# hitbc/deSAMBA

Measured on AMD Instinct MI355X. Metric: classified reads/s (50 kbp ONT reads, viral index), higher is better.
Workload: dtype u8/u64 integer

## Files before the change

desamba_amd/__init__.py:

```python
import ctypes as C
import os

_HERE = os.path.dirname(os.path.abspath(__file__))
LIB_PATH = os.environ.get("DSB_LIB_PATH", os.path.join(_HERE, "libdesamba_amd.so"))

DSB_OK, DSB_EIO, DSB_ENODEV, DSB_ENOMEM, DSB_EINVAL, DSB_ECAP = 0, -1, -2, -3, -4, -5


class DsbOpts(C.Structure):
    _fields_ = [("L_min_matching", C.c_int), ("min_score", C.c_int), ("max_sec_N", C.c_int), ("n_slots", C.c_int),
                ("max_read_len", C.c_uint32), ("max_batch_reads", C.c_uint32), ("input_slots", C.c_int), ("reserved", C.c_int), ("max_batch_bases", C.c_uint64)]


class DsbRead(C.Structure):
    _fields_ = [("name", C.c_char_p), ("seq", C.c_char_p), ("qual", C.c_char_p), ("len", C.c_uint32)]


class DsbHit(C.Structure):
    _fields_ = [("ref_ID", C.c_uint32), ("t_st", C.c_uint32), ("t_ed", C.c_uint32), ("q_st", C.c_uint32), ("q_ed", C.c_uint32),
                ("sum_score", C.c_uint32), ("indel", C.c_uint32), ("direction", C.c_uint8), ("primary", C.c_uint8),
                ("pri_index", C.c_uint8), ("pad", C.c_uint8)]

    def key(self):
        return (self.ref_ID, self.t_st, self.t_ed, self.q_st, self.q_ed, self.sum_score, self.direction, self.primary, self.pri_index)


class DsbReadResult(C.Structure):
    _fields_ = [("first", C.c_uint32), ("n", C.c_uint32), ("status", C.c_int32), ("fast", C.c_uint32), ("device_us", C.c_uint32), ("n_anc", C.c_uint32)]


class DsbResult(C.Structure):
    _fields_ = [("reads", C.POINTER(DsbReadResult)), ("hits", C.POINTER(DsbHit)), ("n_hits", C.c_size_t)]


class DsbSeed(C.Structure):
    _fields_ = [("offset", C.c_uint32), ("len", C.c_uint32), ("top", C.c_uint8), ("pad", C.c_uint8 * 3)]


class DsbTiming(C.Structure):
    _fields_ = [("encode_ms", C.c_float), ("seed_probe_ms", C.c_float), ("classify_ms", C.c_float), ("total_ms", C.c_float),
                ("windows", C.c_uint64), ("probes_t1", C.c_uint64), ("bases", C.c_uint64),
                ("order_ms", C.c_float), ("tail_ms", C.c_float), ("n_early", C.c_uint32), ("n_retry", C.c_uint32),
                ("n_regrow", C.c_uint32), ("seed_scan", C.c_uint32),
                ("n_occ", C.c_uint64), ("n_mem", C.c_uint64), ("n_sa", C.c_uint64), ("ref_bases", C.c_uint64),
                ("main_occ", C.c_uint64), ("main_mem", C.c_uint64), ("main_sa", C.c_uint64), ("main_ref_bases", C.c_uint64),
                ("n_heavy_mw", C.c_uint32), ("n_requeue", C.c_uint32), ("upload_bytes", C.c_uint64),
                ("anc_pool_asked", C.c_uint64), ("anc_pool_cap", C.c_uint64)]


class DsbBuildStats(C.Structure):
    _fields_ = [(n, C.c_uint64) for n in ("n_bases", "n_refs", "n_kmer", "n_unitig", "n_rows")] + \
               [(n, C.c_double) for n in ("parse_s", "sort_s", "graph_s", "walk_s", "rows_s", "tables_s", "write_s", "total_s")] + \
               [(n, C.c_uint64) for n in ("budget_bytes", "peak_device_bytes")] + \
               [(n, C.c_uint32) for n in ("ranges_kmers", "ranges_unitig_numbers", "ranges_rows", "ranges_exist")] + \
               [("spilled_bytes", C.c_uint64)]


class DsbReadTaxon(C.Structure):
    _fields_ = [("taxid", C.c_uint32), ("score", C.c_uint32), ("len", C.c_uint32), ("mapq", C.c_uint8), ("flags", C.c_uint8), ("pad", C.c_uint16)]


DSB_TAXON_CLASSIFIED, DSB_TAXON_HOST = 1, 2


class DsbRefCoverage(C.Structure):
    _fields_ = [("numreads", C.c_uint64), ("covbases", C.c_uint64), ("aligned_bases", C.c_uint64), ("mapq_sum", C.c_uint64)]


COVERAGE_FIELDS = ("numreads", "covbases", "aligned_bases", "mapq_sum")


class DsbEmOpts(C.Structure):
    _fields_ = [("max_iter", C.c_uint32), ("reserved", C.c_uint32), ("tol", C.c_double)]


class DsbAbundanceSummary(C.Structure):
    _fields_ = [("reads", C.c_uint64), ("classified", C.c_uint64), ("classes", C.c_uint64), ("iterations", C.c_uint32),
                ("converged", C.c_uint32), ("max_change", C.c_double), ("min_permille", C.c_uint32), ("reserved", C.c_uint32)]


ABUNDANCE_DTYPE = [("numreads", "<u8"), ("uniqreads", "<u8"), ("est_reads", "<f8"), ("read_share", "<f8"), ("copy_share", "<f8")]


class DsbReadLca(C.Structure):
    _fields_ = [("taxid", C.c_uint32), ("score", C.c_uint32), ("n_pass", C.c_uint32), ("depth", C.c_uint16), ("flags", C.c_uint8), ("pad", C.c_uint8)]


DSB_LCA_CLASSIFIED, DSB_LCA_NO_TAXON, DSB_LCA_AMBIGUOUS = 1, 2, 4
LCA_DTYPE = [("taxid", "<u4"), ("score", "<u4"), ("n_pass", "<u4"), ("depth", "<u2"), ("flags", "u1"), ("pad", "u1")]
TAXON_COUNT_DTYPE = [("taxid", "<u4"), ("pad", "<u4"), ("clade_reads", "<u8"), ("direct_reads", "<u8")]


class DsbLcaSummary(C.Structure):
    _fields_ = [("reads", C.c_uint64), ("classified", C.c_uint64), ("no_taxon", C.c_uint64), ("ambiguous", C.c_uint64),
                ("min_permille", C.c_uint32), ("reserved", C.c_uint32)]


LCA_SUMMARY_FIELDS = ("reads", "classified", "no_taxon", "ambiguous", "min_permille")


class DsbChunk(C.Structure):
    _fields_ = [("start", C.c_uint64), ("end", C.c_uint64), ("hist_max_before", C.c_uint32), ("rank", C.c_int32)]


EXPORTS = ["dsb_index_open", "dsb_index_close", "dsb_index_n_ref", "dsb_index_ref_name", "dsb_index_ref_len", "dsb_index_ek_len",
           "dsb_index_occ_host", "dsb_ctx_create", "dsb_ctx_destroy", "dsb_ctx_reset_history", "dsb_ctx_reload_env", "dsb_classify_batch",
           "dsb_batch_upload", "dsb_batch_upload_fastq", "dsb_batch_upload_text", "dsb_ctx_set_history", "dsb_host_alloc", "dsb_host_free", "dsb_host_cpus", "dsb_batch_run", "dsb_batch_fetch", "dsb_batch_timing", "dsb_batch_seeds", "dsb_batch_exist_bits",
           "dsb_format_sam", "dsb_format_des", "dsb_strerror", "dsb_version",
           "dsb_device_count", "dsb_ctx_select_slot", "dsb_ctx_create_multi", "dsb_multi_destroy", "dsb_multi_n", "dsb_multi_ctx",
           "dsb_multi_reset_history", "dsb_multi_last_calls", "dsb_multi_classify_batch", "dsb_shard_plan", "dsb_ctx_use_synthetic_filter", "dsb_synthetic_filter_bit", "dsb_index_prefix_interval", "dsb_index_build",
           "dsb_taxonomy_load", "dsb_taxonomy_load_any", "dsb_taxonomy_close", "dsb_taxonomy_max_tid", "dsb_taxonomy_parent",
           "dsb_ctx_set_taxonomy", "dsb_multi_set_taxonomy", "dsb_batch_taxa", "dsb_multi_taxa",
           "dsb_report_create", "dsb_report_add", "dsb_report_add_sam", "dsb_report_format", "dsb_report_destroy",
           "dsb_ctx_enable_coverage", "dsb_ctx_reset_coverage", "dsb_ctx_coverage", "dsb_multi_enable_coverage", "dsb_multi_coverage",
           "dsb_coverage_format", "dsb_ctx_enable_abundance", "dsb_ctx_reset_abundance", "dsb_ctx_abundance", "dsb_multi_enable_abundance",
           "dsb_multi_abundance", "dsb_abundance_format",
           "dsb_ctx_enable_lca", "dsb_ctx_reset_lca", "dsb_batch_lca", "dsb_ctx_lca_counts", "dsb_multi_enable_lca", "dsb_multi_lca",
           "dsb_multi_lca_counts", "dsb_taxnames_load", "dsb_taxnames_close", "dsb_format_kraken", "dsb_lca_report_format"]

_lib = None


def lib():
    global _lib
    if _lib is not None:
        return _lib
    if not os.path.exists(LIB_PATH):
        raise RuntimeError("desamba_amd: %s is missing -- run __graft_entry__.build(); there is no CPU fallback" % LIB_PATH)
    L = C.CDLL(LIB_PATH)
    L.dsb_index_open.argtypes = [C.c_char_p, C.POINTER(C.c_void_p)]
    L.dsb_index_close.argtypes = [C.c_void_p]
    L.dsb_index_n_ref.argtypes = [C.c_void_p]; L.dsb_index_n_ref.restype = C.c_uint64
    L.dsb_index_ref_name.argtypes = [C.c_void_p, C.c_uint32]; L.dsb_index_ref_name.restype = C.c_char_p
    L.dsb_index_ref_len.argtypes = [C.c_void_p, C.c_uint32]; L.dsb_index_ref_len.restype = C.c_uint64
    L.dsb_index_ek_len.argtypes = [C.c_void_p]
    L.dsb_index_occ_host.argtypes = [C.c_void_p, C.c_uint64, C.POINTER(C.c_uint8)]; L.dsb_index_occ_host.restype = C.c_uint64
    L.dsb_ctx_create.argtypes = [C.c_void_p, C.c_int, C.POINTER(DsbOpts), C.POINTER(C.c_void_p)]
    L.dsb_ctx_destroy.argtypes = [C.c_void_p]
    L.dsb_ctx_reset_history.argtypes = [C.c_void_p]
    L.dsb_ctx_reload_env.argtypes = [C.c_void_p]; L.dsb_ctx_reload_env.restype = None
    L.dsb_classify_batch.argtypes = [C.c_void_p, C.POINTER(DsbRead), C.c_size_t, C.POINTER(DsbResult)]
    L.dsb_batch_upload.argtypes = [C.c_void_p, C.POINTER(DsbRead), C.c_size_t]
    L.dsb_batch_upload_fastq.argtypes = [C.c_void_p, C.c_char_p, C.c_size_t, C.c_size_t]; L.dsb_batch_upload_fastq.restype = C.c_long
    L.dsb_batch_run.argtypes = [C.c_void_p]
    L.dsb_batch_fetch.argtypes = [C.c_void_p, C.POINTER(DsbResult)]
    L.dsb_batch_timing.argtypes = [C.c_void_p, C.POINTER(DsbTiming)]
    L.dsb_batch_seeds.argtypes = [C.c_void_p, C.c_size_t, C.c_int, C.POINTER(DsbSeed), C.c_size_t, C.POINTER(C.c_uint32), C.POINTER(C.c_uint32)]
    L.dsb_batch_exist_bits.argtypes = [C.c_void_p, C.c_size_t, C.c_int, C.POINTER(C.c_uint8), C.c_size_t, C.POINTER(C.c_uint32)]
    L.dsb_format_sam.argtypes = [C.c_void_p, C.POINTER(DsbRead), C.POINTER(DsbHit), C.c_uint32, C.c_int, C.c_int, C.c_char_p, C.c_size_t]
    L.dsb_format_sam.restype = C.c_long
    L.dsb_format_des.argtypes = [C.c_void_p, C.POINTER(DsbRead), C.POINTER(DsbReadResult), C.POINTER(DsbHit), C.c_int, C.c_int, C.c_char_p, C.c_size_t]
    L.dsb_format_des.restype = C.c_long
    L.dsb_batch_upload_text.argtypes = [C.c_void_p, C.c_void_p, C.c_size_t, C.POINTER(C.c_uint64), C.POINTER(C.c_uint32), C.c_size_t]
    L.dsb_ctx_set_history.argtypes = [C.c_void_p, C.c_uint32]; L.dsb_ctx_set_history.restype = None
    L.dsb_host_alloc.argtypes = [C.c_size_t]; L.dsb_host_alloc.restype = C.c_void_p
    L.dsb_host_free.argtypes = [C.c_void_p]; L.dsb_host_free.restype = None
    L.dsb_device_count.argtypes = []; L.dsb_device_count.restype = C.c_int
    L.dsb_ctx_select_slot.argtypes = [C.c_void_p, C.c_int]
    L.dsb_ctx_create_multi.argtypes = [C.c_void_p, C.POINTER(C.c_int), C.c_int, C.POINTER(DsbOpts), C.POINTER(C.c_void_p)]
    L.dsb_multi_destroy.argtypes = [C.c_void_p]; L.dsb_multi_destroy.restype = None
    L.dsb_multi_n.argtypes = [C.c_void_p]
    L.dsb_multi_ctx.argtypes = [C.c_void_p, C.c_int]; L.dsb_multi_ctx.restype = C.c_void_p
    L.dsb_multi_reset_history.argtypes = [C.c_void_p]; L.dsb_multi_reset_history.restype = None
    L.dsb_multi_last_calls.argtypes = [C.c_void_p, C.c_int]; L.dsb_multi_last_calls.restype = C.c_uint32
    L.dsb_multi_classify_batch.argtypes = [C.c_void_p, C.POINTER(DsbRead), C.c_size_t, C.POINTER(DsbResult)]
    L.dsb_shard_plan.argtypes = [C.POINTER(C.c_uint32), C.c_size_t, C.c_int, C.c_uint64, C.c_uint32, C.POINTER(DsbChunk), C.c_size_t, C.POINTER(C.c_size_t)]
    L.dsb_ctx_use_synthetic_filter.argtypes = [C.c_void_p, C.c_uint64, C.c_double]
    L.dsb_synthetic_filter_bit.argtypes = [C.c_int, C.c_uint64, C.c_double]
    L.dsb_index_prefix_interval.argtypes = [C.c_void_p, C.c_uint32, C.c_int, C.POINTER(C.c_uint64), C.POINTER(C.c_uint64)]
    L.dsb_index_build.argtypes = [C.c_char_p, C.c_char_p, C.c_char_p, C.c_int, C.POINTER(DsbBuildStats)]
    L.dsb_index_close.restype = None; L.dsb_ctx_destroy.restype = None; L.dsb_ctx_reset_history.restype = None
    L.dsb_taxonomy_load.argtypes = [C.c_char_p, C.POINTER(C.c_void_p)]
    L.dsb_taxonomy_load_any.argtypes = [C.c_char_p, C.POINTER(C.c_void_p)]
    L.dsb_taxonomy_close.argtypes = [C.c_void_p]; L.dsb_taxonomy_close.restype = None
    L.dsb_taxonomy_max_tid.argtypes = [C.c_void_p]; L.dsb_taxonomy_max_tid.restype = C.c_uint32
    L.dsb_taxonomy_parent.argtypes = [C.c_void_p, C.c_uint32]; L.dsb_taxonomy_parent.restype = C.c_uint32
    L.dsb_ctx_set_taxonomy.argtypes = [C.c_void_p, C.c_void_p]
    L.dsb_multi_set_taxonomy.argtypes = [C.c_void_p, C.c_void_p]
    L.dsb_batch_taxa.argtypes = [C.c_void_p, C.POINTER(C.POINTER(DsbReadTaxon))]
    L.dsb_multi_taxa.argtypes = [C.c_void_p, C.POINTER(C.POINTER(DsbReadTaxon))]
    L.dsb_report_create.argtypes = [C.c_void_p, C.POINTER(C.c_void_p)]
    L.dsb_report_add.argtypes = [C.c_void_p, C.c_void_p, C.POINTER(DsbRead), C.POINTER(DsbResult), C.POINTER(DsbReadTaxon), C.c_size_t, C.c_int]
    L.dsb_report_add_sam.argtypes = [C.c_void_p, C.c_char_p, C.c_size_t]
    L.dsb_report_format.argtypes = [C.c_void_p, C.c_int, C.c_char_p, C.c_size_t]; L.dsb_report_format.restype = C.c_long
    L.dsb_report_destroy.argtypes = [C.c_void_p]; L.dsb_report_destroy.restype = None
    L.dsb_ctx_enable_coverage.argtypes = [C.c_void_p, C.c_int]
    L.dsb_ctx_reset_coverage.argtypes = [C.c_void_p]
    L.dsb_ctx_coverage.argtypes = [C.c_void_p, C.c_void_p]
    L.dsb_multi_enable_coverage.argtypes = [C.c_void_p, C.c_int]
    L.dsb_multi_coverage.argtypes = [C.c_void_p, C.c_void_p]
    L.dsb_coverage_format.argtypes = [C.c_void_p, C.c_void_p, C.c_char_p, C.c_size_t]; L.dsb_coverage_format.restype = C.c_long
    L.dsb_ctx_enable_abundance.argtypes = [C.c_void_p, C.c_int, C.c_uint32]
    L.dsb_ctx_reset_abundance.argtypes = [C.c_void_p]
    L.dsb_ctx_abundance.argtypes = [C.c_void_p, C.c_void_p, C.c_void_p, C.c_void_p]
    L.dsb_multi_enable_abundance.argtypes = [C.c_void_p, C.c_int, C.c_uint32]
    L.dsb_multi_abundance.argtypes = [C.c_void_p, C.c_void_p, C.c_void_p, C.c_void_p]
    L.dsb_abundance_format.argtypes = [C.c_void_p, C.c_void_p, C.c_void_p, C.c_char_p, C.c_size_t]; L.dsb_abundance_format.restype = C.c_long
    L.dsb_ctx_enable_lca.argtypes = [C.c_void_p, C.c_int, C.c_uint32]
    L.dsb_ctx_reset_lca.argtypes = [C.c_void_p]
    L.dsb_batch_lca.argtypes = [C.c_void_p, C.POINTER(C.POINTER(DsbReadLca))]
    L.dsb_ctx_lca_counts.argtypes = [C.c_void_p, C.c_void_p, C.c_size_t, C.POINTER(C.c_size_t), C.c_void_p]
    L.dsb_multi_enable_lca.argtypes = [C.c_void_p, C.c_int, C.c_uint32]
    L.dsb_multi_lca.argtypes = [C.c_void_p, C.POINTER(C.POINTER(DsbReadLca))]
    L.dsb_multi_lca_counts.argtypes = [C.c_void_p, C.c_void_p, C.c_size_t, C.POINTER(C.c_size_t), C.c_void_p]
    L.dsb_taxnames_load.argtypes = [C.c_char_p, C.POINTER(C.c_void_p)]
    L.dsb_taxnames_close.argtypes = [C.c_void_p]; L.dsb_taxnames_close.restype = None
    L.dsb_format_kraken.argtypes = [C.c_void_p, C.c_void_p, C.c_char_p, C.c_size_t]; L.dsb_format_kraken.restype = C.c_long
    L.dsb_lca_report_format.argtypes = [C.c_void_p, C.c_void_p, C.c_void_p, C.c_size_t, C.c_void_p, C.c_char_p, C.c_size_t]; L.dsb_lca_report_format.restype = C.c_long
    L.dsb_strerror.argtypes = [C.c_int]; L.dsb_strerror.restype = C.c_char_p
    L.dsb_version.restype = C.c_char_p
    _lib = L
    return L


class DsbError(RuntimeError):
    def __init__(self, code, what):
        RuntimeError.__init__(self, "%s: %s (%d)" % (what, lib().dsb_strerror(code).decode(), code))
        self.code = code


class Index:

    def __init__(self, path):
        self.h = C.c_void_p()
        rc = lib().dsb_index_open(os.fsencode(path), C.byref(self.h))
        if rc != 0:
            raise DsbError(rc, "dsb_index_open(%s)" % path)
        self.path = path

    def close(self):
        if self.h:
            lib().dsb_index_close(self.h); self.h = C.c_void_p()

    @property
    def n_ref(self):
        return lib().dsb_index_n_ref(self.h)

    @property
    def ek_len(self):
        return lib().dsb_index_ek_len(self.h)

    def ref_name(self, i):
        return lib().dsb_index_ref_name(self.h, i).decode()

    def ref_len(self, i):
        return int(lib().dsb_index_ref_len(self.h, i))

    def occ_host(self, r, c):
        cc = C.c_uint8(c)
        v = lib().dsb_index_occ_host(self.h, r, C.byref(cc))
        return v, cc.value


def build_index(fasta, out_dir, kmer_srt=None, device=0):
    st = DsbBuildStats()
    rc = lib().dsb_index_build(kmer_srt.encode() if kmer_srt else None, fasta.encode(), out_dir.encode(), device, C.byref(st))
    if rc != 0:
        raise DsbError(rc, "dsb_index_build(%s)" % fasta)
    return st


def make_reads(records):
    n = len(records)
    arr = (DsbRead * n)()
    keep = []
    for i, (name, seq, qual) in enumerate(records):
        name = name if isinstance(name, bytes) else name.encode()
        seq = seq if isinstance(seq, bytes) else seq.encode()
        qual = (qual if isinstance(qual, bytes) else qual.encode()) if qual is not None else None
        keep.append((name, seq, qual))
        arr[i].name, arr[i].seq, arr[i].qual, arr[i].len = name, seq, qual, len(seq)
    arr._keep = keep
    return arr


class Ctx:

    def __init__(self, index, device=0, L_min_matching=170, min_score=64, max_sec_N=5, n_slots=0, max_read_len=0, max_batch_reads=0, input_slots=1, max_batch_bases=0):
        self.index = index
        self.opts = DsbOpts(L_min_matching, min_score, max_sec_N, n_slots, max_read_len, max_batch_reads, input_slots, 0, max_batch_bases)
        self.h = C.c_void_p()
        rc = lib().dsb_ctx_create(index.h, device, C.byref(self.opts), C.byref(self.h))
        if rc != 0:
            raise DsbError(rc, "dsb_ctx_create(device %d)" % device)
        self.reads = None
        self.slot = 0
        self.staged = {}
        self.ran = (None, 0)

    def close(self):
        if self.h:
            lib().dsb_ctx_destroy(self.h); self.h = C.c_void_p()

    def reset_history(self):
        lib().dsb_ctx_reset_history(self.h)

    def reload_env(self):
        lib().dsb_ctx_reload_env(self.h)

    def set_history(self, max_len_before):
        lib().dsb_ctx_set_history(self.h, max_len_before)

    def use_synthetic_filter(self, table_bytes, fill):
        rc = lib().dsb_ctx_use_synthetic_filter(self.h, table_bytes, fill)
        if rc != 0:
            raise DsbError(rc, "dsb_ctx_use_synthetic_filter")
        self.synthetic = (table_bytes, fill)

    def select_slot(self, slot):
        rc = lib().dsb_ctx_select_slot(self.h, slot)
        if rc != 0:
            raise DsbError(rc, "dsb_ctx_select_slot(%d)" % slot)
        self.slot = slot

    def upload_text(self, text_ptr, text_len, seq_off, seq_len, n):
        self.reads = None
        rc = lib().dsb_batch_upload_text(self.h, text_ptr, text_len, seq_off, seq_len, n)
        if rc != 0:
            raise DsbError(rc, "dsb_batch_upload_text")
        self.staged[self.slot] = (None, int(n))

    def upload(self, reads):
        self.reads = reads
        rc = lib().dsb_batch_upload(self.h, reads, len(reads))
        if rc != 0:
            raise DsbError(rc, "dsb_batch_upload")
        self.staged[self.slot] = (reads, len(reads))

    def upload_fastq(self, path, skip=0, max_reads=1 << 62):
        self.reads = None
        n = lib().dsb_batch_upload_fastq(self.h, os.fsencode(path), skip, max_reads)
        if n < 0:
            raise DsbError(int(n), "dsb_batch_upload_fastq(%s)" % path)
        self.n_uploaded = int(n)
        self.staged[self.slot] = (None, int(n))
        return int(n)

    def run(self):
        rc = lib().dsb_batch_run(self.h)
        if rc != 0:
            raise DsbError(rc, "dsb_batch_run")
        self.ran = self.staged.get(self.slot, (None, 0))

    def fetch(self, strict=True):
        res = DsbResult()
        rc = lib().dsb_batch_fetch(self.h, C.byref(res))
        if rc != 0 and (strict or rc != DSB_ECAP):
            raise DsbError(rc, "dsb_batch_fetch")
        return res

    def classify(self, reads, strict=True):
        self.upload(reads); self.run()
        return self.fetch(strict)

    def timing(self):
        t = DsbTiming()
        lib().dsb_batch_timing(self.h, C.byref(t))
        return t

    def seeds(self, read, strand):
        cap = (self.reads[read].len >> 1) + 64
        buf = (DsbSeed * cap)(); n = C.c_uint32(); ts = C.c_uint32()
        rc = lib().dsb_batch_seeds(self.h, read, strand, buf, cap, C.byref(n), C.byref(ts))
        if rc != 0:
            raise DsbError(rc, "dsb_batch_seeds")
        return [(buf[i].offset, buf[i].len, buf[i].top) for i in range(n.value)], ts.value

    def exist_bits(self, read, strand):
        cap = self.reads[read].len + 1
        buf = (C.c_uint8 * cap)(); n = C.c_uint32()
        rc = lib().dsb_batch_exist_bits(self.h, read, strand, buf, cap, C.byref(n))
        if rc != 0:
            raise DsbError(rc, "dsb_batch_exist_bits")
        return bytes(buf[:n.value])

    def set_taxonomy(self, taxonomy):
        rc = lib().dsb_ctx_set_taxonomy(self.h, taxonomy.h if taxonomy is not None else None)
        if rc != 0:
            raise DsbError(rc, "dsb_ctx_set_taxonomy")
        self.taxonomy = taxonomy

    def taxa(self, records=False):
        p = C.POINTER(DsbReadTaxon)()
        rc = lib().dsb_batch_taxa(self.h, C.byref(p))
        if rc != 0:
            raise DsbError(rc, "dsb_batch_taxa")
        n = self.in_last_batch()
        return _taxa(p, n, records)

    def enable_coverage(self, on=True):
        rc = lib().dsb_ctx_enable_coverage(self.h, 1 if on else 0)
        if rc != 0:
            raise DsbError(rc, "dsb_ctx_enable_coverage")

    def reset_coverage(self):
        rc = lib().dsb_ctx_reset_coverage(self.h)
        if rc != 0:
            raise DsbError(rc, "dsb_ctx_reset_coverage")

    def coverage(self):
        return _coverage(lib().dsb_ctx_coverage, self.h, self.index.n_ref, "dsb_ctx_coverage")

    def enable_abundance(self, on=True, min_frac=0.95):
        rc = lib().dsb_ctx_enable_abundance(self.h, 1 if on else 0, _permille(min_frac) if on else 0)
        if rc != 0:
            raise DsbError(rc, "dsb_ctx_enable_abundance")

    def reset_abundance(self):
        rc = lib().dsb_ctx_reset_abundance(self.h)
        if rc != 0:
            raise DsbError(rc, "dsb_ctx_reset_abundance")

    def abundance(self, max_iter=10000, tol=0.01):
        return _abundance(lib().dsb_ctx_abundance, self.h, self.index.n_ref, max_iter, tol, "dsb_ctx_abundance")

    def enable_lca(self, on=True, min_frac=0.95):
        rc = lib().dsb_ctx_enable_lca(self.h, 1 if on else 0, _permille(min_frac) if on else 0)
        if rc != 0:
            raise DsbError(rc, "dsb_ctx_enable_lca")

    def reset_lca(self):
        rc = lib().dsb_ctx_reset_lca(self.h)
        if rc != 0:
            raise DsbError(rc, "dsb_ctx_reset_lca")

    def lca(self):
        p = C.POINTER(DsbReadLca)()
        rc = lib().dsb_batch_lca(self.h, C.byref(p))
        if rc != 0:
            raise DsbError(rc, "dsb_batch_lca")
        return _lca(p, self.in_last_batch())

    def lca_counts(self):
        return _lca_counts(lib().dsb_ctx_lca_counts, self.h, "dsb_ctx_lca_counts")

    def in_last_batch(self):
        return self.ran[1]

    def sam(self, res, full=False, reads=None):
        if reads is None:
            reads = self.ran[0] if self.ran[0] is not None else self.reads
        return format_sam(self.index, reads, res, self.opts.max_sec_N, full)


def format_sam(index, reads, res, max_sec_N=5, full=False):
    out = []
    buf = C.create_string_buffer(1 << 20)
    for i in range(len(reads)):
        rr = res.reads[i]
        hits = C.cast(C.byref(res.hits.contents, rr.first * C.sizeof(DsbHit)), C.POINTER(DsbHit)) if rr.n else None
        cap = len(buf)
        need = 4096 + 700 * rr.n + (2 * reads[i].len if full else 0)
        if need > cap:
            buf = C.create_string_buffer(need)
        n = lib().dsb_format_sam(index.h, C.byref(reads[i]), hits, rr.n, max_sec_N, 1 if full else 0, buf, len(buf))
        if n < 0:
            raise DsbError(DSB_EINVAL, "dsb_format_sam")
        out.append(buf.raw[:n])
    return b"".join(out)


class Multi:

    def __init__(self, index, devices, L_min_matching=170, min_score=64, max_sec_N=5, n_slots=0):
        self.index = index
        self.opts = DsbOpts(L_min_matching, min_score, max_sec_N, n_slots, 0, 0, 1, 0)
        ids = (C.c_int * len(devices))(*devices)
        self.h = C.c_void_p()
        rc = lib().dsb_ctx_create_multi(index.h, ids, len(devices), C.byref(self.opts), C.byref(self.h))
        if rc != 0:
            raise DsbError(rc, "dsb_ctx_create_multi(%r)" % (devices,))

    def close(self):
        if self.h:
            lib().dsb_multi_destroy(self.h); self.h = C.c_void_p()

    def reset_history(self):
        lib().dsb_multi_reset_history(self.h)

    def last_calls(self):
        return [int(lib().dsb_multi_last_calls(self.h, i)) for i in range(int(lib().dsb_multi_n(self.h)))]

    def classify(self, reads, strict=True):
        res = DsbResult()
        rc = lib().dsb_multi_classify_batch(self.h, reads, len(reads), C.byref(res))
        if rc != 0 and (strict or rc != DSB_ECAP):
            raise DsbError(rc, "dsb_multi_classify_batch")
        self.n_last = len(reads)
        return res

    def set_taxonomy(self, taxonomy):
        rc = lib().dsb_multi_set_taxonomy(self.h, taxonomy.h if taxonomy is not None else None)
        if rc != 0:
            raise DsbError(rc, "dsb_multi_set_taxonomy")
        self.taxonomy = taxonomy

    def enable_coverage(self, on=True):
        rc = lib().dsb_multi_enable_coverage(self.h, 1 if on else 0)
        if rc != 0:
            raise DsbError(rc, "dsb_multi_enable_coverage")

    def coverage(self):
        return _coverage(lib().dsb_multi_coverage, self.h, self.index.n_ref, "dsb_multi_coverage")

    def enable_abundance(self, on=True, min_frac=0.95):
        rc = lib().dsb_multi_enable_abundance(self.h, 1 if on else 0, _permille(min_frac) if on else 0)
        if rc != 0:
            raise DsbError(rc, "dsb_multi_enable_abundance")

    def reset_abundance(self):
        for i in range(int(lib().dsb_multi_n(self.h))):
            rc = lib().dsb_ctx_reset_abundance(lib().dsb_multi_ctx(self.h, i))
# ... 310 lines not shown
```

desamba_amd/csrc/dsb_ctx.h:

```cpp
#pragma once
#include <stdio.h>
#include <string.h>
#include <time.h>
#include <string>
#include "dsb_seed_scan.h"
#include "dsb_reductions.h"

#define HIPCHK(e) do { hipError_t _e = (e); if (_e != hipSuccess) { fprintf(stderr, "[desamba_amd] HIP error %s at %s:%d\n", hipGetErrorString(_e), __FILE__, __LINE__); return DSB_ENODEV; } } while (0)

struct DsbStaged;

struct InSlot {
	DsbReadDesc *d_rd = nullptr; char *d_ascii = nullptr; size_t cap_rd = 0, cap_ascii = 0;
	std::vector<DsbReadDesc> h_rd;
	size_t n_reads = 0; uint64_t n_words_total = 0, total_bases = 0, total_windows = 0, seed_entries = 0; uint32_t max_len = 0, min_len = 0;
	uint32_t *d_scan_order = nullptr; size_t cap_scan_order = 0;
	bool ragged = false;
	uint64_t upload_bytes = 0;
	bool packed = false;
};

struct UpStage { char *buf[2] = {nullptr, nullptr}; hipEvent_t ev[2] = {nullptr, nullptr}; bool used[2] = {false, false}; hipStream_t st = nullptr; };

struct DsbKnobs {
	bool upload_text = false;
	bool debug = false, upload_trace = false, no_turn = false, turn_whole_run = false, no_group = false, heavy_first_set = false;
	long hout_cap = 0, sms_cap = 0, anc_cap_rt = 0, upload_chunk_kb = 0, step_limit_rt = 0, group_head = -1;
	int upload_threads = 0, seed_scan = -1, heavy_mw = -1, heavy_first = 0;
	bool heavy_preds_set = false; uint32_t heavy_preds = 0;
	uint64_t em_hash_mask = ~0ull;
	bool anchor_kernel = true; long anc_pool_rt = 0;
	bool scan_look_set = false; DsbScanLook scan_look;
	std::string order_file;
};
inline bool g_upload_trace = false;

struct dsb_ctx {
	bool ek_dense = false;
	DsbKnobs knobs;
	dsb_index *idx = nullptr; int device = 0; hipStream_t stream = nullptr;
	DsbStaged *staged = nullptr; DsbDevIndex dx;
	std::vector<InSlot> in; int cur = 0;
	DsbWordDesc *d_wd = nullptr; uint8_t *d_bin = nullptr; uint64_t *d_pk = nullptr; uint64_t *d_bits = nullptr;
	size_t cap_wd = 0, cap_bin = 0, cap_pk = 0, cap_bits = 0;
	DsbReadOut *d_rout = nullptr; DsbHitOut *d_hout = nullptr; size_t cap_rout = 0, cap_hout = 0;
	unsigned int *d_counters = nullptr;
	DsbSlotArena arena; int n_slots = 0, n_extra = 0;
	DsbSlotArena arena_big; int n_slots_big = 0;
	DsbSlotArena arena_anc; int n_slots_anc = 0;
	DsbAncRec *d_arec = nullptr; DsbAnchor *d_apool = nullptr; size_t cap_arec = 0, cap_apool = 0;
	uint32_t hint_len = 0;
	unsigned mw_reads = 16; bool mw_grown = false; int mw_calm = 0;
	uint32_t *d_score = nullptr, *d_order = nullptr, *d_heavy = nullptr; size_t cap_score = 0, cap_order = 0, cap_heavy = 0;
	DsbSeed *d_seeds = nullptr; DsbSeedInfo *d_sinfo = nullptr; size_t cap_seeds = 0, cap_sinfo = 0;
	uint8_t *d_summ = nullptr; int summ_shift = 0;
	uint8_t *syn0 = nullptr, *syn1 = nullptr; bool seed_only = false;
	bool bits_valid = false, seeds_valid = false;
	unsigned n_early = 0;
	std::vector<DsbReadOut> h_rout; std::vector<DsbHitOut> h_hout;
	std::vector<dsb_read_result> res_reads;
	int hist_max = 0;
	hipEvent_t ev[4] = {nullptr, nullptr, nullptr, nullptr}; dsb_timing timing; unsigned long long p1 = 0;
	hipStream_t stream3 = nullptr; hipEvent_t ev_heavy3 = nullptr;
	hipStream_t stream2 = nullptr; hipEvent_t ev_order = nullptr, ev_heavy = nullptr, ev_hprobe = nullptr, ev_cls = nullptr, ev_cls_wait = nullptr;
	uint32_t *dbg_host = nullptr, *dbg_dev = nullptr;
	std::vector<UpStage> up; size_t up_chunk = 0;
	dsb_opts opts;
	DsbTaxa taxa; DsbCover cover; DsbEmStore em; DsbLca lca;
	dsb_ctx() { memset(&dx, 0, sizeof dx); memset(&arena, 0, sizeof arena); memset(&arena_big, 0, sizeof arena_big); memset(&arena_anc, 0, sizeof arena_anc); memset(&timing, 0, sizeof timing); memset(&opts, 0, sizeof opts); }
};

struct dsb_multi {
	dsb_index *idx = nullptr; std::vector<dsb_ctx *> ctx; uint32_t hist = 0;
	uint32_t chunk_reads_env = 0;
	std::vector<uint32_t> last_calls;
	std::vector<dsb_read_result> reads; std::vector<dsb_hit> hits;
	const dsb_taxonomy *tx = nullptr; std::vector<dsb_read_taxon> taxa; bool taxa_ok = false;
	std::vector<dsb_read_lca> lca; bool lca_on = false, lca_ok = false;
};

template <class T> static int grow(T **p, size_t *cap, size_t need)
{
	if (need <= *cap) return 0;
	const bool tr = g_upload_trace; struct timespec t0, t1; if (tr) clock_gettime(CLOCK_MONOTONIC, &t0);
	const size_t old = *cap;
	if (*p) hipFree(*p);
	size_t n = need + need / 8 + 1024;
	if (hipMalloc((void **)p, n * sizeof(T)) != hipSuccess) { *p = nullptr; *cap = 0; return DSB_ENOMEM; }
	*cap = n;
	if (tr) { clock_gettime(CLOCK_MONOTONIC, &t1); fprintf(stderr, "[upload] a device buffer grew from %zu to %zu elements of %zu bytes (needed: %zu) in %.3f s\n", old, n, sizeof(T), need, (t1.tv_sec - t0.tv_sec) + 1e-9 * (t1.tv_nsec - t0.tv_nsec)); }
	return 0;
}
```

desamba_amd/csrc/dsb_gpu.hip:

```cpp
#include <hip/hip_runtime.h>
#include <stdint.h>
#include <stdio.h>
#include <string.h>
#include <stdlib.h>
#include <vector>
#include <string>
#include <unistd.h>
#include <fcntl.h>
#include <sys/mman.h>
#include <sys/stat.h>
#include "dsb_device.h"
#include "dsb_probe.h"
#include "dsb_seed_scan.h"
#define DSB_GROUP 64
#define DSB_NS dsb_g64
#include "dsb_classify_dev.h"
#undef DSB_GROUP
#undef DSB_NS
#include "dsb_host.h"
#include "dsb_sam_fields.h"

#if !defined(DSB_KUNIT)
#define DSB_UNIT_HAS(n) 1
#define DSB_UNIT_HOST 1
// ... 170 lines not shown
}
#define DSB_HPROBE_SPLIT 16
__global__ void __launch_bounds__(256) k_seed_probe_reads(DsbDevIndex x, const DsbReadDesc *__restrict__ rd, const uint32_t *__restrict__ list,
                                                          const uint64_t *__restrict__ pk, uint64_t *__restrict__ bits, const uint8_t *__restrict__ summ, int summ_shift)
{
	const int lane = threadIdx.x & 63;
	const uint32_t wave = __builtin_amdgcn_readfirstlane((uint32_t)((blockIdx.x % DSB_HPROBE_SPLIT) * 4 + (threadIdx.x >> 6)));
	const uint32_t r = list[blockIdx.x / DSB_HPROBE_SPLIT];
	const uint32_t n_words = rd[r].n_words, n_items = 2 * n_words;
	const int k = x.ek_len; const int sbm = x.single_base_max;
	const uint64_t kmask = k >= 32 ? ~0ULL : ((1ULL << (2 * k)) - 1ULL);
	unsigned long long p1_local = 0;
	for (uint32_t w0 = wave * DSB_PROBE_UN; w0 < n_items; w0 += 4 * DSB_HPROBE_SPLIT * DSB_PROBE_UN) {
		DsbWordDesc wds[DSB_PROBE_UN]; bool have[DSB_PROBE_UN];
#pragma unroll
		for (int u = 0; u < DSB_PROBE_UN; u++) {
			uint32_t it = w0 + u; have[u] = it < n_items;
			wds[u].read = r; wds[u].word = it >= n_words ? ((it - n_words) | 0x80000000u) : it;
		}
		probe_un(x, rd, pk, bits, wds, have, lane, k, sbm, kmask, summ, summ_shift, p1_local);
	}
}


__global__ void __launch_bounds__(256) k_seed_scan(DsbDevIndex x, const DsbReadDesc *__restrict__ rd, const uint32_t *__restrict__ order, uint32_t n_reads,
                                                   const uint64_t *__restrict__ pk, DsbSeed *__restrict__ seeds, DsbSeedInfo *__restrict__ sinfo,
                                                   const uint8_t *__restrict__ summ, int summ_shift, unsigned long long *counters, DsbScanLook look)
{
	const uint64_t g = (uint64_t)blockIdx.x * 256 + threadIdx.x;
	const bool active = g < 2ull * n_reads;
	const uint32_t r = active ? (order ? order[g >> 1] : (uint32_t)(g >> 1)) : 0u;
	const bool rc = (g & 1) != 0;
	DsbReadDesc d = rd[r];
	const uint64_t *__restrict__ P = pk + d.pk_off;
	const uint32_t L = d.len, nF = L >> 2, cap = rc ? ((L >> 1) + 64 - nF) : nF;
	DsbSeed *__restrict__ sv = seeds + d.seed_off + (rc ? nF : 0);
	auto store = [&](uint32_t idx, uint32_t off, uint32_t len) { if (idx < cap) { DsbSeed v; v.offset = off; v.len = (uint16_t)len; v.top = 0; sv[idx] = v; } };
	auto mark = [&](uint32_t idx) { if (idx < cap) sv[idx].top = 1; };
	const int k = x.ek_len, sbm = x.single_base_max;
	const uint64_t kmask = k >= 32 ? ~0ULL : ((1ULL << (2 * k)) - 1ULL);
	DsbScan s; dsb_scan_init(s, active ? d.n_win : 0u, look);
	uint32_t p0 = 0, p1 = 0;
	uint64_t K0 = 0, K1 = 0, K2 = 0; uint32_t wbase = 0xfffffff0u;
	for (;;) {
		if (!__any(s.mode != DSB_SCAN_DONE)) break;
		uint32_t want[DSB_SCAN_W]; dsb_scan_want(s, want);
		uint32_t lo = DSB_SCAN_NONE;
#pragma unroll
		for (int t = 0; t < DSB_SCAN_W; t++) lo = want[t] < lo ? want[t] : lo;
		const uint32_t base = lo & ~31u;
		if (lo != DSB_SCAN_NONE) {
			const uint32_t wi = lo >> 5;
			uint64_t n0, n1, n2;
#define DSB_SCAN_WORD(dst, idx) \
			if ((idx) == wbase) dst = K0; else if ((idx) == wbase + 1) dst = K1; else if ((idx) == wbase + 2) dst = K2; \
			else { dst = P[idx]; if (rc) dst = dsb_revcomp_kmer(dst, 32); }
			DSB_SCAN_WORD(n0, wi) DSB_SCAN_WORD(n1, wi + 1) DSB_SCAN_WORD(n2, wi + 2)
#undef DSB_SCAN_WORD
			K0 = n0; K1 = n1; K2 = n2; wbase = wi;
		}
		const uint64_t B0 = rc ? K2 : K0, B1 = K1, B2 = rc ? K0 : K2;
		uint64_t km[DSB_SCAN_W], h1[DSB_SCAN_W]; bool ok[DSB_SCAN_W];
#pragma unroll
		for (int t = 0; t < DSB_SCAN_W; t++) {
			ok[t] = want[t] != DSB_SCAN_NONE; km[t] = 0; h1[t] = 0;
			if (ok[t]) {
				uint32_t rel = want[t] - base;
				if (rc) rel = 96u - rel - (uint32_t)k;
				const uint64_t a = rel < 32 ? B0 : rel < 64 ? B1 : B2, b = rel < 32 ? B1 : B2; const uint32_t sh = (rel & 31u) * 2;
				const uint64_t hi = sh ? ((a << sh) | (b >> (64 - sh))) : a;
				const uint64_t v = (hi >> (64 - 2 * k)) & kmask;
				ok[t] = dsb_kmer_ok(v, k, sbm); km[t] = v;
				if (ok[t]) { p0++; h1[t] = dsb_ph1(v) & x.ek_mask; }
			}
		}
		if (summ) {
			uint8_t sb[DSB_SCAN_W];
#pragma unroll
			for (int t = 0; t < DSB_SCAN_W; t++) { sb[t] = 0xff; if (ok[t]) sb[t] = summ[(h1[t] >> summ_shift) >> 3]; }
#pragma unroll
			for (int t = 0; t < DSB_SCAN_W; t++) ok[t] = ok[t] && ((sb[t] >> ((h1[t] >> summ_shift) & 7)) & 1);
		}
		uint8_t t0[DSB_SCAN_W];
#pragma unroll
		for (int t = 0; t < DSB_SCAN_W; t++) { t0[t] = 0; if (ok[t]) t0[t] = x.ek0[h1[t] >> 3]; }
		bool any1 = false;
#pragma unroll
		for (int t = 0; t < DSB_SCAN_W; t++) { ok[t] = ok[t] && ((t0[t] >> (7 - (h1[t] & 7))) & 1); any1 |= ok[t]; }
		uint32_t bits = 0;
		if (__any(any1)) {
			uint8_t t1[DSB_SCAN_W]; uint64_t h2[DSB_SCAN_W];
#pragma unroll
			for (int t = 0; t < DSB_SCAN_W; t++) { t1[t] = 0; h2[t] = 0; if (ok[t]) { h2[t] = dsb_ph2(km[t]) & x.ek_mask; t1[t] = x.ek1[h2[t] >> 3]; p1++; } }
#pragma unroll
			for (int t = 0; t < DSB_SCAN_W; t++) if (ok[t] && ((t1[t] >> (7 - (h2[t] & 7))) & 1)) bits |= 1u << t;
		}
		if (s.mode != DSB_SCAN_DONE) dsb_scan_consume(s, bits, rc, store, mark);
	}
	dsb_scan_finish(s, mark);
	if (active) { sinfo[r].n_seed[rc ? 1 : 0] = s.ns; sinfo[r].total[rc ? 1 : 0] = s.total; if (!rc) { sinfo[r].flags = 0; sinfo[r].pad = 0; } }
	if (counters) {
		unsigned long long a0 = p0, a1 = p1;
		for (int o = 32; o > 0; o >>= 1) { a0 += __shfl_down(a0, o); a1 += __shfl_down(a1, o); }
		if ((threadIdx.x & 63) == 0) { if (a0) atomicAdd(counters, a0); if (a1) atomicAdd(counters + 1, a1); }
	}
}

__host__ __device__ inline uint32_t dsb_synth_mix(uint64_t b, uint32_t which)
{
	uint64_t z = b * 0x9E3779B97F4A7C15ULL + ((uint64_t)which + 1) * 0xD1342543DE82EF95ULL;
	z = (z ^ (z >> 30)) * 0xBF58476D1CE4E5B9ULL; z = (z ^ (z >> 27)) * 0x94D049BB133111EBULL;
	return (uint32_t)((z ^ (z >> 31)) >> 40);
}
__global__ void __launch_bounds__(256) k_synth_table(uint8_t *tab, uint64_t n_bytes, uint32_t which, uint32_t thresh)
{
	for (uint64_t i = (uint64_t)blockIdx.x * 256 + threadIdx.x; i < n_bytes; i += (uint64_t)gridDim.x * 256) {
		uint32_t v = 0;
#pragma unroll
		for (int j = 0; j < 8; j++) if (dsb_synth_mix(i * 8 + j, which) < thresh) v |= 1u << (7 - j);
		tab[i] = (uint8_t)v;
	}
}

__global__ void __launch_bounds__(256) k_repeat_score(const DsbReadDesc *rd, const uint64_t *pk, uint32_t *score)
{
	__shared__ uint32_t bloom[1u << 13];
	__shared__ uint32_t dup;
	DsbReadDesc d = rd[blockIdx.x];
	for (uint32_t i = threadIdx.x; i < (1u << 13); i += 256) bloom[i] = 0;
	if (threadIdx.x == 0) dup = 0;
	__syncthreads();
	const uint64_t *P = pk + d.pk_off;
	uint32_t n = d.len >= 12 ? d.len - 12 + 1 : 0, mine = 0;
	for (uint32_t p = 2 * threadIdx.x; p < n; p += 512) {
		uint32_t w0 = p >> 5, sh = (p & 31) * 2;
		uint64_t a = P[w0], b = P[w0 + 1];
		uint64_t hi = sh ? ((a << sh) | (b >> (64 - sh))) : a;
		uint64_t kmer = hi >> 40;
		uint32_t h1 = (uint32_t)(dsb_ph1(kmer) >> 20) & 0x3ffffu, h2 = (uint32_t)(dsb_ph2(kmer) >> 13) & 0x3ffffu;
		uint32_t o1 = atomicOr(&bloom[h1 >> 5], 1u << (h1 & 31)), o2 = atomicOr(&bloom[h2 >> 5], 1u << (h2 & 31));
		if ((o1 >> (h1 & 31)) & (o2 >> (h2 & 31)) & 1u) mine++;
	}
	if (mine) atomicAdd(&dup, mine);
	__syncthreads();
	if (threadIdx.x == 0) score[blockIdx.x] = dup;
}
__device__ __forceinline__ uint32_t order_bucket(uint32_t s)
{
	s |= 1u;
	const uint32_t lg = 31u - (uint32_t)__clz((int)s);
	const uint32_t mant = lg >= 6u ? (s >> (lg - 6u)) & 63u : (s << (6u - lg)) & 63u;
	return lg * 64u + mant;
}
__global__ void __launch_bounds__(1024) k_order(const uint32_t *score, uint32_t n, uint32_t *order)
{
	__shared__ uint32_t hist[2048], start[2048];
	hist[threadIdx.x] = 0; hist[threadIdx.x + 1024] = 0;
	__syncthreads();
	for (uint32_t i = threadIdx.x; i < n; i += 1024) atomicAdd(&hist[order_bucket(score[i])], 1u);
	__syncthreads();
	if (threadIdx.x == 0) { uint32_t acc = 0; for (int b = 2047; b >= 0; b--) { start[b] = acc; acc += hist[b]; } }
	__syncthreads();
	for (uint32_t i = threadIdx.x; i < n; i += 1024) order[atomicAdd(&start[order_bucket(score[i])], 1u)] = i;
}

#endif

#ifndef DSB_WAVES_PER_EU
#define DSB_WAVES_PER_EU 3
#endif
#if DSB_UNIT_HAS(1) || DSB_UNIT_HAS(2) || DSB_UNIT_HAS(3)
__device__ __forceinline__ void classify_kernel_body(const DsbDevIndex &x, const DsbReadDesc *rd, uint32_t n_fixed, const unsigned int *n_ptr,
        const uint32_t *list, uint8_t *bin, const uint64_t *bits, const DsbSlotArena &ar, unsigned int *work_counter, DsbReadOut *rout,
        DsbHitOut *hout, unsigned int *hout_counter, uint32_t hout_cap, uint32_t *dbg, uint32_t item_base, uint32_t slot_base, unsigned long long *work_cnt, DsbSeed *seed_blob, const DsbSeedInfo *sinfo, const uint64_t *pk, uint32_t group_mode,
        const DsbAncRec *arec, const DsbAnchor *apool)
{
	const int lane = threadIdx.x;
	const uint32_t slot_id = slot_base + blockIdx.x;
	uint8_t *slot = ar.base + (size_t)slot_id * ar.stride;
	__shared__ DsbDevIndex sx;
	__shared__ uint4 lds_ring[DSB_RING];
	__shared__ __attribute__((aligned(16))) uint32_t lds_wtab[DSB_WTAB_SLOTS];
	__shared__ uint32_t lds_red[2];
	__shared__ unsigned int s_word;
	__shared__ uint32_t lds_cnt[4];
	__shared__ dsb_g64::DpBatch lds_dpb;
	if (lane < 4) lds_cnt[lane] = 0;
	if (lane == 0) sx = x;
	__syncthreads();
	__shared__ dsb_g64::WCtx s_w;
	dsb_g64::WCtxL &w = *(dsb_g64::WCtxL *)&s_w;
	w.ring = lds_ring; w.dpb = (dsb_g64::DpBatchL *)&lds_dpb; w.red = lds_red; w.k.c = (dsb_g64::lds_u32 *)lds_cnt; w.k.uni = 1;
	w.x = (dsb_g64::DsbXP)&sx; w.dbg = dbg ? dbg + 4 * slot_id : nullptr;
	for (int i = 0; i < 14; i++) w.tacc[i] = 0;
	for (int i = 0; i < 10; i++) w.tx[i] = 0;
	w.seeds = (DsbSeed *)(slot + ar.off_seeds);
	w.anc = (DsbAnchor *)(slot + ar.off_anc); w.anc_tmp = (DsbAnchor *)(slot + ar.off_anc_tmp);
	w.hit = (DsbChain *)(slot + ar.off_hit); w.hit_tmp = (DsbChain *)(slot + ar.off_hit_tmp);
	w.sms = (DsbSms *)(slot + ar.off_sms);
	w.sc = (DsbScHash *)(slot + ar.off_sc); w.wtab = lds_wtab;
	w.mem_slow = (DsbMem *)(slot + ar.off_mem);
	w.spset = (uint64_t *)(slot + ar.off_spset);
	w.score_v = (int *)(slot + ar.off_scorev);
	w.sortkey = (uint64_t *)(slot + ar.off_sortkey); w.sortidx = (uint32_t *)(slot + ar.off_sortidx);
	w.win_mid = slot + ar.off_win + DSB_REFWIN_FRONT; w.win_right = w.win_mid + DSB_REFWIN; w.win_left = w.win_right + DSB_REFWIN;
	w.lane_anc = (DsbAnchor *)(slot + ar.off_lane_anc); w.lane_spset = (uint64_t *)(slot + ar.off_lane_sp);
	w.top_idx = (uint32_t *)(slot + ar.off_top); w.round_info = (uint32_t *)(slot + ar.off_round);
	w.anc_cap = ar.anc_cap; w.anc_cap_main = ar.anc_cap; w.hit_cap = ar.hit_cap; w.step_limit = x.step_limit; w.heavy_limit = x.heavy_limit; w.sp_gen = 0; w.mw = nullptr; w.n_waves = 1;
	for (uint32_t i = lane; i < 64u * DSB_SPHASH; i += 64) w.lane_spset[i] = 0;
	for (uint32_t i = lane; i < DSB_SPHASH; i += 64) w.spset[i] = 0;
	__syncthreads();
	const unsigned int n_items = n_ptr ? *n_ptr : n_fixed;
	if (w.dbg && lane == 0) w.dbg[0] = 300;
	for (;;) {
		unsigned int n_grp = 1u;
		if (group_mode && seed_blob) n_grp = __hip_atomic_load(work_counter, __ATOMIC_RELAXED, __HIP_MEMORY_SCOPE_AGENT) >= group_mode ? 64u : 1u;
		n_grp = (unsigned int)__builtin_amdgcn_readfirstlane((int)n_grp);
		if (lane == 0) s_word = atomicAdd(work_counter, n_grp);
		__syncthreads();
		unsigned int k = s_word + item_base;
		__syncthreads();
		if (k >= n_items) {
			if (lane < 4 && lds_cnt[lane]) atomicAdd(work_cnt + lane, (unsigned long long)lds_cnt[lane]);
			if (w.dbg && lane == 0) { w.dbg[0] = 999; for (int i = 0; i < 14; i++) dbg[4 * 65536 + 14 * slot_id + i] += (uint32_t)(w.tacc[i] / 100); for (int i = 0; i < 10; i++) dbg[8 * 65536 + 10 * slot_id + i] += (uint32_t)(i < 6 ? w.tx[i] / 100 : w.tx[i]); }
			break;
		}
		uint32_t g_nanc = 0, g_ovf = 0;
		if (n_grp > 1) {
			const bool valid = k + lane < n_items;
			const unsigned int rl = valid ? (list ? list[k + lane] : k + lane) : 0u;
			const DsbReadDesc dl = rd[rl];
			uint64_t tg = w.dbg ? wall_clock64() : 0;
			dsb_g64::fast_classify_lane(w, valid, bin + dl.bin_off + DSB_QPAD_L, dl.len, seed_blob + dl.seed_off, sinfo + rl, &g_nanc, &g_ovf);
			if (w.dbg) w.tacc[1] += wall_clock64() - tg;
		}
		for (unsigned int pass = 0; pass < (n_grp > 1 ? 2u : 1u); pass++)
		for (unsigned int gl = 0; gl < n_grp; gl++) {
			const unsigned int pos = k + gl;
			if (pos >= n_items) break;
			bool have_anc = false;
			if (n_grp > 1) {
				const uint32_t ovf_l = dsb_g64::dsb_shfl(g_ovf, (int)gl);
				if ((ovf_l != 0) != (pass == 1)) continue;
				have_anc = !ovf_l;
			}
		unsigned int r = list ? list[pos] : pos;
		DsbReadDesc d = rd[r];
		uint64_t t_start = wall_clock64();
		uint64_t tacc0[14]; if (w.dbg) for (int i = 0; i < 14; i++) tacc0[i] = w.tacc[i];
		if (w.dbg && lane == 0) { w.dbg[2] = r; w.dbg[0] = 100; }
		w.bin = bin + d.bin_off + DSB_QPAD_L; w.L = d.len; w.status = 0; w.max_read_l = d.hist_max;
		w.pre_seeds = seed_blob ? seed_blob + d.seed_off : nullptr; w.pre_info = sinfo + r;
		w.pk[0] = pk + d.pk_off; w.pk[1] = w.pk[0] + ((d.len + 31) / 32 + 1);
		uint32_t anc_lsteps = 0;
		if (have_anc) {
			const uint32_t na = dsb_g64::dsb_shfl(g_nanc, (int)gl);
			const DsbAnchor *src = w.lane_anc + (size_t)gl * DSB_LANE_ANC_CAP;
			for (uint32_t i = lane; i < na; i += 64) w.anc[i] = src[i];
			w.n_anc = na;
			dsb_g64::wave_sync();
		} else if (arec) {
			const DsbAncRec ar_r = arec[r];
			if (ar_r.use) {
				const DsbAnchor *src = apool + ar_r.off;
				for (uint32_t i = lane; i < ar_r.n; i += 64) w.anc[i] = src[i];
				w.n_anc = ar_r.n; anc_lsteps = ar_r.lsteps; have_anc = true;
				dsb_g64::wave_sync();
			}
		}
		uint32_t fast = dsb_g64::classify_read<false>(w, bits + d.bit_off, bits + d.bit_off + d.n_words, have_anc, anc_lsteps);
		if (w.boosted) __builtin_amdgcn_s_setprio(0);
		if (w.status & DSB_ST_HEAVY) w.n_hit = 0;
		if (lane == 0) s_word = w.n_hit ? atomicAdd(hout_counter, w.n_hit) : 0u;
		__syncthreads();
		unsigned int first = s_word;
		__syncthreads();
		uint32_t n_out = w.n_hit;
		if (first + n_out > hout_cap) { w.status |= DSB_ST_OUT_OVF; n_out = 0; }
		for (uint32_t i = lane; i < n_out; i += 64) {
			DsbChain h = w.hit[i]; DsbHitOut o;
			o.ref_ID = h.ref_ID; o.t_st = h.t_st; o.t_ed = h.t_ed; o.q_st = h.q_st; o.q_ed = h.q_ed; o.sum_score = h.sum_score; o.indel = h.indel;
			o.direction = h.direction; o.primary = h.primary; o.pri_index = h.pri_index; o.pad = 0;
			hout[first + i] = o;
		}
		if (w.dbg && lane == 0) { w.dbg[0] = 200; if (r < 65536u) for (int i = 0; i < 14; i++) dbg[16 * 65536 + 14 * r + i] = (uint32_t)((w.tacc[i] - tacc0[i]) / 100); }
		if (lane == 0) { DsbReadOut ro; ro.first = first; ro.n = n_out; ro.status = w.status | (w.status ? (w.stage << 8) : 0);
			ro.fast = fast | ((uint32_t)((wall_clock64() - t_start) / 100) << 1); ro.n_anc = w.n_anc; ro.pad = 0; rout[r] = ro; }
		}
	}
}
#endif

#define DSB_CLASSIFY_ARGS DsbDevIndex x, const DsbReadDesc *rd, uint32_t n_fixed, const unsigned int *n_ptr, const uint32_t *list, uint8_t *bin, const uint64_t *bits, DsbSlotArena ar, \
        unsigned int *work_counter, DsbReadOut *rout, DsbHitOut *hout, unsigned int *hout_counter, uint32_t hout_cap, uint32_t *dbg, uint32_t item_base, uint32_t slot_base, unsigned long long *work_cnt, \
        DsbSeed *seed_blob, const DsbSeedInfo *sinfo, const uint64_t *pk, uint32_t group_mode, const DsbAncRec *arec, const DsbAnchor *apool
#define DSB_CLASSIFY_PASS x, rd, n_fixed, n_ptr, list, bin, bits, ar, work_counter, rout, hout, hout_counter, hout_cap, dbg, item_base, slot_base, work_cnt, seed_blob, sinfo, pk, group_mode, arec, apool
#if DSB_UNIT_HAS(1)
__global__ void __launch_bounds__(64, DSB_WAVES_PER_EU) k_classify(DSB_CLASSIFY_ARGS) { classify_kernel_body(DSB_CLASSIFY_PASS); }
#else
__global__ void k_classify(DSB_CLASSIFY_ARGS);
#endif
#if DSB_UNIT_HAS(2)
__global__ void __launch_bounds__(64, DSB_WAVES_PER_EU) k_classify_early(DSB_CLASSIFY_ARGS) { classify_kernel_body(DSB_CLASSIFY_PASS); }
#else
__global__ void k_classify_early(DSB_CLASSIFY_ARGS);
#endif
#if DSB_UNIT_HAS(3)
__global__ void __launch_bounds__(64, DSB_WAVES_PER_EU) k_classify_second(DSB_CLASSIFY_ARGS) { classify_kernel_body(DSB_CLASSIFY_PASS); }
#else
__global__ void k_classify_second(DSB_CLASSIFY_ARGS);
#endif

#ifndef DSB_ANCHOR_WPE
#define DSB_ANCHOR_WPE 5
#endif
#if DSB_UNIT_HAS(5)
// ... 147 lines not shown
			if (first + n_out > hout_cap) { w.status |= DSB_ST_OUT_OVF; n_out = 0; }
			for (uint32_t i = lane; i < n_out; i += 64) {
				DsbChain h = w.hit[i]; DsbHitOut o;
				o.ref_ID = h.ref_ID; o.t_st = h.t_st; o.t_ed = h.t_ed; o.q_st = h.q_st; o.q_ed = h.q_ed; o.sum_score = h.sum_score; o.indel = h.indel;
				o.direction = h.direction; o.primary = h.primary; o.pri_index = h.pri_index; o.pad = 0;
				hout[first + i] = o;
			}
			if (lane == 0) { DsbReadOut ro; ro.first = first; ro.n = n_out; ro.status = w.status | (w.status ? (w.stage << 8) : 0);
				ro.fast = fast | ((uint32_t)((wall_clock64() - t_start) / 100) << 1); ro.n_anc = w.n_anc; ro.pad = 0; rout[r] = ro; }
		} else {
			__builtin_amdgcn_s_setprio(3);
			for (;;) {
				__syncthreads();
				const uint32_t cmd = mw.cmd;
				if (cmd == 3) break;
				if (cmd == 1) dsb_g64::sdp_batch_old_mw<1>(&mw, lds_ring, lds_red, lane, wv, MWW, nullptr);
				else dsb_g64::sdp_batch_old_mw<2>(&mw, lds_ring, lds_red, lane, wv, MWW, nullptr);
			}
		}
	}
}
#if defined(DSB_KUNIT)
template __global__ void k_classify_heavy<8>(DsbDevIndex, const DsbReadDesc *, uint32_t, const unsigned int *, const uint32_t *, uint8_t *, const uint64_t *, DsbSlotArena, unsigned int *, DsbReadOut *, DsbHitOut *, unsigned int *, uint32_t, uint32_t, unsigned long long *, const uint64_t *, DsbSeed *, const DsbSeedInfo *);
#endif
#else
template <int MWW>
__global__ void k_classify_heavy(DsbDevIndex x, const DsbReadDesc *rd, uint32_t n_fixed, const unsigned int *n_ptr,
        const uint32_t *list, uint8_t *bin, const uint64_t *bits, DsbSlotArena ar, unsigned int *work_counter, DsbReadOut *rout,
        DsbHitOut *hout, unsigned int *hout_counter, uint32_t hout_cap, uint32_t slot_base, unsigned long long *work_cnt, const uint64_t *pk,
        DsbSeed *seed_blob, const DsbSeedInfo *sinfo);
#endif

#if DSB_UNIT_HOST
__global__ void k_collect_retry(const DsbReadOut *rout, uint32_t n, uint32_t *list, unsigned int *count, int mask, int clear_n)
{
	uint32_t i = blockIdx.x * 256 + threadIdx.x;
	if (i >= n) return;
	int st = rout[i].status & 0xff;
	if (st & mask) list[atomicAdd(count, 1u)] = i;
	(void)clear_n;
}

#include "dsb_ctx.h"
#include <mutex>
#include <thread>
#include <algorithm>

struct DsbStaged {
	const dsb_index *idx; int device; int refs;
	DsbDevIndex dx;
	std::vector<void *> allocs;
	uint8_t *d_summ; int summ_shift;
	bool ek_dense = false;
	std::mutex run_mu;
};
static std::mutex g_stage_mu;
static std::vector<DsbStaged *> g_staged;

template <class T> static int stage_upload(DsbStaged *s, const T *src, size_t n, const T **dst)
{
	void *p = nullptr;
	if (hipMalloc(&p, n * sizeof(T) + 256) != hipSuccess) return DSB_ENOMEM;
	s->allocs.push_back(p);
	if (hipMemcpy(p, src, n * sizeof(T), hipMemcpyHostToDevice) != hipSuccess) return DSB_ENODEV;
	*dst = (const T *)p;
	return 0;
}
static void stage_free(DsbStaged *s)
{
	hipSetDevice(s->device);
	for (void *p : s->allocs) hipFree(p);
	delete s;
}
static int stage_build(dsb_index *idx, int device, DsbStaged **out)
{
	const DsbHostIndex *h = dsb_index_host(idx);
	DsbStaged *s = new DsbStaged(); s->idx = idx; s->device = device; s->refs = 0; s->d_summ = nullptr; s->summ_shift = 0;
	DsbDevIndex &dx = s->dx; memset(&dx, 0, sizeof dx);
	int rc = 0;
#define ST(call) do { if (!rc) rc = (call); } while (0)
	ST(stage_upload(s, h->ek0, h->ek_size, &dx.ek0));
	ST(stage_upload(s, h->ek1, h->ek_size, &dx.ek1));
	dx.ek_mask = h->ek_mask; dx.ek_len = h->ek_len; dx.single_base_max = h->single_base_max;
	if (!rc) {
		const char *lv = getenv("DSB_EK_SUMMARY");
		int shift = lv ? atoi(lv) : (h->ek_size <= (256ull << 20) ? 6 : h->ek_size <= (1024ull << 20) ? 8 : 0);
		if (shift >= 3 && shift <= 8 && (h->ek_size >> (shift - 3)) >= 4096) {
			uint64_t n_out = h->ek_size >> shift;
			void *p = nullptr;
			if (hipMalloc(&p, n_out + 256) != hipSuccess) rc = DSB_ENOMEM;
			else {
				s->allocs.push_back(p); s->d_summ = (uint8_t *)p; s->summ_shift = shift;
				hipLaunchKernelGGL(k_ek_summary, dim3((unsigned)((n_out + 255) / 256)), dim3(256), 0, 0, dx.ek0, n_out, shift, s->d_summ);
				if (hipDeviceSynchronize() != hipSuccess) rc = DSB_ENODEV;
				if (!rc && !lv) {
					std::vector<uint64_t> hs((n_out + 7) / 8, 0);
					if (hipMemcpy(hs.data(), s->d_summ, n_out, hipMemcpyDeviceToHost) != hipSuccess) rc = DSB_ENODEV;
					uint64_t ones = 0; for (uint64_t v : hs) ones += (uint64_t)__builtin_popcountll(v);
					if ((double)ones > 0.9 * 8.0 * (double)n_out) { s->d_summ = nullptr; s->summ_shift = 0; s->ek_dense = true; }
				}
			}
		}
	}
	ST(stage_upload(s, h->fm, h->n_fm, &dx.fm));
	if (h->fm_sb) ST(stage_upload(s, h->fm_sb, h->n_fm_sb * 5, &dx.fm_sb));
	dx.bwt_len = h->bwt_len; memcpy(dx.rank, h->rank, sizeof dx.rank); dx.dollar_pos = h->dollar_pos; dx.dollar_row = h->dollar_row;
	if (h->hash_c) { ST(stage_upload(s, h->hash_c, (size_t)h->n_hash_c, &dx.hash_c)); dx.hash_index = nullptr; }
	else { ST(stage_upload(s, h->hash_index, ((size_t)1 << 26) + 1, &dx.hash_index)); dx.hash_c = nullptr; }
	ST(stage_upload(s, (const uint2 *)h->sa, h->sa_size, &dx.sa));
	ST(stage_upload(s, (const uint2 *)h->uni, h->n_uni + 1, &dx.uni));
	ST(stage_upload(s, h->refpos, h->n_refpos + 1, &dx.refpos));
	ST(stage_upload(s, h->refbin, h->n_refbin + 4096, &dx.refbin)); dx.ref_bases = h->n_refbin * 4;
	ST(stage_upload(s, h->refinfo, h->n_ref, &dx.refinfo));
	ST(stage_upload(s, h->Q_MEM, (size_t)2000, &dx.qmem));
	ST(stage_upload(s, &h->Q_LV[0][0], (size_t)400, &dx.qlv));
#undef ST
	if (rc) { stage_free(s); return rc; }
	*out = s;
	return 0;
}
static int stage_acquire(dsb_index *idx, int device, DsbStaged **out)
{
	std::lock_guard<std::mutex> g(g_stage_mu);
	for (DsbStaged *s : g_staged) if (s->idx == idx && s->device == device) { s->refs++; *out = s; return 0; }
	DsbStaged *s = nullptr; int rc = stage_build(idx, device, &s);
	if (rc) return rc;
	s->refs = 1; g_staged.push_back(s); *out = s;
	return 0;
}
static void stage_release(DsbStaged *s)
{
	std::lock_guard<std::mutex> g(g_stage_mu);
	if (--s->refs > 0) return;
	for (size_t i = 0; i < g_staged.size(); i++) if (g_staged[i] == s) { g_staged.erase(g_staged.begin() + i); break; }
	stage_free(s);
}

static void knobs_read(DsbKnobs &k)
{
	auto num = [](const char *name, long dflt) { const char *e = getenv(name); return e ? atol(e) : dflt; };
	k = DsbKnobs();
	k.debug = getenv("DSB_DEBUG") != nullptr; k.upload_trace = getenv("DSB_UPLOAD_TRACE") != nullptr;
	k.upload_text = getenv("DSB_UPLOAD_TEXT") != nullptr;
	k.no_turn = getenv("DSB_NO_TURN") != nullptr; k.turn_whole_run = getenv("DSB_TURN_WHOLE_RUN") != nullptr; k.no_group = getenv("DSB_NO_GROUP") != nullptr;
	k.hout_cap = num("DSB_HOUT_CAP", 0); if (getenv("DSB_HOUT_CAP") && k.hout_cap <= 0) k.hout_cap = 1;
	k.sms_cap = num("DSB_SMS_CAP", 0); if (getenv("DSB_SMS_CAP") && k.sms_cap < 64) k.sms_cap = 64;
	k.anc_cap_rt = num("DSB_ANC_CAP_RT", 0); if (getenv("DSB_ANC_CAP_RT")) { if (k.anc_cap_rt < 64) k.anc_cap_rt = 64; if (k.anc_cap_rt > DSB_ANC_CAP) k.anc_cap_rt = DSB_ANC_CAP; }
	k.upload_chunk_kb = num("DSB_UPLOAD_CHUNK_KB", 0); k.upload_threads = (int)num("DSB_UPLOAD_THREADS", 0);
	k.step_limit_rt = num("DSB_STEP_LIMIT_RT", 0); k.group_head = num("DSB_GROUP_HEAD", -1);
	k.seed_scan = getenv("DSB_SEED_SCAN") ? (num("DSB_SEED_SCAN", 0) != 0 ? 1 : 0) : -1;
	k.heavy_mw = getenv("DSB_HEAVY_MW") ? (int)num("DSB_HEAVY_MW", 0) : -1;
	k.heavy_first_set = getenv("DSB_HEAVY_FIRST") != nullptr; k.heavy_first = (int)num("DSB_HEAVY_FIRST", 0);
	k.anchor_kernel = num("DSB_ANCHOR_KERNEL", 1) != 0;
	if (getenv("DSB_EM_HASH_BITS")) { const long b = num("DSB_EM_HASH_BITS", 64); k.em_hash_mask = b >= 64 ? ~0ull : b < 1 ? 1ull : (1ull << b) - 1; }
	k.anc_pool_rt = num("DSB_ANC_POOL_RT", 0); if (getenv("DSB_ANC_POOL_RT") && k.anc_pool_rt < 1) k.anc_pool_rt = 1;
	if (const char *e = getenv("DSB_HEAVY_PREDS")) { k.heavy_preds_set = true; k.heavy_preds = (uint32_t)strtoul(e, nullptr, 10); }
	if (const char *e = getenv("DSB_ORDER_FILE")) k.order_file = e;
	k.scan_look_set = false;
	if (const char *e = getenv("DSB_SCAN_LOOK")) {
		int a = 0, b = 0, f = 0, st = 0;
		if (sscanf(e, "%d,%d,%d,%d", &a, &b, &f, &st) == 4 && a >= 1 && a <= DSB_SCAN_W && b >= 1 && b <= DSB_SCAN_W - 2 && f >= 1 && f <= DSB_SCAN_W && st >= 1 && st <= DSB_SCAN_W) {
			k.scan_look.after_seed = (uint8_t)a; k.scan_look.back_fwd = (uint8_t)b; k.scan_look.fwd_n = (uint8_t)f; k.scan_look.stride_n = (uint8_t)st; k.scan_look_set = true;
		}
	}
	g_upload_trace = k.upload_trace;
}


extern "C" int dsb_device_count(void)
{
	int n = 0;
	return hipGetDeviceCount(&n) == hipSuccess ? n : 0;
}

static int ensure_buffers(dsb_ctx *c, size_t n, uint32_t max_len, uint64_t bin_bytes, uint64_t pk_words, uint64_t bit_words, uint64_t seed_entries);
struct SeqView { const char *p; uint32_t len; };
static int upload_views(dsb_ctx *c, const SeqView *reads, size_t n, const char *ext_text = nullptr, size_t ext_len = 0, const uint64_t *ext_off = nullptr);
static int upload_stages(dsb_ctx *c, int T);
static int upload_threads(const dsb_ctx *c);

extern "C" void dsb_ctx_reload_env(dsb_ctx *c)
{
	if (!c) return;
	knobs_read(c->knobs);
}

extern "C" void dsb_ctx_destroy(dsb_ctx *c)
{
	if (!c) return;
	hipSetDevice(c->device);
	if (c->stream) hipStreamSynchronize(c->stream);
	if (c->stream2) hipStreamSynchronize(c->stream2);
	for (InSlot &s : c->in) { hipFree(s.d_rd); hipFree(s.d_ascii); hipFree(s.d_scan_order); }
	hipFree(c->d_wd); hipFree(c->d_bin); hipFree(c->d_pk); hipFree(c->d_bits);
	reductions_release(c);
	hipFree(c->d_rout); hipFree(c->d_hout); hipFree(c->d_counters); hipFree(c->arena.base); hipFree(c->arena_big.base); hipFree(c->arena_anc.base); hipFree(c->d_arec); hipFree(c->d_apool); hipFree(c->d_score); hipFree(c->d_order); hipFree(c->d_heavy); hipFree(c->d_seeds); hipFree(c->d_sinfo); hipFree(c->syn0); hipFree(c->syn1);
	if (c->dbg_host) hipHostFree(c->dbg_host);
	for (UpStage &u : c->up) { if (u.st) { hipStreamSynchronize(u.st); hipStreamDestroy(u.st); } for (int k = 0; k < 2; k++) { if (u.ev[k]) hipEventDestroy(u.ev[k]); if (u.buf[k]) hipHostFree(u.buf[k]); } }
	for (int i = 0; i < 4; i++) if (c->ev[i]) hipEventDestroy(c->ev[i]);
	if (c->ev_order) hipEventDestroy(c->ev_order);
	if (c->ev_cls) hipEventDestroy(c->ev_cls);
	if (c->ev_cls_wait) hipEventDestroy(c->ev_cls_wait);
	if (c->ev_heavy) hipEventDestroy(c->ev_heavy);
	if (c->ev_hprobe) hipEventDestroy(c->ev_hprobe);
	if (c->stream2) hipStreamDestroy(c->stream2);
	if (c->stream3) { hipStreamSynchronize(c->stream3); hipStreamDestroy(c->stream3); }
	if (c->ev_heavy3) hipEventDestroy(c->ev_heavy3);
	if (c->stream) hipStreamDestroy(c->stream);
	if (c->staged) stage_release(c->staged);
	delete c;
}

extern "C" int dsb_ctx_create(dsb_index *idx, int device_id, const dsb_opts *opts, dsb_ctx **out)
{
	if (!idx || !out) return DSB_EINVAL;
	int ndev = 0;
	if (hipGetDeviceCount(&ndev) != hipSuccess || ndev <= 0) { fprintf(stderr, "[desamba_amd] no HIP device: this library has no CPU path\n"); return DSB_ENODEV; }
	if (device_id < 0 || device_id >= ndev) return DSB_EINVAL;
	HIPCHK(hipSetDevice(device_id));
	hipDeviceProp_t prop; HIPCHK(hipGetDeviceProperties(&prop, device_id));
	if (strncmp(prop.gcnArchName, "gfx950", 6) != 0) { fprintf(stderr, "[desamba_amd] device %d is %s, kernels are built for gfx950 only\n", device_id, prop.gcnArchName); return DSB_ENODEV; }
	dsb_ctx *c = new dsb_ctx();
	knobs_read(c->knobs);
	c->idx = idx; c->device = device_id;
	if (opts) c->opts = *opts;
	else { c->opts.L_min_matching = 170; c->opts.min_score = 64; c->opts.max_sec_N = 5; }
	int rc = DSB_OK;
#define CK(e) do { if (rc == DSB_OK && (e) != hipSuccess) { fprintf(stderr, "[desamba_amd] HIP error %s at %s:%d\n", hipGetErrorString(hipGetLastError()), __FILE__, __LINE__); rc = DSB_ENODEV; } } while (0)
	CK(hipStreamCreateWithFlags(&c->stream, hipStreamNonBlocking));
	for (int i = 0; i < 3; i++) CK(hipEventCreate(&c->ev[i]));
	CK(hipEventCreateWithFlags(&c->ev[3], hipEventBlockingSync));
	CK(hipStreamCreateWithFlags(&c->stream2, hipStreamNonBlocking)); CK(hipEventCreate(&c->ev_order)); CK(hipEventCreate(&c->ev_cls)); CK(hipEventCreateWithFlags(&c->ev_cls_wait, hipEventBlockingSync));
	CK(hipEventCreateWithFlags(&c->ev_heavy, hipEventDisableTiming)); CK(hipEventCreateWithFlags(&c->ev_hprobe, hipEventDisableTiming));
	CK(hipStreamCreateWithFlags(&c->stream3, hipStreamNonBlocking)); CK(hipEventCreateWithFlags(&c->ev_heavy3, hipEventDisableTiming));
	if (rc == DSB_OK) rc = stage_acquire(idx, device_id, &c->staged);
	if (rc == DSB_OK) {
		c->dx = c->staged->dx; c->d_summ = c->staged->d_summ; c->summ_shift = c->staged->summ_shift; c->ek_dense = c->staged->ek_dense;
		c->dx.filter_min_length = c->opts.L_min_matching; c->dx.filter_min_score = c->opts.min_score; c->dx.filter_min_score_LV3 = c->opts.min_score + 10;
		if (hipMalloc((void **)&c->d_counters, 256) != hipSuccess) rc = DSB_ENOMEM;
	}
	if (rc == DSB_OK && c->knobs.debug) {
		CK(hipHostMalloc((void **)&c->dbg_host, 32 * 65536 * sizeof(uint32_t), hipHostMallocMapped | hipHostMallocCoherent));
		if (rc == DSB_OK) { memset(c->dbg_host, 0, 32 * 65536 * sizeof(uint32_t)); CK(hipHostGetDevicePointer((void **)&c->dbg_dev, c->dbg_host, 0)); }
	}
#undef CK
	if (rc == DSB_OK) {
		c->in.resize(c->opts.input_slots > 1 ? (size_t)c->opts.input_slots : 1);
		if (c->opts.max_read_len && c->opts.max_batch_reads) {
			const uint32_t L = c->opts.max_read_len; const size_t n = c->opts.max_batch_reads; const int k = c->dx.ek_len;
			c->hint_len = L;
			const uint64_t nwin = L >= 40 ? L - k + 1 : 0;
			if (c->opts.max_batch_bases) {
				const uint64_t B = c->opts.max_batch_bases;
				rc = ensure_buffers(c, n, L, 2 * B + n * (uint64_t)(DSB_QPAD_L + DSB_QPAD_R + 256), B / 16 + 4 * (uint64_t)n, B / 32 + 4 * (uint64_t)n, B / 2 + 64 * (uint64_t)n);
				for (InSlot &s : c->in) { if (!rc) rc = grow(&s.d_rd, &s.cap_rd, n + 1); if (!rc) rc = grow(&s.d_ascii, &s.cap_ascii, (size_t)B + 64); if (!rc) rc = grow(&s.d_scan_order, &s.cap_scan_order, n + 1); }
			} else
			rc = ensure_buffers(c, n, L, n * ((DSB_QPAD_L + 2 * (uint64_t)L + DSB_QPAD_R + 255) & ~(uint64_t)255), n * 2 * ((L + 31) / 32 + 1), n * 2 * ((nwin + 63) / 64), n * (((uint64_t)L >> 1) + 64));
		}
	}
	if (rc == DSB_OK && c->opts.max_read_len && c->opts.max_batch_reads && !getenv("DSB_NO_WARMUP")) {
		std::vector<char> seq(2048); uint64_t z = 88172645463325252ULL;
		for (char &ch : seq) { z ^= z << 13; z ^= z >> 7; z ^= z << 17; ch = "ACGT"[z & 3]; }
		SeqView v[4]; for (int i = 0; i < 4; i++) { v[i].p = seq.data() + 100 * i; v[i].len = 1500; }
		rc = upload_stages(c, upload_threads(c));
		if (rc == DSB_OK) rc = upload_views(c, v, 4);
		if (rc == DSB_OK) rc = dsb_batch_run(c);
		c->hist_max = 0; c->in[c->cur].n_reads = 0; memset(&c->timing, 0, sizeof c->timing);
		if (rc == DSB_ECAP) rc = DSB_OK;
	}
	if (rc != DSB_OK) { dsb_ctx_destroy(c); return rc; }
	*out = c;
	return DSB_OK;
}

extern "C" int dsb_synthetic_filter_bit(int which, uint64_t bit, double fill)
{
	return dsb_synth_mix(bit, (uint32_t)which) < (uint32_t)(fill * 16777216.0);
}
extern "C" int dsb_ctx_use_synthetic_filter(dsb_ctx *c, uint64_t table_bytes, double fill)
{
	if (!c || fill <= 0 || fill >= 1) return DSB_EINVAL;
	int bits, k;
	switch (table_bytes) {
	case 1ULL << 27: bits = 30; k = 16; break; case 1ULL << 28: bits = 31; k = 17; break; case 1ULL << 29: bits = 32; k = 17; break;
	case 1ULL << 30: bits = 33; k = 18; break; case 1ULL << 31: bits = 34; k = 18; break; case 1ULL << 32: bits = 35; k = 19; break;
	case 1ULL << 33: bits = 36; k = 19; break; case 1ULL << 34: bits = 37; k = 20; break;
	default: return DSB_EINVAL;
	}
	HIPCHK(hipSetDevice(c->device));
	hipFree(c->syn0); hipFree(c->syn1); c->syn0 = c->syn1 = nullptr;
	if (hipMalloc((void **)&c->syn0, table_bytes + 256) != hipSuccess || hipMalloc((void **)&c->syn1, table_bytes + 256) != hipSuccess) return DSB_ENOMEM;
	const uint32_t thresh = (uint32_t)(fill * 16777216.0);
	hipLaunchKernelGGL(k_synth_table, dim3(256 * 16), dim3(256), 0, c->stream, c->syn0, table_bytes, 0u, thresh);
	hipLaunchKernelGGL(k_synth_table, dim3(256 * 16), dim3(256), 0, c->stream, c->syn1, table_bytes, 1u, thresh);
	HIPCHK(hipStreamSynchronize(c->stream));
	c->dx.ek0 = c->syn0; c->dx.ek1 = c->syn1; c->dx.ek_mask = (1ULL << bits) - 1; c->dx.ek_len = k; c->dx.single_base_max = (int)(0.8 * k);
	c->d_summ = nullptr; c->summ_shift = 0;
	c->ek_dense = fill > 0.04;
	c->seed_only = true;
	return DSB_OK;
}

extern "C" void dsb_ctx_reset_history(dsb_ctx *c) { if (c) c->hist_max = 0; }
extern "C" void dsb_ctx_set_history(dsb_ctx *c, uint32_t max_len_before) { if (c) c->hist_max = (int)max_len_before; }
extern "C" int dsb_ctx_select_slot(dsb_ctx *c, int slot)
{
	if (!c || slot < 0 || (size_t)slot >= c->in.size()) return DSB_EINVAL;
	c->cur = slot;
	return DSB_OK;
}
#include <sched.h>
static bool gpu_node_cpus(cpu_set_t *set)
{
	int dev = 0; char bdf[64] = {0};
	if (hipGetDevice(&dev) != hipSuccess || hipDeviceGetPCIBusId(bdf, sizeof bdf, dev) != hipSuccess) return false;
	for (char *q = bdf; *q; q++) *q = (char)tolower(*q);
	char path[192]; snprintf(path, sizeof path, "/sys/bus/pci/devices/%s/numa_node", bdf);
	FILE *f = fopen(path, "r"); if (!f) return false;
	int node = -1; if (fscanf(f, "%d", &node) != 1) node = -1;
	fclose(f);
	if (node < 0) return false;
	snprintf(path, sizeof path, "/sys/devices/system/node/node%d/cpulist", node);
	f = fopen(path, "r"); if (!f) return false;
	char list[4096] = {0}; const bool got = fgets(list, sizeof list, f) != nullptr; fclose(f);
	if (!got) return false;
	CPU_ZERO(set); int n = 0;
	for (char *q = list; *q && *q != '\n';) {
		char *e; long a = strtol(q, &e, 10), b = a;
		if (e == q) break;
		if (*e == '-') { q = e + 1; b = strtol(q, &e, 10); }
		for (long c = a; c <= b && c < CPU_SETSIZE; c++) { CPU_SET((int)c, set); n++; }
		q = (*e == ',') ? e + 1 : e;
	}
	return n > 0;
}
extern "C" void *dsb_host_alloc(size_t bytes)
{
	cpu_set_t old, want; bool moved = false;
	if (!getenv("DSB_NO_NUMA") && sched_getaffinity(0, sizeof old, &old) == 0 && gpu_node_cpus(&want)) {
		cpu_set_t both; CPU_AND(&both, &old, &want);
		if (CPU_COUNT(&both) > 0) moved = sched_setaffinity(0, sizeof both, &both) == 0;
	}
	void *p = nullptr;
	const bool ok = hipHostMalloc(&p, bytes, hipHostMallocDefault) == hipSuccess;
	if (moved) sched_setaffinity(0, sizeof old, &old);
	return ok ? p : nullptr;
}
extern "C" void dsb_host_free(void *p) { if (p) hipHostFree(p); }

static size_t al256(size_t v) { return (v + 255) & ~(size_t)255; }

#define DSB_HEAVY_SLOTS 512
#define DSB_RETRY_SLOTS 64
#define DSB_RETRY_GROW 32
#define DSB_RETRY_MAX_NODES (8u << 20)
#define DSB_RETRY_ANC (8u * DSB_ANC_CAP)
#define DSB_RETRY_HIT (4u * DSB_HIT_CAP)
static size_t arena_layout(DsbSlotArena &a, uint32_t max_len, int group, uint32_t sms_cap, uint32_t anc_cap, uint32_t hit_cap)
{
	size_t o = 0; const size_t f = hit_cap ? 1 : 0;
	a.max_len = max_len; a.sms_cap = sms_cap; a.anc_cap = anc_cap; a.hit_cap = hit_cap;
	a.off_seeds = o;   o += f * al256(((size_t)(max_len >> 1) + 64) * sizeof(DsbSeed));
	a.off_anc = o;     o += al256((size_t)anc_cap * sizeof(DsbAnchor));
	a.off_anc_tmp = o; o += f * al256((size_t)anc_cap * sizeof(DsbAnchor));
	a.off_hit = o;     o += al256((size_t)hit_cap * sizeof(DsbChain));
	a.off_hit_tmp = o; o += al256((size_t)hit_cap * sizeof(DsbChain));
	a.off_sms = o;     o += f * al256((size_t)sms_cap * sizeof(DsbSms));
	a.off_sc = o;      o += f * al256((size_t)(256 + 2 * 400 + 64) * sizeof(DsbScHash));
	a.off_mem = o;     o += f * al256((size_t)DSB_MEMSLOW_CAP * sizeof(DsbMem));
	a.off_spset = o;   o += al256((size_t)DSB_SPHASH * 8);
	a.off_scorev = o;  o += f * al256((size_t)1024 * sizeof(int));
	a.off_sortkey = o; o += f * al256((size_t)2 * anc_cap * sizeof(uint64_t));
	a.off_sortidx = o; o += al256((size_t)2 * anc_cap * sizeof(uint32_t));
	a.off_win = o;     o += f * al256((size_t)3 * DSB_REFWIN + DSB_REFWIN_FRONT);
	a.off_lane_anc = o; o += al256((size_t)group * DSB_LANE_ANC_CAP * sizeof(DsbAnchor));
	a.off_lane_sp = o;  o += al256((size_t)group * DSB_SPHASH * 8);
	a.off_top = o;      o += al256(((size_t)(max_len >> 1) + 64) * 4);
	a.off_round = o;    o += al256(((size_t)(max_len >> 1) + 64) * 4);
	a.stride = al256(o);
	return a.stride;
}
static int size_arena(DsbSlotArena &a, int *cur_slots, uint32_t max_len, int want_slots, int min_slots, uint32_t sms_cap, uint32_t anc_cap, uint32_t hit_cap,
                      int extra_slots, size_t budget, bool exact_cap = false, bool check_only = false, int *cur_extra = nullptr)
{
	const int have_extra = cur_extra ? *cur_extra : extra_slots;
	const bool fits = a.base && a.max_len >= max_len && (exact_cap ? a.sms_cap == sms_cap : a.sms_cap >= sms_cap) && have_extra >= extra_slots;
	const bool oversized = a.base && a.max_len > 4 * (uint64_t)max_len + 65536 && a.stride * ((size_t)*cur_slots + have_extra) > ((size_t)4 << 30);
	if (fits && !oversized && (*cur_slots >= want_slots || a.max_len > max_len)) return 0;
	if (check_only) return 1;
	if (g_upload_trace) fprintf(stderr, "[upload] an arena is (re)built: has max_len %u, %d + %d slots, sms_cap %u; wanted max_len %u, %d + %d slots, sms_cap %u%s\n", a.base ? a.max_len : 0u, *cur_slots, have_extra, a.base ? a.sms_cap : 0u, max_len, want_slots, extra_slots, sms_cap, oversized ? " (oversized)" : "");
	if (a.base && !oversized && a.max_len > max_len) max_len = a.max_len;
	if (a.base) { hipFree(a.base); a.base = nullptr; budget += a.stride * ((size_t)*cur_slots + have_extra); }
	DsbSlotArena n = a;
	const size_t stride = arena_layout(n, max_len, 64, sms_cap, anc_cap, hit_cap);
	int slots = want_slots;
	while (slots > min_slots && stride * ((size_t)slots + extra_slots) > budget) slots = slots * 3 / 4 > min_slots ? slots * 3 / 4 : min_slots;
	while (cur_extra && extra_slots > 0 && stride * ((size_t)slots + extra_slots) > budget) extra_slots /= 2;
	for (;;) {
		if (hipMalloc((void **)&n.base, stride * ((size_t)slots + extra_slots)) == hipSuccess) break;
		(void)hipGetLastError();
		n.base = nullptr;
		if (slots <= min_slots && !(cur_extra && extra_slots > 0)) { a.base = nullptr; *cur_slots = 0; if (cur_extra) *cur_extra = 0; return DSB_ENOMEM; }
		if (slots > min_slots) slots = slots / 2 > min_slots ? slots / 2 : min_slots; else extra_slots /= 2;
	}
	a = n; *cur_slots = slots; if (cur_extra) *cur_extra = extra_slots;
	return 0;
}

static int ensure_buffers(dsb_ctx *c, size_t n, uint32_t max_len, uint64_t bin_bytes, uint64_t pk_words, uint64_t bit_words, uint64_t seed_entries)
{
	int rc;
	if ((rc = grow(&c->d_seeds, &c->cap_seeds, (size_t)seed_entries + 64))) return rc;
	if ((rc = grow(&c->d_sinfo, &c->cap_sinfo, n + 1))) return rc;
	if ((rc = grow(&c->d_wd, &c->cap_wd, (size_t)bit_words + 1))) return rc;
	if ((rc = grow(&c->d_bin, &c->cap_bin, (size_t)bin_bytes + 256))) return rc;
	if ((rc = grow(&c->d_pk, &c->cap_pk, (size_t)pk_words + 8))) return rc;
	if ((rc = grow(&c->d_bits, &c->cap_bits, (size_t)bit_words + 8))) return rc;
	if ((rc = grow(&c->d_rout, &c->cap_rout, n + 1))) return rc;
	size_t want_hout = 16 * n + 4096;
	if (c->knobs.hout_cap) want_hout = (size_t)c->knobs.hout_cap;
	if (c->cap_hout < want_hout || c->knobs.hout_cap) {
		if (c->cap_hout != want_hout) { if (c->d_hout) hipFree(c->d_hout); c->d_hout = nullptr; c->cap_hout = 0; if (hipMalloc((void **)&c->d_hout, want_hout * sizeof(DsbHitOut)) != hipSuccess) return DSB_ENOMEM; c->cap_hout = want_hout; }
	}
	if ((rc = grow(&c->d_score, &c->cap_score, n + 1))) return rc;
	if ((rc = grow(&c->d_heavy, &c->cap_heavy, n + 1))) return rc;
	if ((rc = grow(&c->d_order, &c->cap_order, n + 1))) return rc;
	if (c->knobs.anchor_kernel) {
		if ((rc = grow(&c->d_arec, &c->cap_arec, n + 1))) return rc;
		uint64_t pool = (uint64_t)bin_bytes / 128 + 64 * (uint64_t)n;
		if (c->knobs.anc_pool_rt) pool = (uint64_t)c->knobs.anc_pool_rt;
		if (pool > 0xffffffffu) pool = 0xffffffffu;
		if (c->cap_apool < pool || c->knobs.anc_pool_rt) {
			if (c->cap_apool != pool) { hipFree(c->d_apool); c->d_apool = nullptr; c->cap_apool = 0; if (hipMalloc((void **)&c->d_apool, pool * sizeof(DsbAnchor)) != hipSuccess) return DSB_ENOMEM; c->cap_apool = pool; }
		}
	}
	int want = c->opts.n_slots > 0 ? c->opts.n_slots : 256 * 4 * DSB_WAVES_PER_EU;
	if ((size_t)want > n) want = (int)(n ? n : 1);
	if (want < c->n_slots) want = c->n_slots;
	int want_anc = 256 * 4 * DSB_ANCHOR_WPE;
	if ((size_t)want_anc > n) want_anc = (int)(n ? n : 1);
	if (want_anc < c->n_slots_anc) want_anc = c->n_slots_anc;
	if (max_len < c->hint_len) max_len = c->hint_len;
	if (c->arena.base && max_len > c->arena.max_len) { const uint64_t g = (uint64_t)max_len + max_len / 4; max_len = g > 0xfffffff0ull ? 0xfffffff0u : (uint32_t)g; }
	uint32_t cap1 = dsb_sms_cap_for(max_len);
	const bool cap_forced = c->knobs.sms_cap != 0;
	if (cap_forced) cap1 = (uint32_t)c->knobs.sms_cap;
	uint64_t cap2 = (uint64_t)cap1 * DSB_RETRY_GROW; if (cap2 > DSB_RETRY_MAX_NODES) cap2 = cap1 > DSB_RETRY_MAX_NODES ? cap1 : DSB_RETRY_MAX_NODES;
	uint32_t anc1 = DSB_ANC_CAP;
	if (c->knobs.anc_cap_rt) anc1 = (uint32_t)c->knobs.anc_cap_rt;
	const bool exact = cap_forced || c->knobs.anc_cap_rt;
	int want_extra = (n >= 4096 || c->knobs.heavy_first_set) ? DSB_HEAVY_SLOTS : 0;
	if (want_extra < c->n_extra) want_extra = c->n_extra;
	for (int pass = 0; pass < 2; pass++) {
		size_t budget_big = 0, budget_main = 0, budget_anc = 0;
		if (pass) {
			size_t free_b = 0, total_b = 0;
			if (hipMemGetInfo(&free_b, &total_b) != hipSuccess) { free_b = (size_t)64 << 30; }
			const size_t reserve = (size_t)2 << 30;
			budget_big = free_b > reserve ? (free_b - reserve) / 4 : 0; budget_main = free_b > reserve ? (free_b - reserve) / 2 : 0;
			budget_anc = free_b > reserve ? (free_b - reserve) / 8 : 0;
		}
		const int r1 = size_arena(c->arena_big, &c->n_slots_big, max_len, DSB_RETRY_SLOTS, 4, (uint32_t)cap2, DSB_RETRY_ANC, DSB_RETRY_HIT, 0, budget_big, false, pass == 0);
		const int r2 = size_arena(c->arena, &c->n_slots, max_len, want, 64 < want ? 64 : want, cap1, anc1, DSB_HIT_CAP, want_extra, budget_main, exact, pass == 0, &c->n_extra);
		if (c->knobs.anchor_kernel && c->arena_anc.base && c->arena_anc.anc_cap != anc1) { hipFree(c->arena_anc.base); c->arena_anc.base = nullptr; c->n_slots_anc = 0; }
		const int r3 = c->knobs.anchor_kernel ? size_arena(c->arena_anc, &c->n_slots_anc, max_len, want_anc, 64 < want_anc ? 64 : want_anc, 0u, anc1, 0u, 0, budget_anc, false, pass == 0) : 0;
		if (r1 == 1 || r2 == 1 || r3 == 1) continue;
		if (r1) return r1;
		if (r2) return r2;
		if (r3) return r3;
		break;
	}
	return DSB_OK;
}

#include <atomic>
#include <time.h>
static size_t upload_chunk(dsb_ctx *c)
{
	if (!c->up_chunk) c->up_chunk = c->knobs.upload_chunk_kb > 0 ? (size_t)c->knobs.upload_chunk_kb << 10 : (size_t)8 << 20;
	return c->up_chunk;
}
static int upload_threads(const dsb_ctx *c)
{
	int T = dsb_host_cpus() / 2; if (T > 16) T = 16;
	if (c->knobs.upload_threads) T = c->knobs.upload_threads;
	return T < 1 ? 1 : T;
}
static int upload_stages(dsb_ctx *c, int T)
{
	const size_t CB = upload_chunk(c);
	while (c->up.size() < (size_t)T) {
		UpStage u;
		for (int k = 0; k < 2; k++) { u.buf[k] = (char *)dsb_host_alloc(CB); if (!u.buf[k] || hipEventCreateWithFlags(&u.ev[k], hipEventDisableTiming) != hipSuccess) { for (int j = 0; j <= k; j++) { if (u.buf[j]) hipHostFree(u.buf[j]); if (u.ev[j]) hipEventDestroy(u.ev[j]); } return DSB_ENOMEM; } }
		if (hipStreamCreateWithFlags(&u.st, hipStreamNonBlocking) != hipSuccess) { for (int k = 0; k < 2; k++) { hipHostFree(u.buf[k]); hipEventDestroy(u.ev[k]); } return DSB_ENODEV; }
		c->up.push_back(u);
	}
	return DSB_OK;
}
static const uint8_t *pack_lut(void)
{
	static uint8_t *lut = nullptr; static std::once_flag once;
	std::call_once(once, [] {
		uint8_t one[256];
		for (int ch = 0; ch < 256; ch++) one[ch] = (ch == 'A' || ch == 'a') ? 0 : (ch == 'G' || ch == 'g') ? 2 : (ch == 'T' || ch == 't') ? 3 : 1;
		uint8_t *t = (uint8_t *)malloc(65536);
		for (int v = 0; v < 65536; v++) t[v] = (uint8_t)(one[v & 255] << 2 | one[v >> 8]);
		lut = t;
	});
	return lut;
}
static void pack_bases(uint8_t *dst, const char *src, uint64_t b0, uint64_t nb, uint32_t len)
{
	const uint8_t *lut = pack_lut(); const uint8_t *p = (const uint8_t *)src + b0;
	uint64_t full = b0 + 4 * nb <= len ? nb : (len > b0 ? (len - b0) / 4 : 0);
	for (uint64_t k = 0; k < full; k++, p += 4) { uint16_t a, b; memcpy(&a, p, 2); memcpy(&b, p + 2, 2); dst[k] = (uint8_t)(lut[a] << 4 | lut[b]); }
	for (uint64_t k = full; k < nb; k++) {
		uint32_t v = 0;
		for (int j = 0; j < 4; j++) { const uint64_t bi = b0 + 4 * k + j; const uint8_t ch = bi < len ? (uint8_t)src[bi] : (uint8_t)'A'; v = v << 2 | (uint32_t)(lut[ch] >> 2); }
		dst[k] = (uint8_t)v;
	}
}
static int upload_gather(dsb_ctx *c, InSlot &s, const SeqView *reads, size_t n, uint64_t total)
{
	if (!total) return DSB_OK;
	const bool packed = s.packed;
	const size_t CB = upload_chunk(c), n_chunks = (size_t)((total + CB - 1) / CB);
	int T = upload_threads(c);
	if ((size_t)T > n_chunks) T = (int)n_chunks;
	if (T < 1) T = 1;
	if (int rc = upload_stages(c, T)) return rc;
	std::atomic<size_t> next(0); std::atomic<int> err(0);
	const DsbReadDesc *rd = s.h_rd.data();
	const bool trace = c->knobs.upload_trace;
	std::vector<double> t_wait(T, 0.0), t_copy(T, 0.0), t_sub(T, 0.0);
	auto clk = [] { struct timespec ts; clock_gettime(CLOCK_MONOTONIC, &ts); return ts.tv_sec + 1e-9 * ts.tv_nsec; };
	const double t_begin = clk();
	auto work = [&](int t) {
		if (hipSetDevice(c->device) != hipSuccess) { err = 1; return; }
		UpStage &u = c->up[t]; int par = 0;
		for (;;) {
			const size_t ch = next.fetch_add(1);
			if (ch >= n_chunks || err.load()) break;
			const double w0 = trace ? clk() : 0;
			if (u.used[par] && hipEventSynchronize(u.ev[par]) != hipSuccess) { err = 1; break; }
			const double w1 = trace ? clk() : 0;
			const uint64_t lo = (uint64_t)ch * CB, hi = lo + CB < total ? lo + CB : total;
			size_t a = 0, b = n;
			auto ext = [&](size_t m) { return packed ? ((uint64_t)rd[m].len + 3) / 4 : (uint64_t)rd[m].len; };
			while (a < b) { const size_t m = (a + b) / 2; if (rd[m].seq_off + ext(m) > lo) b = m; else a = m + 1; }
			char *dst = u.buf[par];
			for (size_t i = a; i < n && rd[i].seq_off < hi; i++) {
				const uint64_t p = rd[i].seq_off > lo ? rd[i].seq_off : lo, q = rd[i].seq_off + ext(i) < hi ? rd[i].seq_off + ext(i) : hi;
				if (q <= p) continue;
				if (packed) pack_bases((uint8_t *)dst + (p - lo), reads[i].p, 4 * (p - rd[i].seq_off), q - p, rd[i].len);
				else memcpy(dst + (p - lo), reads[i].p + (p - rd[i].seq_off), (size_t)(q - p));
			}
			const double w2 = trace ? clk() : 0;
			if (hipMemcpyAsync(s.d_ascii + lo, dst, (size_t)(hi - lo), hipMemcpyHostToDevice, u.st) != hipSuccess || hipEventRecord(u.ev[par], u.st) != hipSuccess) { err = 1; break; }
			if (trace) { const double w3 = clk(); t_wait[t] += w1 - w0; t_copy[t] += w2 - w1; t_sub[t] += w3 - w2; }
			u.used[par] = true; par ^= 1;
		}
		const double w0 = trace ? clk() : 0;
		if (hipStreamSynchronize(u.st) != hipSuccess) err = 1;
		if (trace) t_wait[t] += clk() - w0;
		u.used[0] = u.used[1] = false;
	};
	std::vector<std::thread> th;
	for (int t = 1; t < T; t++) th.emplace_back(work, t);
	work(0);
	for (std::thread &x : th) x.join();
	if (trace) {
		double a = 0, b = 0, d = 0; for (int t = 0; t < T; t++) { a += t_wait[t]; b += t_copy[t]; d += t_sub[t]; }
		fprintf(stderr, "[upload] %.2f GB%s in %zu chunks on %d threads: %.3f s wall = %.1f GB/s; per thread: gather %.3f s, waiting for a chunk's transfer %.3f s, submitting %.3f s\n", total / 1e9, packed ? " (2 bits per base: bases / 4)" : " of text", n_chunks, T,
		        clk() - t_begin, total / 1e9 / (clk() - t_begin), b / T, a / T, d / T);
	}
	if (err.load()) { fprintf(stderr, "[desamba_amd] HIP error %s in upload_gather\n", hipGetErrorString(hipGetLastError())); return DSB_ENODEV; }
	return DSB_OK;
}
static int upload_views(dsb_ctx *c, const SeqView *reads, size_t n, const char *ext_text, size_t ext_len, const uint64_t *ext_off)
{
	if (!c || (!reads && n)) return DSB_EINVAL;
	HIPCHK(hipSetDevice(c->device));
	InSlot &s = c->in[c->cur];
	const int k = c->dx.ek_len;
	s.h_rd.resize(n);
	uint64_t seq_off = 0, bin_off = 0, pk_off = 0, bit_off = 0, windows = 0, seed_off = 0, blob_off = 0; uint32_t max_len = 64, min_len = 0xffffffffu; int hist = c->hist_max;
	s.packed = !ext_text && !c->knobs.upload_text;
	for (size_t i = 0; i < n; i++) {
		DsbReadDesc &d = s.h_rd[i];
		d.len = reads[i].len; d.seq_off = ext_text ? ext_off[i] : (s.packed ? blob_off : seq_off); d.bin_off = bin_off; d.pk_off = pk_off; d.bit_off = bit_off;
		blob_off += ((uint64_t)d.len + 3) / 4;
		d.n_win = d.len >= 40 ? d.len - k + 1 : 0; d.n_words = (d.n_win + 63) / 64;
		d.hist_max = hist; if ((int)d.len > hist) hist = d.len;
		d.seed_off = seed_off; seed_off += ((uint64_t)d.len >> 1) + 64;
		if (d.len < min_len) min_len = d.len;
		seq_off += d.len; bin_off += al256(DSB_QPAD_L + 2 * (size_t)d.len + DSB_QPAD_R);
		pk_off += 2 * ((d.len + 31) / 32 + 1); bit_off += 2 * (size_t)d.n_words;
		if (d.len > max_len) max_len = d.len;
		windows += 2 * (uint64_t)d.n_win;
	}
	c->hist_max = hist;
	s.n_reads = n; s.n_words_total = bit_off; s.total_bases = seq_off; s.total_windows = windows; s.max_len = max_len; s.seed_entries = seed_off;
	s.min_len = n ? min_len : 0; s.ragged = n && (uint64_t)max_len > (uint64_t)min_len + (min_len >> 3) + 64;
	s.upload_bytes = ext_text ? ext_len : (s.packed ? blob_off : seq_off);
	int rc;
	const bool utrace = c->knobs.upload_trace;
	auto uclk = [] { struct timespec ts; clock_gettime(CLOCK_MONOTONIC, &ts); return ts.tv_sec + 1e-9 * ts.tv_nsec; };
	const double u0 = utrace ? uclk() : 0;
	if ((rc = grow(&s.d_rd, &s.cap_rd, n + 1))) return rc;
	if ((rc = grow(&s.d_ascii, &s.cap_ascii, (ext_text ? ext_len : (size_t)(s.packed ? blob_off : seq_off)) + 64))) return rc;
	if ((rc = ensure_buffers(c, n, max_len, bin_off, pk_off, bit_off, seed_off))) return rc;
	if (utrace) fprintf(stderr, "[upload] %zu reads, longest %u, %.2f Gbases: descriptors %.3f s on the host, device buffers checked / grown in %.3f s%s\n", n, max_len, seq_off / 1e9, 0.0, uclk() - u0, s.ragged ? " (ragged: reads sorted by length for the seed scan)" : "");
	if (n) {
		HIPCHK(hipMemcpyAsync(s.d_rd, s.h_rd.data(), n * sizeof(DsbReadDesc), hipMemcpyHostToDevice, c->stream));
		if (s.ragged) {
			std::vector<uint32_t> ord(n);
			for (size_t i = 0; i < n; i++) ord[i] = (uint32_t)i;
			std::stable_sort(ord.begin(), ord.end(), [&](uint32_t a, uint32_t b) { return s.h_rd[a].len > s.h_rd[b].len; });
			if ((rc = grow(&s.d_scan_order, &s.cap_scan_order, n + 1))) return rc;
			HIPCHK(hipMemcpy(s.d_scan_order, ord.data(), n * 4, hipMemcpyHostToDevice));
		}
		if (ext_text) HIPCHK(hipMemcpyAsync(s.d_ascii, ext_text, ext_len, hipMemcpyHostToDevice, c->stream));
		else {
			if ((rc = upload_gather(c, s, reads, n, s.packed ? blob_off : seq_off))) return rc;
		}
	}
	HIPCHK(hipStreamSynchronize(c->stream));
	return DSB_OK;
}

extern "C" int dsb_batch_upload(dsb_ctx *c, const dsb_read *reads, size_t n)
{
	if (!c || (!reads && n)) return DSB_EINVAL;
	std::vector<SeqView> v(n);
	for (size_t i = 0; i < n; i++) { v[i].p = reads[i].seq; v[i].len = reads[i].len; }
	return upload_views(c, v.data(), n);
}

extern "C" int dsb_batch_upload_text(dsb_ctx *c, const char *text, size_t text_len, const uint64_t *seq_off, const uint32_t *seq_len, size_t n)
{
	if (!c || ((!text || !seq_off || !seq_len) && n)) return DSB_EINVAL;
	std::vector<SeqView> v(n);
	for (size_t i = 0; i < n; i++) { if (seq_off[i] > text_len || seq_len[i] > text_len - seq_off[i]) return DSB_EINVAL; v[i].p = text + seq_off[i]; v[i].len = seq_len[i]; }
	return upload_views(c, v.data(), n, text, text_len, seq_off);
}

#include "dsb_fastq_scan.h"
extern "C" long dsb_batch_upload_fastq(dsb_ctx *c, const char *path, size_t skip, size_t max_reads)
{
	if (!c || !path) return DSB_EINVAL;
	int fd = open(path, O_RDONLY);
	if (fd < 0) return DSB_EIO;
	struct stat st; if (fstat(fd, &st) != 0) { close(fd); return DSB_EIO; }
	size_t sz = (size_t)st.st_size;
	char *b = sz ? (char *)mmap(nullptr, sz, PROT_READ | PROT_WRITE, MAP_PRIVATE, fd, 0) : nullptr;
	close(fd);
	if (sz && b == MAP_FAILED) return DSB_EIO;
	std::vector<SeqView> v;
	size_t pos = 0, rec = 0; int last = 0; dsb_rec_t r;
	while (v.size() < max_reads) {
		int rc = dsb_scan_record(b, pos, sz, 1, last, 0, &r);
		if (rc == 1 && !r.plain) rc = dsb_scan_record(b, pos, sz, 1, last, 1, &r);
		if (rc == -2) { pos = r.next; last = r.next_last; continue; }
		if (rc != 1) break;
		pos = r.next; last = r.next_last;
		if (rec++ < skip) continue;
		if (r.seq_len > 0xffffffffu) { if (b) munmap(b, sz); return DSB_EINVAL; }
		SeqView sv; sv.p = b + r.seq_off; sv.len = (uint32_t)r.seq_len;
		v.push_back(sv);
	}
	int rc = upload_views(c, v.data(), v.size());
	if (b) munmap(b, sz);
	return rc ? rc : (long)v.size();
}

#define DSB_GROUP_MAX_LEN 400u
template <class K>
static void launch_classify(K kern, dsb_ctx *c, hipStream_t st, unsigned grid, const DsbDevIndex &dx, const InSlot &s, uint32_t n_fixed, const unsigned int *n_ptr,
                            const uint32_t *list, const DsbSlotArena &ar, unsigned int *work_counter, uint32_t *dbg, uint32_t item_base, uint32_t slot_base, int cnt_set,
                            bool pre_seeds, const DsbAncRec *arec = nullptr, const DsbAnchor *apool = nullptr)
{
	hipLaunchKernelGGL(kern, dim3(grid), dim3(64), 0, st, dx, (const DsbReadDesc *)s.d_rd, n_fixed, n_ptr, list, c->d_bin, (const uint64_t *)c->d_bits, ar, work_counter,
	                   c->d_rout, c->d_hout, c->d_counters + 1, (uint32_t)c->cap_hout, dbg, item_base, slot_base, (unsigned long long *)(c->d_counters + 16 + 8 * cnt_set),
	                   pre_seeds ? c->d_seeds : nullptr, (const DsbSeedInfo *)c->d_sinfo, (const uint64_t *)c->d_pk, (uint32_t)((pre_seeds && s.max_len <= DSB_GROUP_MAX_LEN && !c->knobs.no_group) ? (c->knobs.group_head >= 0 ? (unsigned)c->knobs.group_head : 8u * grid) : 0u), arec, apool);
}

static int batch_run_locked(dsb_ctx *c, std::unique_lock<std::mutex> *turn);
extern "C" int dsb_batch_run(dsb_ctx *c)
{
	if (!c) return DSB_EINVAL;
	if (c->staged && !c->knobs.no_turn) { std::unique_lock<std::mutex> g(c->staged->run_mu); return batch_run_locked(c, &g); }
	return batch_run_locked(c, nullptr);
}
static int batch_run_locked(dsb_ctx *c, std::unique_lock<std::mutex> *turn)
{
	HIPCHK(hipSetDevice(c->device));
	InSlot &s = c->in[c->cur];
	size_t n = s.n_reads;
	memset(&c->timing, 0, sizeof c->timing);
	c->timing.upload_bytes = s.upload_bytes;
	c->taxa.run = c->taxa.tx != nullptr && n == 0; c->taxa.done = false;
	c->lca.run = c->lca.d_direct != nullptr && n == 0; c->lca.done = false;
	if (n == 0) return DSB_OK;
	HIPCHK(hipMemsetAsync(c->d_counters, 0, 256, c->stream));
	HIPCHK(hipEventRecord(c->ev[0], c->stream));
	if (s.packed) hipLaunchKernelGGL(k_encode_bytes_pk, dim3((unsigned)n), dim3(256), 0, c->stream, s.d_rd, (const uint8_t *)s.d_ascii, c->d_bin);
	else hipLaunchKernelGGL(k_encode_bytes, dim3((unsigned)n), dim3(256), 0, c->stream, s.d_rd, s.d_ascii, c->d_bin);
	hipLaunchKernelGGL(k_encode_pack, dim3((unsigned)n), dim3(256), 0, c->stream, s.d_rd, c->d_bin, c->d_pk);
	HIPCHK(hipEventRecord(c->ev[1], c->stream));
	const bool dbg = c->knobs.debug && c->dbg_dev;
	if (dbg) { HIPCHK(hipStreamSynchronize(c->stream)); fprintf(stderr, "[dsb] encode done\n"); }
	hipLaunchKernelGGL(k_repeat_score, dim3((unsigned)n), dim3(256), 0, c->stream, s.d_rd, c->d_pk, c->d_score);
	hipLaunchKernelGGL(k_order, dim3(1), dim3(1024), 0, c->stream, c->d_score, (uint32_t)n, c->d_order);
	if (const char *of = c->knobs.order_file.empty() ? nullptr : c->knobs.order_file.c_str()) {
		std::vector<uint32_t> ord(n); FILE *f = fopen(of, "rb");
		if (f && fread(ord.data(), 4, n, f) == n) HIPCHK(hipMemcpyAsync(c->d_order, ord.data(), n * 4, hipMemcpyHostToDevice, c->stream));
		if (f) fclose(f);
		HIPCHK(hipStreamSynchronize(c->stream));
	}
	HIPCHK(hipEventRecord(c->ev_order, c->stream));
	unsigned n_heavy = 0;
	if (!dbg && s.n_words_total && !c->seed_only) {
		n_heavy = c->knobs.heavy_first_set ? (unsigned)c->knobs.heavy_first : (n >= 4096 ? (unsigned)(n / 64) : 0u);
		if (n_heavy > (unsigned)c->n_extra) n_heavy = (unsigned)c->n_extra;
		if (n_heavy > n / 2) n_heavy = (unsigned)(n / 2);
	}
	c->n_early = n_heavy;
	bool use_scan = n >= 2048;
	if (c->knobs.seed_scan >= 0) use_scan = c->knobs.seed_scan != 0;
	c->bits_valid = !use_scan; c->seeds_valid = use_scan;
	uint32_t step_limit = DSB_STEP_LIMIT;
	if (c->knobs.step_limit_rt > 0) step_limit = (uint32_t)c->knobs.step_limit_rt;
	DsbDevIndex dx1 = c->dx; dx1.sms_cap = c->arena.sms_cap; dx1.step_limit = step_limit;
	dx1.heavy_limit = DSB_HEAVY_PREDS;
	if (dbg) dx1.heavy_limit = 0;
	if (c->knobs.heavy_preds_set) dx1.heavy_limit = c->knobs.heavy_preds;
	if (n_heavy) {
		hipLaunchKernelGGL(k_seed_probe_reads, dim3(n_heavy * DSB_HPROBE_SPLIT), dim3(256), 0, c->stream, c->dx, (const DsbReadDesc *)s.d_rd, (const uint32_t *)c->d_order, c->d_pk, c->d_bits, c->d_summ, c->summ_shift);
		HIPCHK(hipEventRecord(c->ev_hprobe, c->stream));
		HIPCHK(hipEventRecord(c->ev_order, c->stream));
		unsigned n_mw = c->mw_reads;
		if (c->knobs.heavy_mw >= 0) n_mw = (unsigned)c->knobs.heavy_mw;
		if (n_mw > n_heavy) n_mw = n_heavy;
		c->timing.n_heavy_mw = n_mw;
		if (n_mw) {
			HIPCHK(hipStreamWaitEvent(c->stream3, c->ev_hprobe, 0));
			hipLaunchKernelGGL(k_classify_heavy<8>, dim3(n_mw), dim3(64 * 8), 0, c->stream3, dx1, (const DsbReadDesc *)s.d_rd, (uint32_t)n_mw, (const unsigned int *)nullptr, (const uint32_t *)c->d_order, c->d_bin,
			                   (const uint64_t *)c->d_bits, c->arena, c->d_counters + 10, c->d_rout, c->d_hout, c->d_counters + 1, (uint32_t)c->cap_hout, (uint32_t)c->n_slots,
			                   (unsigned long long *)(c->d_counters + 16 + 8), (const uint64_t *)c->d_pk, (DsbSeed *)nullptr, (const DsbSeedInfo *)c->d_sinfo);
			HIPCHK(hipEventRecord(c->ev_heavy3, c->stream3));
		}
		HIPCHK(hipStreamWaitEvent(c->stream2, c->ev_hprobe, 0));
		if (n_heavy > n_mw)
			launch_classify(k_classify_early, c, c->stream2, n_heavy - n_mw, dx1, s, (uint32_t)n_heavy, nullptr, (const uint32_t *)c->d_order, c->arena, c->d_counters + 4, nullptr, n_mw, (uint32_t)c->n_slots + n_mw, 1, false);
		HIPCHK(hipEventRecord(c->ev_heavy, c->stream2));
	}
	if (use_scan) {
		hipLaunchKernelGGL(k_seed_scan, dim3((unsigned)((2 * n + 255) / 256)), dim3(256), 0, c->stream, c->dx, (const DsbReadDesc *)s.d_rd, (const uint32_t *)(s.ragged ? s.d_scan_order : nullptr),
		                   (uint32_t)n, (const uint64_t *)c->d_pk, c->d_seeds, c->d_sinfo, (const uint8_t *)c->d_summ, c->summ_shift, (unsigned long long *)(c->d_counters + 40),
		                   c->knobs.scan_look_set ? c->knobs.scan_look : dsb_scan_look_for((c->dx.ek_mask + 1) / 8, c->ek_dense));
	} else if (s.n_words_total) {
		uint64_t waves = (s.n_words_total + DSB_PROBE_UN - 1) / DSB_PROBE_UN; unsigned blocks = (unsigned)((waves + 3) / 4);
		if (blocks > 256u * 32u) blocks = 256u * 32u;
		hipLaunchKernelGGL(k_build_wd, dim3((unsigned)n), dim3(256), 0, c->stream, s.d_rd, c->d_wd);
		hipLaunchKernelGGL(k_seed_probe, dim3(blocks), dim3(256), 0, c->stream, c->dx, (const DsbReadDesc *)s.d_rd, (const DsbWordDesc *)c->d_wd, s.n_words_total, c->d_pk, c->d_bits,
		                   (unsigned long long *)(c->d_counters + 2), c->d_summ, c->summ_shift);
	}
	HIPCHK(hipEventRecord(c->ev[2], c->stream));
	if (c->seed_only) {
		HIPCHK(hipStreamSynchronize(c->stream));
		hipEventElapsedTime(&c->timing.encode_ms, c->ev[0], c->ev[1]);
		hipEventElapsedTime(&c->timing.order_ms, c->ev[1], c->ev_order);
		hipEventElapsedTime(&c->timing.seed_probe_ms, c->ev_order, c->ev[2]);
		unsigned long long pc[2] = {0, 0};
		HIPCHK(hipMemcpy(pc, use_scan ? c->d_counters + 40 : c->d_counters + 2, use_scan ? 16 : 8, hipMemcpyDeviceToHost));
		c->timing.windows = use_scan ? pc[0] : s.total_windows; c->timing.probes_t1 = use_scan ? pc[1] : pc[0]; c->timing.bases = s.total_bases;
		c->timing.seed_scan = use_scan ? 1 : 0; c->timing.total_ms = c->timing.encode_ms + c->timing.order_ms + c->timing.seed_probe_ms;
		return DSB_OK;
	}
	if (dbg) { HIPCHK(hipStreamSynchronize(c->stream)); fprintf(stderr, "[dsb] seed probe done\n"); }
	unsigned slots = (unsigned)c->n_slots; if (slots > n - n_heavy) slots = (unsigned)(n - n_heavy);
	{
		uint32_t *dbgp = dbg ? c->dbg_dev : nullptr;
		if (dbg) memset(c->dbg_host, 0, 32 * 65536 * sizeof(uint32_t));
		const bool grp = s.max_len <= DSB_GROUP_MAX_LEN && !c->knobs.no_group;
		const bool anc_k = use_scan && !dbg && !grp && c->knobs.anchor_kernel && c->arena_anc.base && c->n_slots_anc > 0 && c->arena_anc.anc_cap == c->arena.anc_cap
		                   && c->d_arec && c->cap_arec >= n && c->d_apool && n > n_heavy;
		if (anc_k) {
			unsigned ga = (unsigned)c->n_slots_anc; if (ga > n - n_heavy) ga = (unsigned)(n - n_heavy);
			hipLaunchKernelGGL(k_anchor, dim3(ga), dim3(64), 0, c->stream, dx1, (const DsbReadDesc *)s.d_rd, (uint32_t)n, (uint32_t)n_heavy, (const uint32_t *)c->d_order, c->d_bin, c->arena_anc,
			                   c->d_counters + 14, c->d_seeds, (const DsbSeedInfo *)c->d_sinfo, c->d_arec, c->d_apool, c->d_counters + 15, (uint32_t)c->cap_apool, (unsigned long long *)(c->d_counters + 16));
		}
		launch_classify(k_classify, c, c->stream, slots, dx1, s, (uint32_t)n, nullptr, (const uint32_t *)c->d_order, c->arena, c->d_counters, dbgp, (uint32_t)n_heavy, 0u, 0, use_scan,
		                anc_k ? c->d_arec : nullptr, anc_k ? c->d_apool : nullptr);
		HIPCHK(hipEventRecord(c->ev_cls, c->stream));
		HIPCHK(hipEventRecord(c->ev_cls_wait, c->stream));
		if (n_heavy) { HIPCHK(hipStreamWaitEvent(c->stream, c->ev_heavy, 0)); if (c->timing.n_heavy_mw) HIPCHK(hipStreamWaitEvent(c->stream, c->ev_heavy3, 0)); }
		if (dbg) {
			for (int sec = 0; sec < 60; sec++) {
				if (hipStreamQuery(c->stream) == hipSuccess) break;
				usleep(1000000);
				if (sec % 5 == 4) {
					fprintf(stderr, "[dsb] classify still running after %d s; slot: code steps read\n", sec + 1);
					for (unsigned sI = 0; sI < slots && sI < 24; sI++) fprintf(stderr, "   slot %u: %u %u %u\n", sI, c->dbg_host[4 * sI], c->dbg_host[4 * sI + 1], c->dbg_host[4 * sI + 2]);
				}
			}
		}
	}
	if (dx1.heavy_limit) {
		DsbDevIndex dxh = dx1; dxh.heavy_limit = 0;
		unsigned gh = (unsigned)(c->n_slots + c->n_extra); if (gh > 256u) gh = 256u;
		hipLaunchKernelGGL(k_collect_retry, dim3((unsigned)((n + 255) / 256)), dim3(256), 0, c->stream, (const DsbReadOut *)c->d_rout, (uint32_t)n, c->d_heavy, c->d_counters + 12, DSB_ST_HEAVY, 0);
		hipLaunchKernelGGL(k_classify_heavy<8>, dim3(gh), dim3(64 * 8), 0, c->stream, dxh, (const DsbReadDesc *)s.d_rd, 0u, (const unsigned int *)(c->d_counters + 12), (const uint32_t *)c->d_heavy, c->d_bin,
		                   (const uint64_t *)c->d_bits, c->arena, c->d_counters + 13, c->d_rout, c->d_hout, c->d_counters + 1, (uint32_t)c->cap_hout, 0u,
		                   (unsigned long long *)(c->d_counters + 16 + 8), (const uint64_t *)c->d_pk, use_scan ? c->d_seeds : (DsbSeed *)nullptr, (const DsbSeedInfo *)c->d_sinfo);
	}
	DsbDevIndex dx2 = c->dx; dx2.sms_cap = c->arena_big.sms_cap; dx2.heavy_limit = 0; dx2.step_limit = step_limit > 0xffffffffu / 16 ? 0xffffffffu : step_limit * 16u;
	const int retry_mask = DSB_ST_SMS_OVF | DSB_ST_ANC_OVF | DSB_ST_HIT_OVF | DSB_ST_TIMEOUT;
	hipLaunchKernelGGL(k_collect_retry, dim3((unsigned)((n + 255) / 256)), dim3(256), 0, c->stream, (const DsbReadOut *)c->d_rout, (uint32_t)n, c->d_score, c->d_counters + 6, retry_mask, 0);
	launch_classify(k_classify_second, c, c->stream, (unsigned)c->n_slots_big, dx2, s, 0u, (const unsigned int *)(c->d_counters + 6), (const uint32_t *)c->d_score, c->arena_big, c->d_counters + 7, nullptr, 0u, 0u, 2, use_scan);
	HIPCHK(hipEventRecord(c->ev[3], c->stream));
	if (turn && !c->knobs.turn_whole_run) { HIPCHK(hipEventSynchronize(c->ev_cls_wait)); turn->unlock(); }
	HIPCHK(hipEventSynchronize(c->ev[3]));
	{
		unsigned int cnt[2] = {0, 0};
		HIPCHK(hipMemcpy(cnt, c->d_counters, 8, hipMemcpyDeviceToHost));
		if (cnt[1] > c->cap_hout) {
			const size_t new_cap = 2 * (size_t)cnt[1] + 4096;
			DsbHitOut *nh = nullptr;
			if (hipMalloc((void **)&nh, new_cap * sizeof(DsbHitOut)) != hipSuccess) return DSB_ENOMEM;
			HIPCHK(hipMemcpy(nh, c->d_hout, c->cap_hout * sizeof(DsbHitOut), hipMemcpyDeviceToDevice));
			hipFree(c->d_hout); c->d_hout = nh; c->cap_hout = new_cap;
			hipLaunchKernelGGL(k_collect_retry, dim3((unsigned)((n + 255) / 256)), dim3(256), 0, c->stream, (const DsbReadOut *)c->d_rout, (uint32_t)n, c->d_score, c->d_counters + 8, DSB_ST_OUT_OVF, 0);
			launch_classify(k_classify_second, c, c->stream, (unsigned)c->n_slots_big, dx2, s, 0u, (const unsigned int *)(c->d_counters + 8), (const uint32_t *)c->d_score, c->arena_big, c->d_counters + 9, nullptr, 0u, 0u, 2, use_scan);
			HIPCHK(hipStreamSynchronize(c->stream));
			unsigned int n3 = 0; HIPCHK(hipMemcpy(&n3, c->d_counters + 8, 4, hipMemcpyDeviceToHost));
			c->timing.n_regrow = n3;
		}
	}
	const DsbBatchView hits = {c->stream, c->d_rout, c->d_hout, c->d_counters, c->cap_hout, s.d_rd, (uint32_t)n};
	if (int rc = reductions_run(c, hits)) return rc;
	if (dbg) {
		static const char *nm[10] = {"seed_vector", "fast_classify", "resolve_tree", "slow+resolve", "hash_build", "sdp_middle", "sdp_right", "sdp_left", "sort/filter", "primary"};
		double tot[10] = {0}, all = 0; unsigned sl = (unsigned)c->n_slots; if (sl > n) sl = (unsigned)n;
		double sub[4] = {0};
		for (unsigned sI = 0; sI < sl; sI++) { for (int i = 0; i < 10; i++) { tot[i] += c->dbg_host[4 * 65536 + 14 * sI + i]; all += c->dbg_host[4 * 65536 + 14 * sI + i]; } for (int i = 0; i < 4; i++) sub[i] += c->dbg_host[4 * 65536 + 14 * sI + 10 + i]; }
		fprintf(stderr, "[dsb] inside sdp_right (ms, -DDSB_TIMERS builds): sdp_match %.1f  dp %.1f  combine %.1f | fast_classify commit phase %.1f\n", sub[0] / 1e3, sub[1] / 1e3, sub[2] / 1e3, sub[3] / 1e3);
		{ double tx[10] = {0}; for (unsigned sI = 0; sI < sl; sI++) for (int i = 0; i < 10; i++) tx[i] += c->dbg_host[8 * 65536 + 10 * sI + i];
		  fprintf(stderr, "[dsb] fine (ms, -DDSB_TIMERS builds): table build %.1f  probe %.1f  block DP: old predecessors %.1f, inside the block %.1f  sdp_match in sdp_left %.1f  dp in sdp_left %.1f  gap-per-lane phase of sdp_middle %.1f | of the old predecessors: beyond the first 64 (sdp_batch_old) %.1f in %.0f blocks; rounds over the first 64: %.0f\n",
		          tx[0] / 1e3, tx[1] / 1e3, tx[2] / 1e3, tx[6] / 100.0 / 1e3, tx[3] / 1e3, tx[4] / 1e3, tx[5] / 1e3, tx[9] / 100.0 / 1e3, tx[7], tx[8]); }
		{
			size_t worst = 0; uint64_t wsum = 0;
			for (size_t r = 0; r < n && r < 65536; r++) { uint64_t sm = 0; for (int i = 0; i < 10; i++) sm += c->dbg_host[16 * 65536 + 14 * r + i]; if (sm > wsum) { wsum = sm; worst = r; } }
			fprintf(stderr, "[dsb] slowest read %zu: %.1f ms:", worst, wsum / 1e3);
			for (int i = 0; i < 10; i++) fprintf(stderr, " %s %.1f", nm[i], c->dbg_host[16 * 65536 + 14 * worst + i] / 1e3);
			fprintf(stderr, " | in right/left: sdp_match %.1f dp %.1f combine %.1f\n", c->dbg_host[16 * 65536 + 14 * worst + 10] / 1e3, c->dbg_host[16 * 65536 + 14 * worst + 11] / 1e3, c->dbg_host[16 * 65536 + 14 * worst + 12] / 1e3);
		}
		fprintf(stderr, "[dsb] classify stage time (wave-seconds, %% of total %.2f s):", all / 1e6);
		for (int i = 0; i < 10; i++) fprintf(stderr, " %s %.1f%%", nm[i], 100.0 * tot[i] / (all > 0 ? all : 1));
		fprintf(stderr, "\n");
	}
	HIPCHK(hipGetLastError());
	hipEventElapsedTime(&c->timing.encode_ms, c->ev[0], c->ev[1]);
	hipEventElapsedTime(&c->timing.order_ms, c->ev[1], c->ev_order);
	hipEventElapsedTime(&c->timing.seed_probe_ms, c->ev_order, c->ev[2]);
	hipEventElapsedTime(&c->timing.classify_ms, c->ev[2], c->ev_cls);
	hipEventElapsedTime(&c->timing.tail_ms, c->ev_cls, c->ev[3]);
	c->timing.n_early = c->n_early;
	hipEventElapsedTime(&c->timing.total_ms, c->ev[0], c->ev[3]);
	unsigned long long wk[12] = {0};
	HIPCHK(hipMemcpy(&c->p1, c->d_counters + 2, 8, hipMemcpyDeviceToHost));
	HIPCHK(hipMemcpy(&c->timing.n_retry, c->d_counters + 6, 4, hipMemcpyDeviceToHost));
	{
		unsigned int h[4] = {0, 0, 0, 0};
		HIPCHK(hipMemcpy(h, c->d_counters + 12, sizeof h, hipMemcpyDeviceToHost));
		c->timing.n_requeue = h[0]; c->timing.anc_pool_asked = h[3]; c->timing.anc_pool_cap = c->cap_apool;
	}
	if (c->timing.tail_ms > 3.0f && c->timing.n_requeue == 0 && c->timing.n_retry == 0 && c->timing.n_early) {
		if (c->mw_reads < 64) c->mw_reads = c->mw_reads ? c->mw_reads * 2 : 16;
		c->mw_grown = true; c->mw_calm = 0;
	} else if (c->timing.tail_ms < 0.5f && !c->mw_grown && c->mw_reads && c->timing.n_early && ++c->mw_calm >= 4) c->mw_reads = 0;
	HIPCHK(hipMemcpy(wk, c->d_counters + 16, 96, hipMemcpyDeviceToHost));
	c->timing.windows = s.total_windows; c->timing.probes_t1 = c->p1; c->timing.bases = s.total_bases;
	c->timing.seed_scan = use_scan ? 1 : 0;
	if (use_scan) {
		unsigned long long pc[2] = {0, 0};
		HIPCHK(hipMemcpy(pc, c->d_counters + 40, 16, hipMemcpyDeviceToHost));
		c->timing.windows = pc[0]; c->timing.probes_t1 = pc[1];
	}
	c->timing.n_occ = wk[0] + wk[4] + wk[8]; c->timing.n_mem = wk[1] + wk[5] + wk[9]; c->timing.n_sa = wk[2] + wk[6] + wk[10]; c->timing.ref_bases = wk[3] + wk[7] + wk[11];
	c->timing.main_occ = wk[0]; c->timing.main_mem = wk[1]; c->timing.main_sa = wk[2]; c->timing.main_ref_bases = wk[3];
	return DSB_OK;
}

extern "C" int dsb_batch_fetch(dsb_ctx *c, dsb_result *out)
{
	if (!c || !out) return DSB_EINVAL;
	HIPCHK(hipSetDevice(c->device));
	const size_t n = c->in[c->cur].n_reads;
	c->h_rout.resize(n); c->res_reads.resize(n);
	unsigned int cnt[2] = {0, 0};
	if (n) {
		HIPCHK(hipMemcpyAsync(cnt, c->d_counters, 8, hipMemcpyDeviceToHost, c->stream));
		HIPCHK(hipMemcpyAsync(c->h_rout.data(), c->d_rout, n * sizeof(DsbReadOut), hipMemcpyDeviceToHost, c->stream));
		HIPCHK(hipStreamSynchronize(c->stream));
	}
	const size_t nh = dsb_hits_out(cnt[1], c->cap_hout);
	c->h_hout.resize(nh);
	if (nh) HIPCHK(hipMemcpyAsync(c->h_hout.data(), c->d_hout, nh * sizeof(DsbHitOut), hipMemcpyDeviceToHost, c->stream));
	static_assert(sizeof(DsbHitOut) == sizeof(dsb_hit), "dsb_hit mirrors DsbHitOut");
	int worst = DSB_OK;
	for (size_t i = 0; i < n; i++) {
		const DsbReadOut &r = c->h_rout[i];
		dsb_read_result &o = c->res_reads[i];
		o.first = r.first; o.n = r.n; o.fast = r.fast & 1u; o.device_us = r.fast >> 1; o.n_anc = r.n_anc;
		o.status = r.status ? (DSB_ECAP * 256 - r.status) : 0;
		if (r.status) worst = DSB_ECAP;
		if (dsb_hits_cut(r.first, r.n, nh)) { o.n = 0; o.first = 0; }
	}
	if (int rc = reductions_fetch(c, n, nh != 0)) return rc;
	out->reads = c->res_reads.data(); out->hits = reinterpret_cast<const dsb_hit *>(c->h_hout.data()); out->n_hits = nh;
	return worst;
}

extern "C" int dsb_classify_batch(dsb_ctx *c, const dsb_read *reads, size_t n, dsb_result *out)
{
	int rc;
	if ((rc = dsb_batch_upload(c, reads, n))) return rc;
	if ((rc = dsb_batch_run(c))) return rc;
	return dsb_batch_fetch(c, out);
}

extern "C" int dsb_batch_timing(const dsb_ctx *c, dsb_timing *t) { if (!c || !t) return DSB_EINVAL; *t = c->timing; return DSB_OK; }

extern "C" int dsb_batch_exist_bits(dsb_ctx *c, size_t read, int strand, uint8_t *out, size_t cap, uint32_t *n_out)
{
	if (!c || read >= c->in[c->cur].n_reads) return DSB_EINVAL;
	HIPCHK(hipSetDevice(c->device));
	const InSlot &sl = c->in[c->cur];
	const DsbReadDesc &d = sl.h_rd[read];
	if (n_out) *n_out = d.n_win;
	if (cap < d.n_win) return DSB_EINVAL;
	if (!c->bits_valid && sl.n_words_total) {
		uint64_t waves = (sl.n_words_total + DSB_PROBE_UN - 1) / DSB_PROBE_UN; unsigned blocks = (unsigned)((waves + 3) / 4);
		if (blocks > 256u * 32u) blocks = 256u * 32u;
		hipLaunchKernelGGL(k_build_wd, dim3((unsigned)sl.n_reads), dim3(256), 0, c->stream, sl.d_rd, c->d_wd);
		hipLaunchKernelGGL(k_seed_probe, dim3(blocks), dim3(256), 0, c->stream, c->dx, (const DsbReadDesc *)sl.d_rd, (const DsbWordDesc *)c->d_wd, sl.n_words_total, c->d_pk, c->d_bits,
		                   (unsigned long long *)nullptr, c->d_summ, c->summ_shift);
		HIPCHK(hipStreamSynchronize(c->stream));
		c->bits_valid = true;
	}
	std::vector<uint64_t> wv(d.n_words);
	if (d.n_words) HIPCHK(hipMemcpy(wv.data(), c->d_bits + d.bit_off + (strand ? 0 : d.n_words), d.n_words * 8, hipMemcpyDeviceToHost));
	for (uint32_t i = 0; i < d.n_win; i++) out[i] = (uint8_t)((wv[i >> 6] >> (i & 63)) & 1);
	return DSB_OK;
}

__global__ void __launch_bounds__(64) k_seed_dump(DsbDevIndex x, DsbReadDesc d, uint8_t *bin, const uint64_t *bits, int strand, DsbSeed *out, uint32_t *n_out)
{
	__shared__ DsbDevIndex sx;
	__shared__ uint32_t lds_cnt[4];
	if (threadIdx.x == 0) sx = x;
	__syncthreads();
	__shared__ dsb_g64::WCtx s_w;
	dsb_g64::WCtxL &w = *(dsb_g64::WCtxL *)&s_w;
	w.x = (dsb_g64::DsbXP)&sx; w.L = d.len; w.status = 0; w.dbg = nullptr; w.anc_cap = 0; w.wtab = nullptr;
	w.k.c = (dsb_g64::lds_u32 *)lds_cnt; w.k.uni = 1; w.pre_seeds = nullptr; w.pre_info = nullptr; w.pk[0] = w.pk[1] = nullptr; w.mw = nullptr; w.n_waves = 1;
	dsb_g64::SDirL *sd = w.sd;
	uint32_t n = d.len - x.ek_len + 1;
	if (strand) dsb_g64::seed_vector(w, bin + d.bin_off + DSB_QPAD_L, bits + d.bit_off, n, out, D_FORWARD, sd);
	else dsb_g64::seed_vector(w, bin + d.bin_off + DSB_QPAD_L + d.len, bits + d.bit_off + d.n_words, n, out, D_REVERSE, sd);
	if (threadIdx.x == 0) { n_out[0] = sd->l_seed_v; n_out[1] = sd->total_score; }
}
extern "C" int dsb_batch_seeds(dsb_ctx *c, size_t read, int strand, dsb_seed *out, size_t cap, uint32_t *n, uint32_t *total_score)
{
	if (!c || read >= c->in[c->cur].n_reads) return DSB_EINVAL;
	HIPCHK(hipSetDevice(c->device));
	const DsbReadDesc &d = c->in[c->cur].h_rd[read];
	if (d.len < 40) { if (n) *n = 0; if (total_score) *total_score = 0; return DSB_OK; }
	if (c->seeds_valid) {
		DsbSeedInfo si; HIPCHK(hipMemcpy(&si, c->d_sinfo + read, sizeof si, hipMemcpyDeviceToHost));
		const int dir = strand ? 0 : 1; const uint32_t cnt = si.n_seed[dir];
		std::vector<DsbSeed> hs(cnt ? cnt : 1);
		if (cnt) HIPCHK(hipMemcpy(hs.data(), c->d_seeds + d.seed_off + (dir ? (d.len >> 2) : 0), cnt * sizeof(DsbSeed), hipMemcpyDeviceToHost));
		if (n) *n = cnt; if (total_score) *total_score = si.total[dir];
		if (cap < cnt) return DSB_EINVAL;
		for (uint32_t i = 0; i < cnt; i++) { out[i].offset = hs[i].offset; out[i].len = hs[i].len; out[i].top = (uint8_t)hs[i].top; out[i].pad[0] = out[i].pad[1] = out[i].pad[2] = 0; }
		return DSB_OK;
	}
	DsbSeed *ds; uint32_t *dn; size_t m = (d.len >> 1) + 64;
	HIPCHK(hipMalloc((void **)&ds, m * sizeof(DsbSeed))); HIPCHK(hipMalloc((void **)&dn, 8));
	hipLaunchKernelGGL(k_seed_dump, dim3(1), dim3(64), 0, c->stream, c->dx, d, c->d_bin, c->d_bits, strand, ds, dn);
	HIPCHK(hipStreamSynchronize(c->stream));
	uint32_t hn[2]; HIPCHK(hipMemcpy(hn, dn, 8, hipMemcpyDeviceToHost));
	std::vector<DsbSeed> hs(hn[0] ? hn[0] : 1);
	if (hn[0]) HIPCHK(hipMemcpy(hs.data(), ds, hn[0] * sizeof(DsbSeed), hipMemcpyDeviceToHost));
	hipFree(ds); hipFree(dn);
	if (n) *n = hn[0]; if (total_score) *total_score = hn[1];
	if (cap < hn[0]) return DSB_EINVAL;
	for (uint32_t i = 0; i < hn[0]; i++) { out[i].offset = hs[i].offset; out[i].len = hs[i].len; out[i].top = (uint8_t)hs[i].top; out[i].pad[0] = out[i].pad[1] = out[i].pad[2] = 0; }
	return DSB_OK;
}

extern "C" int dsb_shard_plan(const uint32_t *lengths, size_t n, int world, uint64_t chunk_bases, uint32_t chunk_reads, dsb_chunk *out, size_t cap, size_t *n_out)
{
	if ((!lengths && n) || world < 1 || !n_out) return DSB_EINVAL;
	if (!chunk_bases) chunk_bases = 64000000ULL;
	if (!chunk_reads) chunk_reads = 4096;
	size_t k = 0, start = 0; uint64_t bases = 0; uint32_t hist = 0, run_max = 0;
	for (size_t i = 0; i < n; i++) {
		bases += lengths[i];
		if (lengths[i] > run_max) run_max = lengths[i];
		if (bases >= chunk_bases || i + 1 - start >= chunk_reads || i + 1 == n) {
			if (out && k < cap) { out[k].start = start; out[k].end = i + 1; out[k].hist_max_before = hist; out[k].rank = (int32_t)(k % (size_t)world); }
			k++;
			if (run_max > hist) hist = run_max;
			start = i + 1; bases = 0;
		}
	}
	*n_out = k;
	return (out && k > cap) ? DSB_EINVAL : DSB_OK;
}

extern "C" void dsb_multi_destroy(dsb_multi *m)
{
	if (!m) return;
	for (dsb_ctx *c : m->ctx) dsb_ctx_destroy(c);
	delete m;
}
extern "C" int dsb_ctx_create_multi(dsb_index *idx, const int *device_ids, int n_dev, const dsb_opts *opts, dsb_multi **out)
{
	if (!idx || !device_ids || n_dev < 1 || !out) return DSB_EINVAL;
	dsb_multi *m = new dsb_multi(); m->idx = idx;
	if (const char *cr = getenv("DSB_SHARD_CHUNK_READS")) m->chunk_reads_env = (uint32_t)atol(cr);
	for (int i = 0; i < n_dev; i++) {
		dsb_ctx *c = nullptr; int rc = dsb_ctx_create(idx, device_ids[i], opts, &c);
		if (rc) { dsb_multi_destroy(m); return rc; }
		m->ctx.push_back(c);
	}
	*out = m;
	return DSB_OK;
}
extern "C" int dsb_multi_n(const dsb_multi *m) { return m ? (int)m->ctx.size() : 0; }
extern "C" dsb_ctx *dsb_multi_ctx(dsb_multi *m, int i) { return (m && i >= 0 && (size_t)i < m->ctx.size()) ? m->ctx[i] : nullptr; }
extern "C" void dsb_multi_reset_history(dsb_multi *m) { if (m) m->hist = 0; }
extern "C" uint32_t dsb_multi_last_calls(const dsb_multi *m, int i) { return (m && i >= 0 && (size_t)i < m->last_calls.size()) ? m->last_calls[(size_t)i] : 0; }

extern "C" int dsb_multi_classify_batch(dsb_multi *m, const dsb_read *reads, size_t n, dsb_result *out)
{
	if (!m || (!reads && n) || !out) return DSB_EINVAL;
	const int W = (int)m->ctx.size();
	std::vector<uint32_t> len(n);
	for (size_t i = 0; i < n; i++) len[i] = reads[i].len;
	uint32_t chunk_reads = m->chunk_reads_env; uint64_t chunk_bases = 4000000000ULL;
	if (!chunk_reads) {
		uint64_t want = (n + (size_t)W - 1) / (size_t)W; if (want < 32768) want = 32768;
		const dsb_opts &o = m->ctx[0]->opts;
		if (o.max_batch_reads && want > o.max_batch_reads) want = o.max_batch_reads;
		if (o.max_batch_bases) chunk_bases = o.max_batch_bases;
		chunk_reads = want > 0xffffffffULL ? 0xffffffffu : (uint32_t)want;
	}
	size_t nc = 0;
	dsb_shard_plan(len.data(), n, W, chunk_bases, chunk_reads, nullptr, 0, &nc);
	std::vector<dsb_chunk> plan(nc ? nc : 1);
	dsb_shard_plan(len.data(), n, W, chunk_bases, chunk_reads, plan.data(), nc, &nc);
	m->reads.assign(n, dsb_read_result());
	m->taxa_ok = false; if (m->tx) m->taxa.assign(n, dsb_read_taxon());
	m->lca_ok = false; if (m->lca_on) m->lca.assign(n, dsb_read_lca());
	std::vector<std::vector<dsb_hit>> chunk_hits(nc);
	std::vector<int> rcs(W, DSB_OK);
	const uint32_t hist0 = m->hist;
	std::atomic<size_t> next_chunk(0);
	m->last_calls.assign((size_t)W, 0);
	auto worker = [&](int w) {
		dsb_ctx *c = m->ctx[w];
		for (;;) {
			const size_t k = next_chunk.fetch_add(1);
			if (k >= nc) break;
			const dsb_chunk &ch = plan[k];
			dsb_ctx_set_history(c, ch.hist_max_before > hist0 ? ch.hist_max_before : hist0);
			dsb_result r;
			int rc = dsb_classify_batch(c, reads + ch.start, (size_t)(ch.end - ch.start), &r);
			m->last_calls[(size_t)w]++;
// ... 41 lines not shown
```

desamba_amd/csrc/dsb_index.cpp:

```cpp
#include <stdio.h>
#include <stdlib.h>
#include <string.h>
#include <math.h>
#include <thread>
#include <sched.h>
#include <vector>
#include "dsb_host.h"
#include "dsb_sam_fields.h"

struct dsb_index { DsbHostIndex h; };

const DsbHostIndex *dsb_index_host(const dsb_index *idx) { return &idx->h; }

static FILE *open_ext(const char *dir, const char *ext)
{
	char path[4096];
	snprintf(path, sizeof path, "%s/deSAMBA%s", dir, ext);
	FILE *f = fopen(path, "rb");
	if (!f) fprintf(stderr, "[desamba_amd] cannot open %s\n", path);
	return f;
}
extern "C" int dsb_host_cpus(void)
{
	static int cached = 0;
// ... 102 lines not shown
	if (!h.sa || !rd(h.sa, sizeof(DsbHostSa), h.sa_size, f)) FAIL(DSB_EIO);
	fclose(f); f = NULL;
	if (!(f = open_ext(dir, ".exki"))) FAIL(DSB_EIO);
	if (!rd(&h.ek_size, 8, 1, f)) FAIL(DSB_EIO);
	fclose(f); f = NULL;
	int bits = 37, k = 20;
	switch (h.ek_size) {
	case 1ULL << 27: bits = 30; k = 16; break;
	case 1ULL << 28: bits = 31; k = 17; break;
	case 1ULL << 29: bits = 32; k = 17; break;
	case 1ULL << 30: bits = 33; k = 18; break;
	case 1ULL << 31: bits = 34; k = 18; break;
	case 1ULL << 32: bits = 35; k = 19; break;
	case 1ULL << 33: bits = 36; k = 19; break;
	case 1ULL << 34: bits = 37; k = 20; break;
	}
	h.ek_mask = (1ULL << bits) - 1; h.ek_len = k;
	h.single_base_max = (int)(0.8 * k);
	h.ek0 = (uint8_t *)malloc(h.ek_size); h.ek1 = (uint8_t *)malloc(h.ek_size);
	if (!h.ek0 || !h.ek1) FAIL(DSB_ENOMEM);
	if (!(f = open_ext(dir, ".exk0"))) FAIL(DSB_EIO);
	if (!rd(h.ek0, 1, h.ek_size, f)) FAIL(DSB_EIO);
	fclose(f); f = NULL;
	if (!(f = open_ext(dir, ".exk1"))) FAIL(DSB_EIO);
	if (!rd(h.ek1, 1, h.ek_size, f)) FAIL(DSB_EIO);
	fclose(f); f = NULL;
	if (!(f = open_ext(dir, ".unv"))) FAIL(DSB_EIO);
	if (!rd(&h.n_uni, 8, 1, f)) FAIL(DSB_EIO);
	h.uni = (DsbHostUni *)malloc((h.n_uni + 2) * sizeof(DsbHostUni));
	if (!h.uni || !rd(h.uni, sizeof(DsbHostUni), h.n_uni, f)) FAIL(DSB_EIO);
	h.uni[h.n_uni].ref_list = h.uni[h.n_uni - 1].ref_list + 1 + h.uni[h.n_uni - 1].length;
	h.uni[h.n_uni].length = 0;
	h.dollar_pos = h.n_uni - 1 - 1;
	fclose(f); f = NULL;
	if (!(f = open_ext(dir, ".ref_b"))) FAIL(DSB_EIO);
	if (!rd(&h.n_refbin, 8, 1, f)) FAIL(DSB_EIO);
	h.refbin = (uint8_t *)calloc(h.n_refbin + 4096, 1);
	if (!h.refbin || !rd(h.refbin, 1, h.n_refbin, f)) FAIL(DSB_EIO);
	fclose(f); f = NULL;
	if (!(f = open_ext(dir, ".ref_i"))) FAIL(DSB_EIO);
	if (!rd(&h.n_ref, 8, 1, f)) FAIL(DSB_EIO);
	h.refdisk = (DsbHostRefInfoDisk *)malloc(h.n_ref * sizeof(DsbHostRefInfoDisk));
	h.refinfo = (DsbRefInfo *)malloc(h.n_ref * sizeof(DsbRefInfo));
	if (!h.refdisk || !h.refinfo || !rd(h.refdisk, sizeof(DsbHostRefInfoDisk), h.n_ref, f)) FAIL(DSB_EIO);
	for (uint64_t i = 0; i < h.n_ref; i++) { h.refdisk[i].name[127] = 0; h.refinfo[i].seq_l = h.refdisk[i].seq_l; h.refinfo[i].seq_offset = h.refdisk[i].seq_offset; }
	fclose(f); f = NULL;
	if (!(f = open_ext(dir, ".ref_p"))) FAIL(DSB_EIO);
	if (!rd(&h.n_refpos, 8, 1, f)) FAIL(DSB_EIO);
	h.refpos = (uint64_t *)calloc(h.n_refpos + 2, 8);
	if (!h.refpos || !rd(h.refpos, 8, h.n_refpos, f)) FAIL(DSB_EIO);
	fclose(f); f = NULL;
	double P_E = 0.15; uint64_t L_REF = h.n_refbin * 4;
	double REF_SIZE_PUNALTY = -10 * log(L_REF) / log(10);
	double MATCH_SCORE = -10 * log(0.25 / (1 - P_E)) / log(10);
	double MISMATCH_PUNALTY = -10 * log(0.75 / (P_E)) / log(10);
	for (int i = 0; i < 2000; i++) h.Q_MEM[i] = REF_SIZE_PUNALTY + i * MATCH_SCORE + 0.5;
	for (int j = 0; j < 20; j++)
		for (int i = 0; i < 20; i++) {
			h.Q_LV[i][j] = (j - i) * MATCH_SCORE + i * MISMATCH_PUNALTY + 0.5;
			if (j < 5) h.Q_LV[i][j] += 15;
			if (h.Q_LV[i][j] < -8) h.Q_LV[i][j] = -8;
		}
	*out = x;
	return DSB_OK;
}

extern "C" void dsb_index_close(dsb_index *x)
{
	if (!x) return;
	DsbHostIndex &h = x->h;
	free(h.ek0); free(h.ek1); free(h.fm); free(h.fm_sb); free(h.hash_index); free(h.hash_c); free(h.sa); free(h.uni); free(h.refpos); free(h.refbin); free(h.refdisk); free(h.refinfo);
	free(x);
}
extern "C" uint64_t dsb_index_n_ref(const dsb_index *x) { return x ? x->h.n_ref : 0; }
extern "C" const char *dsb_index_ref_name(const dsb_index *x, uint32_t id) { return (x && id < x->h.n_ref) ? x->h.refdisk[id].name : "*"; }
extern "C" uint64_t dsb_index_ref_len(const dsb_index *x, uint32_t id) { return (x && id < x->h.n_ref) ? x->h.refdisk[id].seq_l : 0; }
extern "C" int dsb_index_ek_len(const dsb_index *x) { return x ? x->h.ek_len : 0; }

extern "C" int dsb_index_prefix_interval(const dsb_index *x, uint32_t p, int form, uint64_t *sp, uint64_t *ep)
{
	const DsbHostIndex &h = x->h;
	if (p >= (1u << 26)) return DSB_EINVAL;
	if (form == 0) { *sp = h.hash_index[p]; *ep = h.hash_index[p + 1]; return 0; }
	if (!h.hash_c) return -1;
	const uint32_t ln = DSB_HI_DIV29(p), sl = p - ln * DSB_HI_PER_LINE;
	*sp = (uint64_t)h.hash_c[ln].base + h.hash_c[ln].off[sl]; *ep = (uint64_t)h.hash_c[ln].base + h.hash_c[ln].off[sl + 1];
	return 0;
}

extern "C" uint64_t dsb_index_occ_host(const dsb_index *x, uint64_t r, uint8_t *cp)
{
	const DsbHostIndex &h = x->h;
	const DsbFmBlock &b = h.fm[r >> 7];
	uint32_t off = (uint32_t)r & 127u; uint32_t c = *cp;
	if (c == 0xffu) {
		uint32_t w = off >> 6, bi = off & 63u;
		uint32_t s = (b.sp[w] >> bi) & 1, q0 = (b.p0[w] >> bi) & 1, q1 = (b.p1[w] >> bi) & 1;
		c = s ? (4u + q0) : (q0 | (q1 << 1));
		*cp = (uint8_t)c;
		if (c == 5u) return h.dollar_pos;
	}
	uint64_t m0 = off >= 64u ? ~0ULL : ((1ULL << off) - 1ULL);
	uint64_t m1 = off > 64u ? ((1ULL << (off - 64u)) - 1ULL) : 0ULL;
	if (c < 4u) {
		uint64_t e0 = ~b.sp[0] & ((c & 1u) ? b.p0[0] : ~b.p0[0]) & ((c & 2u) ? b.p1[0] : ~b.p1[0]) & m0;
		uint64_t e1 = ~b.sp[1] & ((c & 1u) ? b.p0[1] : ~b.p0[1]) & ((c & 2u) ? b.p1[1] : ~b.p1[1]) & m1;
		return (uint64_t)b.cnt[c] + (h.fm_sb ? h.fm_sb[(r >> 22) * 5 + c] : 0) + __builtin_popcountll(e0) + __builtin_popcountll(e1);
	}
	uint64_t blk0 = (r >> 7) << 7;
	uint64_t base = blk0 - ((uint64_t)b.cnt[0] + b.cnt[1] + b.cnt[2] + b.cnt[3] + (h.fm_sb ? h.fm_sb[(r >> 22) * 5 + 4] : 0)) - (h.dollar_row < blk0 ? 1u : 0u);
	return base + __builtin_popcountll(b.sp[0] & ~b.p0[0] & m0) + __builtin_popcountll(b.sp[1] & ~b.p0[1] & m1);
}

extern "C" long dsb_format_sam(const dsb_index *x, const dsb_read *rd_, const dsb_hit *h, uint32_t n, int max_sec, int full, char *buf, size_t cap)
{
	const char *seq_s = full ? rd_->seq : "*", *qual_s = full ? (rd_->qual ? rd_->qual : "(null)") : "*";
	int seq_n = full ? (int)rd_->len : 1, qual_n = full ? (int)(rd_->qual ? rd_->len : 6) : 1;
	size_t o = 0; int w;
#define EMIT(...) do { w = snprintf(buf + o, cap > o ? cap - o : 0, __VA_ARGS__); if (w < 0 || (size_t)w >= (cap > o ? cap - o : 0)) return -1; o += (size_t)w; } while (0)
	if (n == 0) { EMIT("%s\t4\t*\t0\t0\t*\t*\t0\t0\t%.*s\t%.*s\t\n", rd_->name, seq_n, seq_s, qual_n, qual_s); return (long)o; }
	uint32_t read_l = rd_->len;
	int flag = h[0].direction ? 0 : 0x10, mapQ_PRI = dsb_sam_mapq_pri(h, n), cg[3];
	dsb_sam_cigar(h, read_l, cg);
	EMIT("%s\t%d\t%s\t%d\t%d\t%dS%dM%dS\t*\t0\t0\t%.*s\t%.*s\tAS:i:%d\t\n", rd_->name, flag, dsb_index_ref_name(x, h[0].ref_ID),
	     h[0].t_st, mapQ_PRI, cg[0], cg[1], cg[2], seq_n, seq_s, qual_n, qual_s, h[0].sum_score);
	for (int loop = 0; loop <= 1; loop++)
		for (uint32_t i = 1; i < n; i++) {
			const dsb_hit *c = h + i;
			int show = dsb_sam_shown(c, loop, max_sec), fl = c->direction ? 0 : 0x10, mapQ = 0;
			if (show && loop == 0) { fl += 0x800; mapQ = dsb_sam_mapq_sup(mapQ_PRI); }
			else if (show) fl += 0x100;
			if (show) {
				dsb_sam_cigar(c, read_l, cg);
				EMIT("%s\t%d\t%s\t%d\t%d\t%d%c%dM%d%c\t*\t0\t0\t*\t*\tAS:i:%d\t\n", rd_->name, fl, dsb_index_ref_name(x, c->ref_ID), c->t_st, mapQ,
				     cg[0], loop == 0 ? 'H' : 'S', cg[1], cg[2], loop == 0 ? 'H' : 'S', c->sum_score);
			}
		}
#undef EMIT
	return (long)o;
}

extern "C" const char *dsb_strerror(int code)
{
	switch (code) {
	case DSB_OK: return "ok";
	case DSB_EIO: return "index file missing or short";
	case DSB_ENODEV: return "no gfx950 device / HIP runtime error (there is no CPU path)";
	case DSB_ENOMEM: return "out of memory";
	case DSB_EINVAL: return "invalid argument";
	case DSB_ECAP: return "a per-read device arena overflowed";
	}
	return "unknown error";
}
extern "C" const char *dsb_version(void) { return "desamba_amd 0.5 (gfx950)"; }

extern "C" long dsb_format_des(const dsb_index *x, const dsb_read *rd_, const dsb_read_result *rr, const dsb_hit *h, int max_sec, int full, char *buf, size_t cap)
{
	static const char *primary_string[3] = {"PRI", "SEC", "SUP"};
	size_t o = 0; int w;
#define EMIT(...) do { w = snprintf(buf + o, cap > o ? cap - o : 0, __VA_ARGS__); if (w < 0 || (size_t)w >= (cap > o ? cap - o : 0)) return -1; o += (size_t)w; } while (0)
	EMIT("%s\t%s\t%s\t%ld\tn_rst:[%ld]\tn_anc:[%ld]\t\n", rd_->name, rr->n ? "CLASSIFY" : "UNCLASSIFY", rr->fast ? "FAST" : "SLOW", (long)rd_->len, (long)rr->n, (long)rr->n_anc);
	int rst_cnt = 0;
	for (int loop = 0; loop <= 1; loop++)
		for (uint32_t i = 0; i < rr->n; i++) {
			const dsb_hit *c = h + i;
			bool show = loop == 0 ? c->pri_index == 0 : (c->pri_index > 0 && (full || c->pri_index <= max_sec));
			if (!show) continue;
			unsigned ps = (unsigned)(c->primary - 1); if (ps > 2) ps = 2;
			EMIT("%3d %s %s %20s ts:%-10d te:%-10d qs:%-10d qe:%-10d %-5d\t%d\t\n", rst_cnt++, primary_string[ps], c->direction ? "F" : "R",
			     dsb_index_ref_name(x, c->ref_ID), (int)c->t_st, (int)c->t_ed, (int)c->q_st, (int)c->q_ed, (int)c->sum_score, (int)c->indel);
		}
	EMIT("\n");
#undef EMIT
	return (long)o;
}

extern "C" long dsb_coverage_format(const dsb_index *x, const dsb_ref_coverage *cov, char *buf, size_t cap)
{
	if (!x || !cov || (!buf && cap)) return -1;
	size_t o = 0; int w;
#define EMIT(...) do { w = snprintf(buf + o, cap > o ? cap - o : 0, __VA_ARGS__); if (w < 0 || (size_t)w >= (cap > o ? cap - o : 0)) return -1; o += (size_t)w; } while (0)
	EMIT("#rname\tstartpos\tendpos\tnumreads\tcovbases\tcoverage\tmeandepth\tmeanmapq\n");
	const uint64_t n_ref = dsb_index_n_ref(x);
	for (uint64_t r = 0; r < n_ref; r++) {
		const dsb_ref_coverage &c = cov[r];
		if (!c.numreads) continue;
		const uint64_t ln = dsb_index_ref_len(x, (uint32_t)r);
		const double L = ln ? (double)ln : 1.0;
		EMIT("%s\t1\t%llu\t%llu\t%llu\t%g\t%g\t%.1f\n", dsb_index_ref_name(x, (uint32_t)r), (unsigned long long)ln, (unsigned long long)c.numreads,
		     (unsigned long long)c.covbases, 100.0 * (double)c.covbases / L, (double)c.aligned_bases / L, (double)c.mapq_sum / (double)c.numreads);
	}
#undef EMIT
	return (long)o;
}
```

include/desamba_amd.h:

```cpp
#ifndef DESAMBA_AMD_H
#define DESAMBA_AMD_H
#include <stddef.h>
#include <stdint.h>

#ifdef __cplusplus
extern "C" {
#endif

#define DSB_OK        0
#define DSB_EIO      -1
#define DSB_ENODEV   -2
#define DSB_ENOMEM   -3
#define DSB_EINVAL   -4
#define DSB_ECAP     -5

typedef struct dsb_index dsb_index;
typedef struct dsb_ctx dsb_ctx;
typedef struct dsb_multi dsb_multi;

typedef struct {
	int L_min_matching;
	int min_score;
	int max_sec_N;
	int n_slots;
	uint32_t max_read_len;
	uint32_t max_batch_reads;
	int input_slots;
	int reserved;
	uint64_t max_batch_bases;
} dsb_opts;

typedef struct {
	const char *name;
	const char *seq;
	const char *qual;
	uint32_t len;
} dsb_read;

typedef struct {
	uint32_t ref_ID, t_st, t_ed, q_st, q_ed, sum_score, indel;
	uint8_t direction, primary, pri_index, pad;
} dsb_hit;

typedef struct {
	uint32_t first, n;
	int32_t status;
	uint32_t fast;
	uint32_t device_us;
	uint32_t n_anc;
} dsb_read_result;

typedef struct {
	const dsb_read_result *reads;
	const dsb_hit *hits;
	size_t n_hits;
} dsb_result;

typedef struct { uint32_t offset, len; uint8_t top; uint8_t pad[3]; } dsb_seed;

typedef struct {
	float encode_ms, seed_probe_ms, classify_ms, total_ms;
	uint64_t windows;
	uint64_t probes_t1;
	uint64_t bases;
	float order_ms;
	float tail_ms;
	uint32_t n_early;
	uint32_t n_retry;
	uint32_t n_regrow;
	uint32_t seed_scan;
	uint64_t n_occ;
	uint64_t n_mem;
	uint64_t n_sa;
	uint64_t ref_bases;
	uint64_t main_occ, main_mem, main_sa, main_ref_bases;
	uint32_t n_heavy_mw;
	uint32_t n_requeue;
	uint64_t upload_bytes;
	uint64_t anc_pool_asked;
	uint64_t anc_pool_cap;
} dsb_timing;

typedef struct {
	uint64_t n_bases, n_refs, n_kmer, n_unitig, n_rows;
	double parse_s, sort_s, graph_s, walk_s, rows_s, tables_s, write_s, total_s;
	uint64_t budget_bytes;
	uint64_t peak_device_bytes;
	uint32_t ranges_kmers, ranges_unitig_numbers, ranges_rows, ranges_exist;
	uint64_t spilled_bytes;
} dsb_build_stats;
int  dsb_index_build(const char *kmer_srt, const char *fasta, const char *out_dir, int device, dsb_build_stats *stats);

int  dsb_index_open(const char *dir, dsb_index **idx);
void dsb_index_close(dsb_index *idx);
uint64_t    dsb_index_n_ref(const dsb_index *idx);
const char *dsb_index_ref_name(const dsb_index *idx, uint32_t ref_ID);
uint64_t    dsb_index_ref_len(const dsb_index *idx, uint32_t ref_ID);
int         dsb_index_ek_len(const dsb_index *idx);
int dsb_index_prefix_interval(const dsb_index *idx, uint32_t prefix, int form, uint64_t *sp, uint64_t *ep);
uint64_t dsb_index_occ_host(const dsb_index *idx, uint64_t r, uint8_t *c);

int  dsb_device_count(void);
int  dsb_ctx_create(dsb_index *idx, int device_id, const dsb_opts *opts, dsb_ctx **ctx);
void dsb_ctx_destroy(dsb_ctx *ctx);
void dsb_ctx_reset_history(dsb_ctx *ctx);
void dsb_ctx_reload_env(dsb_ctx *ctx);
void dsb_ctx_set_history(dsb_ctx *ctx, uint32_t max_len_before);
int  dsb_ctx_use_synthetic_filter(dsb_ctx *ctx, uint64_t table_bytes, double fill);
int  dsb_synthetic_filter_bit(int which, uint64_t bit, double fill);
int  dsb_ctx_select_slot(dsb_ctx *ctx, int slot);

int  dsb_ctx_create_multi(dsb_index *idx, const int *device_ids, int n_dev, const dsb_opts *opts, dsb_multi **m);
void dsb_multi_destroy(dsb_multi *m);
int  dsb_multi_n(const dsb_multi *m);
dsb_ctx *dsb_multi_ctx(dsb_multi *m, int i);
void dsb_multi_reset_history(dsb_multi *m);
uint32_t dsb_multi_last_calls(const dsb_multi *m, int i);
int  dsb_multi_classify_batch(dsb_multi *m, const dsb_read *reads, size_t n, dsb_result *out);
typedef struct { uint64_t start, end; uint32_t hist_max_before; int32_t rank; } dsb_chunk;
int  dsb_shard_plan(const uint32_t *lengths, size_t n, int world, uint64_t chunk_bases, uint32_t chunk_reads, dsb_chunk *out, size_t cap, size_t *n_out);

int  dsb_classify_batch(dsb_ctx *ctx, const dsb_read *reads, size_t n, dsb_result *out);

int  dsb_batch_upload(dsb_ctx *ctx, const dsb_read *reads, size_t n);
int  dsb_batch_upload_text(dsb_ctx *ctx, const char *text, size_t text_len, const uint64_t *seq_off, const uint32_t *seq_len, size_t n);
void *dsb_host_alloc(size_t bytes);
void  dsb_host_free(void *p);
int   dsb_host_cpus(void);
long dsb_batch_upload_fastq(dsb_ctx *ctx, const char *path, size_t skip, size_t max_reads);
int  dsb_batch_run(dsb_ctx *ctx);
int  dsb_batch_fetch(dsb_ctx *ctx, dsb_result *out);
int  dsb_batch_timing(const dsb_ctx *ctx, dsb_timing *t);
int  dsb_batch_seeds(dsb_ctx *ctx, size_t read, int strand, dsb_seed *out, size_t cap, uint32_t *n, uint32_t *total_score);
int  dsb_batch_exist_bits(dsb_ctx *ctx, size_t read, int strand, uint8_t *out, size_t cap, uint32_t *n);

long dsb_format_sam(const dsb_index *idx, const dsb_read *read, const dsb_hit *hits, uint32_t n_hits,
                    int max_sec_N, int full, char *buf, size_t cap);

long dsb_format_des(const dsb_index *idx, const dsb_read *read, const dsb_read_result *rr, const dsb_hit *hits,
                    int max_sec_N, int full, char *buf, size_t cap);

typedef struct dsb_taxonomy dsb_taxonomy;
typedef struct dsb_report dsb_report;

int      dsb_taxonomy_load(const char *nodes_dmp, dsb_taxonomy **tx);
int      dsb_taxonomy_load_any(const char *nodes_dmp, dsb_taxonomy **tx);
void     dsb_taxonomy_close(dsb_taxonomy *tx);
uint32_t dsb_taxonomy_max_tid(const dsb_taxonomy *tx);
uint32_t dsb_taxonomy_parent(const dsb_taxonomy *tx, uint32_t taxid);

typedef struct {
	uint32_t taxid;
	uint32_t score;
	uint32_t len;
	uint8_t  mapq;
	uint8_t  flags;
	uint16_t pad;
} dsb_read_taxon;
#define DSB_TAXON_CLASSIFIED 1
#define DSB_TAXON_HOST       2

int  dsb_ctx_set_taxonomy(dsb_ctx *ctx, const dsb_taxonomy *tx);
int  dsb_multi_set_taxonomy(dsb_multi *m, const dsb_taxonomy *tx);
int  dsb_batch_taxa(dsb_ctx *ctx, const dsb_read_taxon **out);
int  dsb_multi_taxa(dsb_multi *m, const dsb_read_taxon **out);

int  dsb_report_create(const dsb_taxonomy *tx, dsb_report **rep);
int  dsb_report_add(dsb_report *rep, const dsb_index *idx, const dsb_read *reads, const dsb_result *res, const dsb_read_taxon *taxa,
                    size_t n, int max_sec_N);
int  dsb_report_add_sam(dsb_report *rep, const char *text, size_t len);
long dsb_report_format(const dsb_report *rep, int by_base, char *buf, size_t cap);
void dsb_report_destroy(dsb_report *rep);

typedef struct {
	uint64_t numreads;
	uint64_t covbases;
	uint64_t aligned_bases;
	uint64_t mapq_sum;
} dsb_ref_coverage;
int  dsb_ctx_enable_coverage(dsb_ctx *ctx, int on);
int  dsb_ctx_reset_coverage(dsb_ctx *ctx);
int  dsb_ctx_coverage(dsb_ctx *ctx, dsb_ref_coverage *out);
int  dsb_multi_enable_coverage(dsb_multi *m, int on);
int  dsb_multi_coverage(dsb_multi *m, dsb_ref_coverage *out);
long dsb_coverage_format(const dsb_index *idx, const dsb_ref_coverage *cov, char *buf, size_t cap);

typedef struct {
	uint64_t numreads;
	uint64_t uniqreads;
	double   est_reads;
	double   read_share;
	double   copy_share;
} dsb_ref_abundance;
typedef struct {
	uint32_t max_iter;
	uint32_t reserved;
	double   tol;
} dsb_em_opts;
typedef struct {
	uint64_t reads;
	uint64_t classified;
	uint64_t classes;
	uint32_t iterations;
	uint32_t converged;
	double   max_change;
	uint32_t min_permille;
	uint32_t reserved;
} dsb_abundance_summary;
int  dsb_ctx_enable_abundance(dsb_ctx *ctx, int on, uint32_t min_permille);
int  dsb_ctx_reset_abundance(dsb_ctx *ctx);
int  dsb_ctx_abundance(dsb_ctx *ctx, const dsb_em_opts *opts, dsb_ref_abundance *out, dsb_abundance_summary *summary);
int  dsb_multi_enable_abundance(dsb_multi *m, int on, uint32_t min_permille);
int  dsb_multi_abundance(dsb_multi *m, const dsb_em_opts *opts, dsb_ref_abundance *out, dsb_abundance_summary *summary);
long dsb_abundance_format(const dsb_index *idx, const dsb_ref_abundance *ab, const dsb_abundance_summary *summary, char *buf, size_t cap);

typedef struct { uint32_t taxid, score, n_pass; uint16_t depth; uint8_t flags, pad; } dsb_read_lca;
#define DSB_LCA_CLASSIFIED 1
#define DSB_LCA_NO_TAXON   2
#define DSB_LCA_AMBIGUOUS  4
typedef struct { uint32_t taxid, pad; uint64_t clade_reads, direct_reads; } dsb_taxon_count;
typedef struct { uint64_t reads, classified , no_taxon, ambiguous; uint32_t min_permille, reserved; } dsb_lca_summary;
int  dsb_ctx_enable_lca(dsb_ctx *ctx, int on, uint32_t min_permille);
int  dsb_ctx_reset_lca(dsb_ctx *ctx);
int  dsb_batch_lca(dsb_ctx *ctx, const dsb_read_lca **out);
int  dsb_ctx_lca_counts(dsb_ctx *ctx, dsb_taxon_count *out, size_t cap, size_t *n, dsb_lca_summary *summary);
int  dsb_multi_enable_lca(dsb_multi *m, int on, uint32_t min_permille);
int  dsb_multi_lca(dsb_multi *m, const dsb_read_lca **out);
int  dsb_multi_lca_counts(dsb_multi *m, dsb_taxon_count *out, size_t cap, size_t *n, dsb_lca_summary *summary);
typedef struct dsb_taxnames dsb_taxnames;
int  dsb_taxnames_load(const char *names_dmp, dsb_taxnames **names);
void dsb_taxnames_close(dsb_taxnames *names);
long dsb_format_kraken(const dsb_read *read, const dsb_read_lca *lca, char *buf, size_t cap);
long dsb_lca_report_format(const dsb_taxonomy *tx, const dsb_taxnames *names, const dsb_taxon_count *rows, size_t n,
                           const dsb_lca_summary *summary, char *buf, size_t cap);

const char *dsb_strerror(int code);
const char *dsb_version(void);

#ifdef __cplusplus
}
#endif
#endif
```

Baseline: 173,900.

## Parallelize read-order bucket sort and add optional LPT rerank after anchoring

The single-block k_order counting sort is replaced by a multi-block three-kernel sort (block histograms, one-block scan, block scatter) that runs by default to build the read order. An env-gated (default off) pass computes a longest-processing-time key per read from length, anchor count and steps, then re-sorts the non-heavy reads before classify to balance load. It also adds timing events and a debug dump API. The sort trades one kernel for three launches plus global atomics.

New measurement: 173,900. About the same (-0.0%).

```diff
diff --git a/desamba_amd/__init__.py b/desamba_amd/__init__.py
--- a/desamba_amd/__init__.py
+++ b/desamba_amd/__init__.py
@@ -45,7 +45,8 @@
                 ("n_occ", C.c_uint64), ("n_mem", C.c_uint64), ("n_sa", C.c_uint64), ("ref_bases", C.c_uint64),
                 ("main_occ", C.c_uint64), ("main_mem", C.c_uint64), ("main_sa", C.c_uint64), ("main_ref_bases", C.c_uint64),
                 ("n_heavy_mw", C.c_uint32), ("n_requeue", C.c_uint32), ("upload_bytes", C.c_uint64),
-                ("anc_pool_asked", C.c_uint64), ("anc_pool_cap", C.c_uint64)]
+                ("anc_pool_asked", C.c_uint64), ("anc_pool_cap", C.c_uint64),
+                ("lpt_ranked", C.c_uint32), ("anchor_ms", C.c_float), ("rerank_ms", C.c_float), ("pad_", C.c_uint32)]
 
 
 class DsbBuildStats(C.Structure):
@@ -105,7 +106,7 @@
 
 EXPORTS = ["dsb_index_open", "dsb_index_close", "dsb_index_n_ref", "dsb_index_ref_name", "dsb_index_ref_len", "dsb_index_ek_len",
            "dsb_index_occ_host", "dsb_ctx_create", "dsb_ctx_destroy", "dsb_ctx_reset_history", "dsb_ctx_reload_env", "dsb_classify_batch",
-           "dsb_batch_upload", "dsb_batch_upload_fastq", "dsb_batch_upload_text", "dsb_ctx_set_history", "dsb_host_alloc", "dsb_host_free", "dsb_host_cpus", "dsb_batch_run", "dsb_batch_fetch", "dsb_batch_timing", "dsb_batch_seeds", "dsb_batch_exist_bits",
+           "dsb_batch_upload", "dsb_batch_upload_fastq", "dsb_batch_upload_text", "dsb_ctx_set_history", "dsb_host_alloc", "dsb_host_free", "dsb_host_cpus", "dsb_batch_run", "dsb_batch_fetch", "dsb_batch_timing", "dsb_batch_lpt_dump", "dsb_batch_seeds", "dsb_batch_exist_bits",
            "dsb_format_sam", "dsb_format_des", "dsb_strerror", "dsb_version",
            "dsb_device_count", "dsb_ctx_select_slot", "dsb_ctx_create_multi", "dsb_multi_destroy", "dsb_multi_n", "dsb_multi_ctx",
            "dsb_multi_reset_history", "dsb_multi_last_calls", "dsb_multi_classify_batch", "dsb_shard_plan", "dsb_ctx_use_synthetic_filter", "dsb_synthetic_filter_bit", "dsb_index_prefix_interval", "dsb_index_build",
@@ -145,6 +146,8 @@
     L.dsb_batch_run.argtypes = [C.c_void_p]
     L.dsb_batch_fetch.argtypes = [C.c_void_p, C.POINTER(DsbResult)]
     L.dsb_batch_timing.argtypes = [C.c_void_p, C.POINTER(DsbTiming)]
+    if hasattr(L, "dsb_batch_lpt_dump"):
+        L.dsb_batch_lpt_dump.argtypes = [C.c_void_p, C.c_int, C.POINTER(C.c_uint32), C.c_size_t]
     L.dsb_batch_seeds.argtypes = [C.c_void_p, C.c_size_t, C.c_int, C.POINTER(DsbSeed), C.c_size_t, C.POINTER(C.c_uint32), C.POINTER(C.c_uint32)]
     L.dsb_batch_exist_bits.argtypes = [C.c_void_p, C.c_size_t, C.c_int, C.POINTER(C.c_uint8), C.c_size_t, C.POINTER(C.c_uint32)]
     L.dsb_format_sam.argtypes = [C.c_void_p, C.POINTER(DsbRead), C.POINTER(DsbHit), C.c_uint32, C.c_int, C.c_int, C.c_char_p, C.c_size_t]
@@ -358,6 +361,13 @@
         lib().dsb_batch_timing(self.h, C.byref(t))
         return t
 
+    def lpt_dump(self, what, n):
+        cnt = n * {0: 1, 1: 1, 2: 1, 3: 4, 4: 2}[what]
+        buf = (C.c_uint32 * max(cnt, 1))()
+        if lib().dsb_batch_lpt_dump(self.h, what, buf, cnt) != 0:
+            return None
+        return list(buf[:cnt])
+
     def seeds(self, read, strand):
         cap = (self.reads[read].len >> 1) + 64
         buf = (DsbSeed * cap)(); n = C.c_uint32(); ts = C.c_uint32()
diff --git a/desamba_amd/csrc/dsb_ctx.h b/desamba_amd/csrc/dsb_ctx.h
--- a/desamba_amd/csrc/dsb_ctx.h
+++ b/desamba_amd/csrc/dsb_ctx.h
@@ -32,6 +32,7 @@
 	bool anchor_kernel = true; long anc_pool_rt = 0;
 	bool scan_look_set = false; DsbScanLook scan_look;
 	std::string order_file;
+	bool lpt_rerank = false, lpt_dump = false;
 };
 inline bool g_upload_trace = false;
 
@@ -52,6 +53,8 @@
 	uint32_t hint_len = 0;
 	unsigned mw_reads = 16; bool mw_grown = false; int mw_calm = 0;
 	uint32_t *d_score = nullptr, *d_order = nullptr, *d_heavy = nullptr; size_t cap_score = 0, cap_order = 0, cap_heavy = 0;
+	uint32_t *d_lpt_list = nullptr, *d_lpt_key = nullptr, *d_lpt_feat = nullptr, *d_rank = nullptr; size_t cap_lpt_list = 0, cap_lpt_key = 0, cap_lpt_feat = 0;
+	uint32_t lpt_ranked = 0; bool anc_ran = false; hipEvent_t ev_anc = nullptr, ev_rank = nullptr;
 	DsbSeed *d_seeds = nullptr; DsbSeedInfo *d_sinfo = nullptr; size_t cap_seeds = 0, cap_sinfo = 0;
 	uint8_t *d_summ = nullptr; int summ_shift = 0;
 	uint8_t *syn0 = nullptr, *syn1 = nullptr; bool seed_only = false;
diff --git a/desamba_amd/csrc/dsb_gpu.hip b/desamba_amd/csrc/dsb_gpu.hip
--- a/desamba_amd/csrc/dsb_gpu.hip
+++ b/desamba_amd/csrc/dsb_gpu.hip
@@ -346,16 +346,79 @@
 	const uint32_t mant = lg >= 6u ? (s >> (lg - 6u)) & 63u : (s << (6u - lg)) & 63u;
 	return lg * 64u + mant;
 }
-__global__ void __launch_bounds__(1024) k_order(const uint32_t *score, uint32_t n, uint32_t *order)
-{
-	__shared__ uint32_t hist[2048], start[2048];
-	hist[threadIdx.x] = 0; hist[threadIdx.x + 1024] = 0;
+#define DSB_RANK_BUCKETS 2048u
+#define DSB_RANK_BLOCK 256u
+#define DSB_RANK_PER_BLOCK 1024u
+__global__ void __launch_bounds__(DSB_RANK_BLOCK) k_rank_hist(const uint32_t *key, uint32_t n, uint32_t *hist)
+{
+	__shared__ uint32_t h[DSB_RANK_BUCKETS];
+	for (uint32_t b = threadIdx.x; b < DSB_RANK_BUCKETS; b += DSB_RANK_BLOCK) h[b] = 0;
 	__syncthreads();
-	for (uint32_t i = threadIdx.x; i < n; i += 1024) atomicAdd(&hist[order_bucket(score[i])], 1u);
+	const uint32_t i0 = blockIdx.x * DSB_RANK_PER_BLOCK, i1 = i0 + DSB_RANK_PER_BLOCK < n ? i0 + DSB_RANK_PER_BLOCK : n;
+	for (uint32_t i = i0 + threadIdx.x; i < i1; i += DSB_RANK_BLOCK) atomicAdd(&h[order_bucket(key[i])], 1u);
 	__syncthreads();
-	if (threadIdx.x == 0) { uint32_t acc = 0; for (int b = 2047; b >= 0; b--) { start[b] = acc; acc += hist[b]; } }
+	for (uint32_t b = threadIdx.x; b < DSB_RANK_BUCKETS; b += DSB_RANK_BLOCK) if (h[b]) atomicAdd(&hist[b], h[b]);
+}
+__global__ void __launch_bounds__(1024) k_rank_scan(uint32_t *hist, uint32_t *start)
+{
+	__shared__ uint32_t s[1024];
+	const uint32_t t = threadIdx.x, b0 = DSB_RANK_BUCKETS - 1u - 2u * t, b1 = b0 - 1u;
+	const uint32_t a = hist[b0], b = hist[b1];
+	hist[b0] = 0; hist[b1] = 0;
+	s[t] = a + b;
 	__syncthreads();
-	for (uint32_t i = threadIdx.x; i < n; i += 1024) order[atomicAdd(&start[order_bucket(score[i])], 1u)] = i;
+	for (uint32_t d = 1; d < 1024u; d <<= 1) {
+		const uint32_t v = t >= d ? s[t - d] : 0u;
+		__syncthreads();
+		s[t] += v;
+		__syncthreads();
+	}
+	const uint32_t before = s[t] - (a + b);
+	start[b0] = before; start[b1] = before + a;
+}
+__global__ void __launch_bounds__(DSB_RANK_BLOCK) k_rank_scatter(const uint32_t *key, uint32_t n, uint32_t *start, const uint32_t *src, uint32_t *out)
+{
+	__shared__ uint32_t h[DSB_RANK_BUCKETS];
+	for (uint32_t b = threadIdx.x; b < DSB_RANK_BUCKETS; b += DSB_RANK_BLOCK) h[b] = 0;
+	__syncthreads();
+	const uint32_t i0 = blockIdx.x * DSB_RANK_PER_BLOCK, i1 = i0 + DSB_RANK_PER_BLOCK < n ? i0 + DSB_RANK_PER_BLOCK : n;
+	for (uint32_t i = i0 + threadIdx.x; i < i1; i += DSB_RANK_BLOCK) atomicAdd(&h[order_bucket(key[i])], 1u);
+	__syncthreads();
+	for (uint32_t b = threadIdx.x; b < DSB_RANK_BUCKETS; b += DSB_RANK_BLOCK) if (h[b]) h[b] = atomicAdd(&start[b], h[b]);
+	__syncthreads();
+	for (uint32_t i = i0 + threadIdx.x; i < i1; i += DSB_RANK_BLOCK) {
+		const uint32_t at = atomicAdd(&h[order_bucket(key[i])], 1u);
+		if (at < n) out[at] = src ? src[i] : i;
+	}
+}
+
+#define DSB_LPT_W_LEN_SHIFT 4
+#define DSB_LPT_W_ANC 8u
+#define DSB_LPT_W_LSTEPS_SHIFT 2
+__global__ void __launch_bounds__(256) k_lpt_key(const DsbReadDesc *rd, const uint32_t *order, uint32_t first, uint32_t n, const DsbAncRec *arec,
+        const DsbAnchor *apool, uint32_t *key, uint32_t *feat)
+{
+	const uint32_t p = first + blockIdx.x * 4u + (threadIdx.x >> 6), lane = threadIdx.x & 63u;
+	if (p >= n) return;
+	const uint32_t r = order[p];
+	const DsbAncRec rec = arec[r];
+	const uint32_t len = rd[r].len;
+	if (feat) {
+		uint32_t runs = 0; uint64_t seen = 0;
+		if (rec.use) for (uint32_t i = lane; i < rec.n; i += 64u) {
+			const DsbAnchor a = apool[rec.off + i];
+			if (i == 0) runs++;
+			else { const DsbAnchor b = apool[rec.off + i - 1]; if (a.ref_ID != b.ref_ID || a.direction != b.direction) runs++; }
+			seen |= 1ull << ((a.ref_ID * 0x9e3779b1u) >> 26);
+		}
+		for (int d = 32; d > 0; d >>= 1) { runs += __shfl_xor(runs, d, 64); seen |= (uint64_t)__shfl_xor((unsigned long long)seen, d, 64); }
+		if (lane == 0) { feat[2 * r] = runs; feat[2 * r + 1] = (uint32_t)__popcll(seen); }
+	}
+	if (lane == 0) {
+		uint64_t k = (uint64_t)(len >> DSB_LPT_W_LEN_SHIFT) + (uint64_t)DSB_LPT_W_ANC * rec.n + (rec.lsteps >> DSB_LPT_W_LSTEPS_SHIFT);
+		if (k > 0x7fffffffull) k = 0x7fffffffull;
+		key[p] = rec.use ? (uint32_t)k : 0x80000000u | (len > 0x7fffffffu ? 0x7fffffffu : len);
+	}
 }
 
 #endif
@@ -809,6 +872,7 @@
 	k.heavy_mw = getenv("DSB_HEAVY_MW") ? (int)num("DSB_HEAVY_MW", 0) : -1;
 	k.heavy_first_set = getenv("DSB_HEAVY_FIRST") != nullptr; k.heavy_first = (int)num("DSB_HEAVY_FIRST", 0);
 	k.anchor_kernel = num("DSB_ANCHOR_KERNEL", 1) != 0;
+	k.lpt_rerank = num("DSB_LPT_RERANK", 0) != 0; k.lpt_dump = getenv("DSB_LPT_DUMP") != nullptr;
 	if (getenv("DSB_EM_HASH_BITS")) { const long b = num("DSB_EM_HASH_BITS", 64); k.em_hash_mask = b >= 64 ? ~0ull : b < 1 ? 1ull : (1ull << b) - 1; }
 	k.anc_pool_rt = num("DSB_ANC_POOL_RT", 0); if (getenv("DSB_ANC_POOL_RT") && k.anc_pool_rt < 1) k.anc_pool_rt = 1;
 	if (const char *e = getenv("DSB_HEAVY_PREDS")) { k.heavy_preds_set = true; k.heavy_preds = (uint32_t)strtoul(e, nullptr, 10); }
@@ -851,11 +915,13 @@
 	for (InSlot &s : c->in) { hipFree(s.d_rd); hipFree(s.d_ascii); hipFree(s.d_scan_order); }
 	hipFree(c->d_wd); hipFree(c->d_bin); hipFree(c->d_pk); hipFree(c->d_bits);
 	reductions_release(c);
-	hipFree(c->d_rout); hipFree(c->d_hout); hipFree(c->d_counters); hipFree(c->arena.base); hipFree(c->arena_big.base); hipFree(c->arena_anc.base); hipFree(c->d_arec); hipFree(c->d_apool); hipFree(c->d_score); hipFree(c->d_order); hipFree(c->d_heavy); hipFree(c->d_seeds); hipFree(c->d_sinfo); hipFree(c->syn0); hipFree(c->syn1);
+	hipFree(c->d_rout); hipFree(c->d_hout); hipFree(c->d_counters); hipFree(c->arena.base); hipFree(c->arena_big.base); hipFree(c->arena_anc.base); hipFree(c->d_arec); hipFree(c->d_apool); hipFree(c->d_score); hipFree(c->d_order); hipFree(c->d_lpt_list); hipFree(c->d_lpt_key); hipFree(c->d_lpt_feat); hipFree(c->d_rank); hipFree(c->d_heavy); hipFree(c->d_seeds); hipFree(c->d_sinfo); hipFree(c->syn0); hipFree(c->syn1);
 	if (c->dbg_host) hipHostFree(c->dbg_host);
 	for (UpStage &u : c->up) { if (u.st) { hipStreamSynchronize(u.st); hipStreamDestroy(u.st); } for (int k = 0; k < 2; k++) { if (u.ev[k]) hipEventDestroy(u.ev[k]); if (u.buf[k]) hipHostFree(u.buf[k]); } }
 	for (int i = 0; i < 4; i++) if (c->ev[i]) hipEventDestroy(c->ev[i]);
 	if (c->ev_order) hipEventDestroy(c->ev_order);
+	if (c->ev_anc) hipEventDestroy(c->ev_anc);
+	if (c->ev_rank) hipEventDestroy(c->ev_rank);
 	if (c->ev_cls) hipEventDestroy(c->ev_cls);
 	if (c->ev_cls_wait) hipEventDestroy(c->ev_cls_wait);
 	if (c->ev_heavy) hipEventDestroy(c->ev_heavy);
@@ -895,6 +961,9 @@
 		c->dx = c->staged->dx; c->d_summ = c->staged->d_summ; c->summ_shift = c->staged->summ_shift; c->ek_dense = c->staged->ek_dense;
 		c->dx.filter_min_length = c->opts.L_min_matching; c->dx.filter_min_score = c->opts.min_score; c->dx.filter_min_score_LV3 = c->opts.min_score + 10;
 		if (hipMalloc((void **)&c->d_counters, 256) != hipSuccess) rc = DSB_ENOMEM;
+		if (rc == DSB_OK && hipMalloc((void **)&c->d_rank, 2 * DSB_RANK_BUCKETS * sizeof(uint32_t)) != hipSuccess) rc = DSB_ENOMEM;
+		if (rc == DSB_OK) CK(hipMemset(c->d_rank, 0, 2 * DSB_RANK_BUCKETS * sizeof(uint32_t)));
+		CK(hipEventCreate(&c->ev_anc)); CK(hipEventCreate(&c->ev_rank));
 	}
 	if (rc == DSB_OK && c->knobs.debug) {
 		CK(hipHostMalloc((void **)&c->dbg_host, 32 * 65536 * sizeof(uint32_t), hipHostMallocMapped | hipHostMallocCoherent));
@@ -1084,6 +1153,9 @@
 	if ((rc = grow(&c->d_order, &c->cap_order, n + 1))) return rc;
 	if (c->knobs.anchor_kernel) {
 		if ((rc = grow(&c->d_arec, &c->cap_arec, n + 1))) return rc;
+		if ((rc = grow(&c->d_lpt_list, &c->cap_lpt_list, n + 1))) return rc;
+		if ((rc = grow(&c->d_lpt_key, &c->cap_lpt_key, n + 1))) return rc;
+		if (c->knobs.lpt_dump && (rc = grow(&c->d_lpt_feat, &c->cap_lpt_feat, 2 * n + 2))) return rc;
 		uint64_t pool = (uint64_t)bin_bytes / 128 + 64 * (uint64_t)n;
 		if (c->knobs.anc_pool_rt) pool = (uint64_t)c->knobs.anc_pool_rt;
 		if (pool > 0xffffffffu) pool = 0xffffffffu;
@@ -1342,6 +1414,14 @@
 	                   pre_seeds ? c->d_seeds : nullptr, (const DsbSeedInfo *)c->d_sinfo, (const uint64_t *)c->d_pk, (uint32_t)((pre_seeds && s.max_len <= DSB_GROUP_MAX_LEN && !c->knobs.no_group) ? (c->knobs.group_head >= 0 ? (unsigned)c->knobs.group_head : 8u * grid) : 0u), arec, apool);
 }
 
+static void rank_launch(dsb_ctx *c, const uint32_t *key, uint32_t n, const uint32_t *src, uint32_t *out)
+{
+	const unsigned g = (n + DSB_RANK_PER_BLOCK - 1) / DSB_RANK_PER_BLOCK;
+	hipLaunchKernelGGL(k_rank_hist, dim3(g), dim3(DSB_RANK_BLOCK), 0, c->stream, key, n, c->d_rank);
+	hipLaunchKernelGGL(k_rank_scan, dim3(1), dim3(1024), 0, c->stream, c->d_rank, c->d_rank + DSB_RANK_BUCKETS);
+	hipLaunchKernelGGL(k_rank_scatter, dim3(g), dim3(DSB_RANK_BLOCK), 0, c->stream, key, n, c->d_rank + DSB_RANK_BUCKETS, src, out);
+}
+
 static int batch_run_locked(dsb_ctx *c, std::unique_lock<std::mutex> *turn);
 extern "C" int dsb_batch_run(dsb_ctx *c)
 {
@@ -1356,6 +1436,7 @@
 	size_t n = s.n_reads;
 	memset(&c->timing, 0, sizeof c->timing);
 	c->timing.upload_bytes = s.upload_bytes;
+	c->lpt_ranked = 0; c->anc_ran = false;
 	c->taxa.run = c->taxa.tx != nullptr && n == 0; c->taxa.done = false;
 	c->lca.run = c->lca.d_direct != nullptr && n == 0; c->lca.done = false;
 	if (n == 0) return DSB_OK;
@@ -1368,7 +1449,7 @@
 	const bool dbg = c->knobs.debug && c->dbg_dev;
 	if (dbg) { HIPCHK(hipStreamSynchronize(c->stream)); fprintf(stderr, "[dsb] encode done\n"); }
 	hipLaunchKernelGGL(k_repeat_score, dim3((unsigned)n), dim3(256), 0, c->stream, s.d_rd, c->d_pk, c->d_score);
-	hipLaunchKernelGGL(k_order, dim3(1), dim3(1024), 0, c->stream, c->d_score, (uint32_t)n, c->d_order);
+	rank_launch(c, c->d_score, (uint32_t)n, nullptr, c->d_order);
 	if (const char *of = c->knobs.order_file.empty() ? nullptr : c->knobs.order_file.c_str()) {
 		std::vector<uint32_t> ord(n); FILE *f = fopen(of, "rb");
 		if (f && fread(ord.data(), 4, n, f) == n) HIPCHK(hipMemcpyAsync(c->d_order, ord.data(), n * 4, hipMemcpyHostToDevice, c->stream));
@@ -1447,8 +1528,21 @@
 			unsigned ga = (unsigned)c->n_slots_anc; if (ga > n - n_heavy) ga = (unsigned)(n - n_heavy);
 			hipLaunchKernelGGL(k_anchor, dim3(ga), dim3(64), 0, c->stream, dx1, (const DsbReadDesc *)s.d_rd, (uint32_t)n, (uint32_t)n_heavy, (const uint32_t *)c->d_order, c->d_bin, c->arena_anc,
 			                   c->d_counters + 14, c->d_seeds, (const DsbSeedInfo *)c->d_sinfo, c->d_arec, c->d_apool, c->d_counters + 15, (uint32_t)c->cap_apool, (unsigned long long *)(c->d_counters + 16));
-		}
-		launch_classify(k_classify, c, c->stream, slots, dx1, s, (uint32_t)n, nullptr, (const uint32_t *)c->d_order, c->arena, c->d_counters, dbgp, (uint32_t)n_heavy, 0u, 0, use_scan,
+			HIPCHK(hipEventRecord(c->ev_anc, c->stream));
+		}
+		const uint32_t *main_list = c->d_order;
+		c->lpt_ranked = 0;
+		if (anc_k && c->knobs.lpt_rerank && c->knobs.order_file.empty() && c->d_lpt_list && c->cap_lpt_list >= n && c->d_lpt_key && c->cap_lpt_key >= n
+		    && (!c->knobs.lpt_dump || (c->d_lpt_feat && c->cap_lpt_feat >= 2 * n))) {
+			const uint32_t m = (uint32_t)(n - n_heavy);
+			hipLaunchKernelGGL(k_lpt_key, dim3((m + 3) / 4), dim3(256), 0, c->stream, (const DsbReadDesc *)s.d_rd, (const uint32_t *)c->d_order, (uint32_t)n_heavy, (uint32_t)n,
+			                   (const DsbAncRec *)c->d_arec, (const DsbAnchor *)c->d_apool, c->d_lpt_key, c->knobs.lpt_dump ? c->d_lpt_feat : (uint32_t *)nullptr);
+			rank_launch(c, c->d_lpt_key + n_heavy, m, c->d_order + n_heavy, c->d_lpt_list + n_heavy);
+			main_list = c->d_lpt_list; c->lpt_ranked = m;
+		}
+		if (anc_k) HIPCHK(hipEventRecord(c->ev_rank, c->stream));
+		c->anc_ran = anc_k;
+		launch_classify(k_classify, c, c->stream, slots, dx1, s, (uint32_t)n, nullptr, main_list, c->arena, c->d_counters, dbgp, (uint32_t)n_heavy, 0u, 0, use_scan,
 		                anc_k ? c->d_arec : nullptr, anc_k ? c->d_apool : nullptr);
 		HIPCHK(hipEventRecord(c->ev_cls, c->stream));
 		HIPCHK(hipEventRecord(c->ev_cls_wait, c->stream));
@@ -1524,6 +1618,8 @@
 	hipEventElapsedTime(&c->timing.classify_ms, c->ev[2], c->ev_cls);
 	hipEventElapsedTime(&c->timing.tail_ms, c->ev_cls, c->ev[3]);
 	c->timing.n_early = c->n_early;
+	c->timing.lpt_ranked = c->lpt_ranked;
+	if (c->anc_ran) { hipEventElapsedTime(&c->timing.anchor_ms, c->ev[2], c->ev_anc); hipEventElapsedTime(&c->timing.rerank_ms, c->ev_anc, c->ev_rank); }
 	hipEventElapsedTime(&c->timing.total_ms, c->ev[0], c->ev[3]);
 	unsigned long long wk[12] = {0};
 	HIPCHK(hipMemcpy(&c->p1, c->d_counters + 2, 8, hipMemcpyDeviceToHost));
@@ -1586,6 +1682,25 @@
 	if ((rc = dsb_batch_upload(c, reads, n))) return rc;
 	if ((rc = dsb_batch_run(c))) return rc;
 	return dsb_batch_fetch(c, out);
+}
+
+extern "C" int dsb_batch_lpt_dump(dsb_ctx *c, int what, uint32_t *out, size_t cap)
+{
+	if (!c || !out) return DSB_EINVAL;
+	HIPCHK(hipSetDevice(c->device));
+	const size_t n = c->in[c->cur].n_reads;
+	const uint32_t *src = nullptr; size_t cnt = n;
+	switch (what) {
+	case 0: src = c->d_order; break;
+	case 1: src = c->lpt_ranked ? c->d_lpt_list : nullptr; break;
+	case 2: src = c->lpt_ranked ? c->d_lpt_key : nullptr; break;
+	case 3: src = c->anc_ran ? (const uint32_t *)c->d_arec : nullptr; cnt = 4 * n; break;
+	case 4: src = c->lpt_ranked && c->knobs.lpt_dump ? c->d_lpt_feat : nullptr; cnt = 2 * n; break;
+	default: return DSB_EINVAL;
+	}
+	if (!src || cap < cnt) return DSB_EINVAL;
+	if (cnt) HIPCHK(hipMemcpy(out, src, cnt * sizeof(uint32_t), hipMemcpyDeviceToHost));
+	return DSB_OK;
 }
 
 extern "C" int dsb_batch_timing(const dsb_ctx *c, dsb_timing *t) { if (!c || !t) return DSB_EINVAL; *t = c->timing; return DSB_OK; }
diff --git a/desamba_amd/csrc/dsb_index.cpp b/desamba_amd/csrc/dsb_index.cpp
--- a/desamba_amd/csrc/dsb_index.cpp
+++ b/desamba_amd/csrc/dsb_index.cpp
@@ -278,7 +278,7 @@
 	}
 	return "unknown error";
 }
-extern "C" const char *dsb_version(void) { return "desamba_amd 0.5 (gfx950)"; }
+extern "C" const char *dsb_version(void) { return "desamba_amd 0.6 (gfx950)"; }
 
 extern "C" long dsb_format_des(const dsb_index *x, const dsb_read *rd_, const dsb_read_result *rr, const dsb_hit *h, int max_sec, int full, char *buf, size_t cap)
 {
diff --git a/include/desamba_amd.h b/include/desamba_amd.h
--- a/include/desamba_amd.h
+++ b/include/desamba_amd.h
@@ -79,6 +79,10 @@
 	uint64_t upload_bytes;
 	uint64_t anc_pool_asked;
 	uint64_t anc_pool_cap;
+	uint32_t lpt_ranked;
+	float anchor_ms;
+	float rerank_ms;
+	uint32_t pad_;
 } dsb_timing;
 
 typedef struct {
@@ -131,6 +135,7 @@
 int  dsb_batch_run(dsb_ctx *ctx);
 int  dsb_batch_fetch(dsb_ctx *ctx, dsb_result *out);
 int  dsb_batch_timing(const dsb_ctx *ctx, dsb_timing *t);
+int  dsb_batch_lpt_dump(dsb_ctx *ctx, int what, uint32_t *out, size_t cap);
 int  dsb_batch_seeds(dsb_ctx *ctx, size_t read, int strand, dsb_seed *out, size_t cap, uint32_t *n, uint32_t *total_score);
 int  dsb_batch_exist_bits(dsb_ctx *ctx, size_t read, int strand, uint8_t *out, size_t cap, uint32_t *n);
 
```
